# metalcycling/polynomial_reduction_with_full_domain_decomposition_preconditioner

Measured on AMD Instinct MI355X. Metric: PCG DOF-updates/sec + SpMV GB/s (%HBM peak), 3D Poisson N=7, higher is better.
Workload: dtype f64; 1 GPU; 3D Poisson, 32x32x32 elements (32^3 per GPU), N=7, flexible PCG + FDD preconditioner (single subdomain = whole domain, inner GMRES(4), polynomial reduction 6); outer=fcg, mesh=box, poly_degree=7, points_per_gpu=16777216, unique_nodes=11390625, preconditioner=fdd_gmres4, comm=single

## Files before the change

include/fdd_hip.h:

```cpp
#ifndef FDD_HIP_H
#define FDD_HIP_H

#include <stddef.h>

#ifdef __cplusplus
extern "C" {
#endif

#define FDD_ERR_INVALID_ARGUMENT (-1)
#define FDD_ERR_UNSUPPORTED (-2)
#define FDD_ERR_NOT_INITIALIZED (-3)

#define FDD_NUM_GEOM_FACTS 6
#define FDD_REDUCE_MAX_BLOCKS 2048

const char *fdd_version(void);
const char *fdd_last_error(void);
int fdd_device_count(int *count);
int fdd_set_device(int device);
int fdd_get_device(int *device);
int fdd_device_name(char *buf, size_t buf_len);
int fdd_malloc(void **ptr, size_t bytes);
int fdd_free(void *ptr);
int fdd_memcpy_h2d(void *dst, const void *src, size_t bytes, void *stream);
// ... 46 lines not shown
int fdd_dom_initialize_arrays(double *u_k, double *r_k, const double *f, int num_points, void *stream);

size_t fdd_reduce_workspace_doubles(void);
int fdd_dom_residual_norm(double *out, double *ws, const double *r_k, const double *QQt_r_k, const double *dirichlet_mask, int num_points, void *stream);
int fdd_dom_projection_inner_products(double *out2, double *ws, const double *z_k, const double *r_k, const double *p_k, const double *q_k, int num_points, void *stream);
int fdd_dom_inner_product_flexible(double *out, double *ws, const double *r_k, const double *r_kp1, const double *z_k, int num_points, void *stream);
int fdd_dom_inner_product_flexible_gamma(double *out2, double *ws, const double *r_k, const double *r_kp1, const double *z_k, int num_points, void *stream);
int fdd_dom_lincomb_flexible_gamma(double *out2, double *ws, const double *r_k, const double *r_kp1, double *z_k, int num_points, int slice_begin, int slice_size, int z_is_zero, const double *coeffs_dev, const double *const *v, const double *v_scale_dev, const double *last_dev, int m, void *stream);
int fdd_dom_inner_product(double *out, double *ws, const double *u_k, const double *v_k, const double *dirichlet_mask, int num_points, void *stream);

int fdd_dom_solution_and_residual_update(double *u_k, double *r_kp1, const double *r_k, const double *p_k, const double *q_k, double alpha_k, int num_points, void *stream);
int fdd_dom_residual_and_search_update(double *p_k, double *r_k, const double *z_k, const double *r_kp1, double beta_k, int num_points, void *stream);
int fdd_dom_solution_and_residual_update_dev(double *u_k, double *r_kp1, const double *r_k, const double *p_k, const double *q_k, const double *alpha_num, const double *alpha_den, int num_points, void *stream);
int fdd_dom_residual_and_search_update_dev(double *p_k, double *r_k, const double *z_k, const double *r_kp1, const double *beta_num, const double *beta_den, int num_points, void *stream);

int fdd_sub_stiffness_matrix_1(double *const GDu[3], const double *u, const double *const *D_hat_ptr, const int *offset, const int *vert, const int *level, const int *poly_degree, int num_levels, const double *const G[FDD_NUM_GEOM_FACTS], int num_points, int dim, void *stream);
int fdd_sub_stiffness_matrix_2(double *Au, const double *const GDu[3], const double *const *D_hat_ptr, const int *offset, const int *vert, const int *level, const int *poly_degree, int num_levels, int num_points, int dim, void *stream);
int fdd_sub_stiffness_matrix(double *Au, const double *u, const double *D_hat, const double *const G[FDD_NUM_GEOM_FACTS], const int *elem_offset, int num_elements, int poly_degree, void *stream);
int fdd_stiffness_matrix_2d(double *Au, const double *u, const double *D_hat, const double *const G[FDD_NUM_GEOM_FACTS], const int *elem_offset, int num_elements, int poly_degree, void *stream);
int fdd_sub_stiffness_matrix_gather(double *Au, const double *v, const int *point_dof, const double *D_hat, const double *const G[FDD_NUM_GEOM_FACTS], const int *elem_offset, int num_elements, int poly_degree, void *stream);

int fdd_sub_inner_product(double *out, double *ws, const double *u, const double *v, int num_values, void *stream);
int fdd_sub_weighted_inner_product(double *out, double *ws, const double *u, const double *v, const double *w, int num_values, void *stream);
int fdd_sub_projection_inner_products(double *out2, double *ws, const double *z_k, const double *r_k, const double *p_k, const double *q_k, const double *weight, int num_values, void *stream);
int fdd_sub_search_update_inner_product(double *out, double *ws, const double *r_k, const double *r_kp1, const double *z_k, const double *weight, int num_points, void *stream);
int fdd_sub_initialize_arrays(double *u_k, double *r_k, const double *f, int num_values, void *stream);
int fdd_sub_solution_and_residual_update(double *u_k, double *r_kp1, const double *r_k, const double *p_k, const double *q_k, double alpha_k, int num_values, void *stream);
int fdd_sub_residual_and_search_update(double *p_k, double *r_k, const double *z_k, const double *r_kp1, double beta_k, int num_values, void *stream);
int fdd_sub_copy_f64_f64(double *u, const double *v, int num_points, void *stream);
int fdd_sub_copy_f32_f64(float *u, const double *v, int num_points, void *stream);
int fdd_sub_copy_f64_f32(double *u, const float *v, int num_points, void *stream);
int fdd_sub_restriction_1(double *Ju, const double *J_cf, const double *u, int num_points, int n_f, int n_c, int dim, void *stream);
int fdd_sub_restriction_2(double *Ju, const double *J_cf, const double *u, int num_points, int n_f, int n_c, int dim, void *stream);
int fdd_sub_restriction_3(double *Ju, const double *J_cf, const double *u, int num_points, int n_f, int n_c, void *stream);
int fdd_sub_restriction(double *u_c, const double *J_cf, const double *u_f, int num_elements, int n_f, int n_c, void *stream);
int fdd_sub_restriction_2d(double *u_c, const double *J_cf, const double *u_f, int num_elements, int n_f, int n_c, void *stream);

int fdd_amg_vector_set_to_value(double *data, double value, int size, void *stream);
int fdd_amg_main_scaled_residual(double *Sr, double *w, const double *f_m_Au, const double *S, double alpha, int size, void *stream);
int fdd_amg_main_polynomial_evaluation(double *w, double *v, const double *r, const double *D_val, double alpha, int size, void *stream);
int fdd_amg_main_update_field(double *u, const double *w, const double *D_val, int size, void *stream);
int fdd_amg_vector_multiplication(double *uv, const double *u, const double *v, int size, void *stream);
int fdd_amg_matvec(double *y, const int *ptr, const int *col, const double *val, const double *x, double alpha, double beta, int num_rows, void *stream);
int fdd_csr_plan_matvec(const fdd_csr_plan *plan, double *y, const int *A_ptr, const int *A_col, const double *A_val, const double *x, double alpha, double beta, void *stream);
int fdd_csr_plan_matvec_to(const fdd_csr_plan *plan, double *y, const double *y_in, const int *A_ptr, const int *A_col, const double *A_val, const double *x, double alpha, double beta, void *stream);
int fdd_amg_smooth_residual_matvec(const fdd_csr_plan *plan, double *work, double *Sr, const int *A_ptr, const int *A_col, const double *A_val, const double *u, const double *f, const double *D_val, double coef, void *stream);
int fdd_amg_smooth_polynomial_matvec(const fdd_csr_plan *plan, double *work_out, const int *A_ptr, const int *A_col, const double *A_val, const double *work_in, const double *Sr, const double *D_val, double coef, void *stream);
int fdd_amg_smooth_update_matvec(const fdd_csr_plan *plan, double *u, const int *A_ptr, const int *A_col, const double *A_val, const double *work_in, const double *Sr, const double *D_val, double coef, void *stream);
int fdd_amg_smooth_start(double *work, double *Sr, const double *f, const double *D_val, double coef, int size, void *stream);

int fdd_lattice_supported(int n, int m, int *supported);
int fdd_lattice_prolong(double *u, const double *coarse, const int *owner_dof, const int *coarse_dof, int n, int m, const int *lo, const int *hi, const double *wl, long long num_elements, void *stream);
int fdd_lattice_prolong_f32(float *u, const float *coarse, const int *owner_dof, const int *coarse_dof, int n, int m, const int *lo, const int *hi, const double *wl, long long num_elements, void *stream);
int fdd_lattice_restrict(double *partial, const double *fine, const int *owner_dof, int n, int m, const int *lo, const int *hi, const double *wl, long long num_elements, void *stream);
int fdd_lattice_restrict_f32(float *partial, const float *fine, const int *owner_dof, int n, int m, const int *lo, const int *hi, const double *wl, long long num_elements, void *stream);
int fdd_csr_plan_create_f32(fdd_csr_plan **plan, const int *A_ptr_host, int num_rows, int num_cols, int num_nnz);
int fdd_csr_plan_matvec_to_f32(const fdd_csr_plan *plan, float *y, const float *y_in, const int *A_ptr, const int *A_col, const float *A_val, const float *x, float alpha, float beta, void *stream);
int fdd_amg_smooth_residual_matvec_f32(const fdd_csr_plan *plan, float *work, float *Sr, const int *A_ptr, const int *A_col, const float *A_val, const float *u, const float *f, const float *D_val, float coef, void *stream);
int fdd_amg_smooth_polynomial_matvec_f32(const fdd_csr_plan *plan, float *work_out, const int *A_ptr, const int *A_col, const float *A_val, const float *work_in, const float *Sr, const float *D_val, float coef, void *stream);
int fdd_amg_smooth_update_matvec_from_zero(const fdd_csr_plan *plan, double *u, const int *A_ptr, const int *A_col, const double *A_val, const double *work_in, const double *Sr, const double *D_val, double coef, void *stream);
int fdd_amg_smooth_update_matvec_from_zero_f32(const fdd_csr_plan *plan, float *u, const int *A_ptr, const int *A_col, const float *A_val, const float *work_in, const float *Sr, const float *D_val, float coef, void *stream);
int fdd_amg_smooth_update_matvec_f32(const fdd_csr_plan *plan, float *u, const int *A_ptr, const int *A_col, const float *A_val, const float *work_in, const float *Sr, const float *D_val, float coef, void *stream);
int fdd_amg_smooth_start_f32(float *work, float *Sr, const float *f, const float *D_val, float coef, int size, void *stream);
int fdd_amg_vector_set_to_value_f32(float *data, float value, int size, void *stream);
int fdd_amg_dot(double *out, double *ws, const double *x, const double *y, int size, void *stream);

#define FDD_MULTI_MAX 8
#define FDD_GMRES_SLOT (FDD_MULTI_MAX + 2)
int fdd_multi_weighted_inner_product(double *out, double *ws, const double *a, const double *const *b, int m, const double *w, int n, void *stream);
int fdd_multi_axpy(double *q, const double *coeffs, const double *const *v, int m, int n, void *stream);
int fdd_multi_axpy_norm2_dev(double *out, double *ws, double *y, const double *coeffs_dev, double sign, const double *const *x, int m, const double *w, int n, void *stream);
int fdd_vector_scaling_rsqrt_dev(double *au, const double *norm2_dev, const double *u, int n, void *stream);
int fdd_multi_axpy_dev(double *q, const double *coeffs_dev, const double *const *v, int m, int n, void *stream);

#define FDD_PROJECTION_MAX 16
int fdd_projection_dots(double *out, double *ws, const double *X, int ld, int K, const double *f, int n, void *stream);
int fdd_projection_apply(double *x, double *b, double *nu2_out, double *ws, const double *x_in, const double *b_in, const double *X, const double *AX, int ld, int K, const double *coeffs_dev, double sign_x, double sign_b, int n, void *stream);
int fdd_projection_store(double *Xk, double *AXk, const double *x, const double *b, const double *nu2_dev, int n, void *stream);

int fdd_cheby_step(double *x, double *d, double *r_out, const double *r_in, const double *q, const double *dinv, double c_d, double c_r, int first, int last, int n, void *stream);
int fdd_cheby_step_f32(float *x, float *d, float *r_out, const float *r_in, const float *q, const float *dinv, float c_d, float c_r, int first, int last, int n, void *stream);
int fdd_csr_plan_gather_cheby(const fdd_csr_plan *plan, double *x, double *d, double *r_out, const int *Qt_ptr, const int *Qt_col, const double *u, const double *r_in, const double *dinv, double c_d, double c_r, int last, void *stream);
int fdd_csr_plan_gather_cheby_f32(const fdd_csr_plan *plan, float *x, float *d, float *r_out, const int *Qt_ptr, const int *Qt_col, const float *u, const float *r_in, const float *dinv, float c_d, float c_r, int last, void *stream);

size_t fdd_gmres_state_bytes(void);
int fdd_gmres_begin_dev(void *state, const double *norm2_dev, int first_cycle, void *stream);
int fdd_gmres_step_dev(void *state, const double *dots_dev, int j, int iterations_before, int max_iterations, double tolerance, int use_relative, void *stream);
int fdd_gmres_finish_dev(void *state, int m, void *stream);
int fdd_gmres_fetch(void *state, double *y, double *hist, int *num_hist, int *j_last, int *steps, int *converged, void *stream);
int fdd_gmres_coefficients(void *state, const double **y_dev);
int fdd_gmres_scales(void *state, const double **inv_dev);
int fdd_gmres_last_column(void *state, const double **j_last_dev);
int fdd_sub_stiffness_matrix_gather_scaled(double *Au, const double *v, const double *v_scale_dev, const int *point_dof, const double *D_hat, const double *const G[FDD_NUM_GEOM_FACTS], const int *elem_offset, int num_elements, int poly_degree, void *stream);
int fdd_multi_weighted_inner_product_scaled(double *out, double *ws, const double *a, const double *const *b, const double *b_scale_dev, int m, const double *w, int n, void *stream);
int fdd_multi_axpy_norm2_scaled_dev(double *out, double *ws, double *dst, const double *y, const double *coeffs_dev, double sign, const double *const *x, const double *x_scale_dev, int m, const double *w, int n, void *stream);
int fdd_multi_axpy_scaled_dev(double *q, const double *coeffs_dev, const double *const *v, const double *v_scale_dev, int m, int n, void *stream);
int fdd_vector_scaling_dev(double *au, const double *scale_dev, const double *u, int n, void *stream);
int fdd_multi_lincomb_scaled_dev(double *q, int q_is_zero, const double *coeffs_dev, const double *const *v, const double *v_scale_dev, int m, int n, void *stream);
int fdd_multi_lincomb_limited_dev(double *q, int q_is_zero, const double *coeffs_dev, const double *const *v, const double *v_scale_dev, const double *last_dev, int m, int n, void *stream);
int fdd_sqrt_sum_dev(double *out, const double *parts_dev, int nparts, void *stream);
int fdd_stiffness_matrix_affine(double *Au, const double *v, const double *v_scale_dev, const int *point_dof, const double *D_hat, const double *elem_factors, const double *gll_weights, const int *elem_offset, int num_elements, int poly_degree, void *stream);
int fdd_stiffness_matrix_mfma_affine(double *Au, const double *v, const double *v_scale_dev, const int *point_dof, const double *D_hat, const double *elem_factors, const double *gll_weights, const int *elem_offset, int num_elements, int poly_degree, void *stream);
int fdd_stiffness_affine_detect(double *elem_factors, double *deviation, const double *const G[FDD_NUM_GEOM_FACTS], const int *elem_offset, const double *gll_weights, int num_elements, int poly_degree, void *stream);
int fdd_stiffness_matrix_diag(double *Au, const double *v, const double *v_scale_dev, const int *point_dof, const double *D_hat, const double *const G[FDD_NUM_GEOM_FACTS], const int *elem_offset, int num_elements, int poly_degree, void *stream);
int fdd_stiffness_matrix_diag_f32(float *Au, const float *v, const double *v_scale_dev, const int *point_dof, const float *D_hat, const float *const G[FDD_NUM_GEOM_FACTS], const int *elem_offset, int num_elements, int poly_degree, void *stream);
int fdd_stiffness_matrix_lines(double *Au, const double *v, const double *v_scale_dev, const int *point_dof, const double *D_hat, const double *const G[FDD_NUM_GEOM_FACTS], const int *elem_offset, int num_elements, int poly_degree, int diag, void *stream);
int fdd_stiffness_matrix_lines_f32(float *Au, const float *v, const double *v_scale_dev, const int *point_dof, const float *D_hat, const float *const G[FDD_NUM_GEOM_FACTS], const int *elem_offset, int num_elements, int poly_degree, int diag, void *stream);
int fdd_stiffness_offdiag_zero(int *flags_out, const double *const G[FDD_NUM_GEOM_FACTS], const int *elem_offset, int num_elements, int poly_degree, void *stream);
int fdd_stiffness_matrix_lines_shared(double *Au, const double *v, const double *v_scale_dev, const int *point_dof, const double *D_hat, const double *const G[FDD_NUM_GEOM_FACTS], const int *elem_offset, const int *factor_elem, int num_elements, int poly_degree, int diag, void *stream);
int fdd_stiffness_matrix_lines_shared_f32(float *Au, const float *v, const double *v_scale_dev, const int *point_dof, const float *D_hat, const float *const G[FDD_NUM_GEOM_FACTS], const int *elem_offset, const int *factor_elem, int num_elements, int poly_degree, int diag, void *stream);
int fdd_stiffness_matrix_lines_lean(double *Au, const double *v, const double *v_scale_dev, const int *point_dof, const double *D_hat, const double *const G[FDD_NUM_GEOM_FACTS], const int *elem_offset, const int *factor_elem, int num_elements, int poly_degree, int diag, void *stream);
int fdd_stiffness_matrix_lines_lean_f32(float *Au, const float *v, const double *v_scale_dev, const int *point_dof, const float *D_hat, const float *const G[FDD_NUM_GEOM_FACTS], const int *elem_offset, const int *factor_elem, int num_elements, int poly_degree, int diag, void *stream);
int fdd_stiffness_factor_block_hash(unsigned long long *out, const double *const G[FDD_NUM_GEOM_FACTS], const int *elem_offset, int num_elements, int poly_degree, void *stream);
int fdd_stiffness_factor_block_verify(int *mismatches, const double *const G[FDD_NUM_GEOM_FACTS], const int *elem_offset, const int *factor_elem, int num_elements, int poly_degree, void *stream);
int fdd_stiffness_matrix_affine_f32(float *Au, const float *v, const double *v_scale_dev, const int *point_dof, const float *D_hat, const float *elem_factors, const float *gll_weights, const int *elem_offset, int num_elements, int poly_degree, void *stream);
int fdd_sub_stiffness_matrix_gather_scaled_f32(float *Au, const float *v, const double *v_scale_dev, const int *point_dof, const float *D_hat, const float *const G[FDD_NUM_GEOM_FACTS], const int *elem_offset, int num_elements, int poly_degree, void *stream);
int fdd_multi_inner_product_scaled_f32(double *out, double *ws, const float *a, const float *const *b, const double *b_scale_dev, int m, int n, void *stream);
int fdd_multi_axpy_norm2_scaled_dev_f32(double *out, double *ws, float *dst, const float *y, const double *coeffs_dev, double sign, const float *const *x, const double *x_scale_dev, int m, int n, void *stream);
int fdd_vector_scaling_dev_f32(float *au, const double *scale_dev, const float *u, int n, void *stream);
int fdd_vector_diagonal_scaling_dev(double *z, const double *d, const double *scale_dev, const double *u, int n, void *stream);
int fdd_vector_diagonal_scaling_dev_f32(float *z, const float *d, const double *scale_dev, const float *u, int n, void *stream);
int fdd_vector_vector_addition_f32(float *uv, float alpha, const float *u, float beta, const float *v, int n, void *stream);
int fdd_multi_lincomb_limited_dev_f32(float *q, int q_is_zero, const double *coeffs_dev, const float *const *v, const double *v_scale_dev, const double *last_dev, int m, int n, void *stream);
int fdd_gather_rows_f32(float *t, const int *ptr, const int *col, const float *u, int row_lo, int row_hi, void *stream);
int fdd_csr_plan_gather_f32(const fdd_csr_plan *plan, float *t, const int *ptr, const int *col, const float *u, int row_lo, int row_hi, void *stream);
int fdd_gather_indexed_f32(float *out, const float *in, const int *index, int n, void *stream);
int fdd_gather_indexed_f32_f64(double *out, const float *in, const int *index, int n, void *stream);
int fdd_xmay_ratio_dev(double *out, const double *x, const double *num_dev, const double *den_dev, const double *y, int n, void *stream);
int fdd_xpby_ratio_dev(double *out, const double *x, const double *num_dev, const double *den_dev, const double *y, int n, void *stream);
int fdd_gather_weighted_norm2(double *out, double *ws, const int *Qt_ptr, const int *Qt_col, const double *u, const double *node_weight, int num_nodes, void *stream);

int fdd_dssum_fused(double *QQtu, double *t, const int *Qt_ptr, const int *Qt_col, const double *u, const double *node_weight, const double *point_mask, int node_start, int node_end, void *stream);
int fdd_dssum_gather(double *t, const int *Qt_ptr, const int *Qt_col, const double *u, const double *node_weight, int node_start, int node_end, void *stream);
int fdd_dssum_scatter(double *QQtu, const double *t, const int *Qt_ptr, const int *Qt_col, const double *point_mask, int node_start, int node_end, void *stream);
int fdd_fill_indexed(double *out, const int *idx, double value, int n, void *stream);
int fdd_gather_indexed(double *out, const double *in, const int *index, const double *scale, int n, void *stream);
int fdd_gather_indexed_split(double *out, const double *lo, const double *hi, int split, const int *index, int n, void *stream);
int fdd_scatter_add_indexed(double *y, const int *index, const double *t, int n, void *stream);
int fdd_scatter_add_indexed_f32(float *y, const int *index, const float *t, int n, void *stream);
int fdd_csr_plan_dssum(const fdd_csr_plan *plan, double *QQtu, double *t, const int *Qt_ptr, const int *Qt_col, const double *u, const double *node_weight, const double *point_mask, int row_lo, int row_hi, int mode, void *stream);
int fdd_csr_plan_gather_weighted_norm2(const fdd_csr_plan *plan, double *out, double *ws, const int *Qt_ptr, const int *Qt_col, const double *u, const double *node_weight, void *stream);

int fdd_interface_pack(double *slots, const int *slot_of, const double *prefix, int n, void *stream);
int fdd_interface_unpack(double *prefix, const double *slots, const int *slot_of, int n, void *stream);
int fdd_interface_gather(double *buf, const int *index, int n, const double *a, const double *b, void *stream);
int fdd_interface_sum(double *a, double *b, const int *ptr, const int *col, int rows, const double *buf, void *stream);

int fdd_amg_setup_row_pointers(int *ptr, int *ptr_host, const int *row_len, int rows, void *stream);
int fdd_amg_setup_spgemm_count(int *row_len, int *cursor_ws, const int *A_ptr, const int *A_col, const int *B_ptr, const int *B_col, int a_rows, int b_rows, void *stream);
int fdd_amg_setup_spgemm_fill(int *C_col, double *C_val, int *cursor_ws, const int *C_ptr, const int *A_ptr, const int *A_col, const double *A_val, const int *B_ptr, const int *B_col, const double *B_val, int a_rows, int b_rows, void *stream);
int fdd_amg_setup_transpose_count(int *row_len, const int *A_ptr, const int *A_col, const double *A_val, int a_rows, int a_cols, double drop_tol, void *stream);
int fdd_amg_setup_transpose_fill(int *T_col, double *T_val, int *cursor_ws, int *src_ws, const int *T_ptr, const int *A_ptr, const int *A_col, const double *A_val, int a_rows, int a_cols, int nnz_t, double drop_tol, void *stream);
int fdd_amg_setup_fem_stencils(double *K, unsigned int *mask, const double *x, const double *y, const double *z, const int *point_dof, int poly_degree, int num_elements, double epsilon, void *stream);
int fdd_amg_setup_fem_count(int *row_len, const int *dof_ptr, const int *dof_points, const unsigned int *mask, const int *point_dof, int poly_degree, int num_dofs, void *stream);
int fdd_amg_setup_fem_fill(int *A_col, double *A_val, const int *A_ptr, const int *dof_ptr, const int *dof_points, const unsigned int *mask, const double *K, const int *point_dof, int poly_degree, int num_dofs, void *stream);
int fdd_amg_setup_inv_sqrt_diagonal(double *D, const int *A_ptr, const int *A_col, const double *A_val, int rows, void *stream);
int fdd_amg_setup_unit_values(int *flag, const double *val, long long nnz, void *stream);
int fdd_amg_setup_lattice_dofs(int *first, int *kept, const int *point_dof, long long num_elements, int num_dofs, int n, int m, const int *keep, const int *lo, const int *hi, const double *wl, void *stream);
int fdd_amg_setup_lattice_coarse_flags(int *flag, const int *first, const int *kept, int num_dofs, void *stream);
int fdd_amg_setup_lattice_cmap(int *cmap, int *owner_dof, int *unplaced, const int *cstart, const int *first, const int *kept, long long num_points, int num_dofs, void *stream);
int fdd_amg_setup_lattice_interp_count(int *row_len, const int *cmap, const int *first, const int *point_dof, int num_dofs, int n, int m, const int *keep, const int *lo, const int *hi, const double *wl, void *stream);
int fdd_amg_setup_lattice_interp_fill(int *P_col, double *P_val, const int *P_ptr, const int *cmap, const int *first, const int *point_dof, int num_dofs, int n, int m, const int *keep, const int *lo, const int *hi, const double *wl, void *stream);
int fdd_amg_setup_lattice_coarse_points(int *coarse_point_dof, const int *point_dof, const int *cmap, long long num_elements, int n, int m, const int *keep, const int *lo, const int *hi, const double *wl, void *stream);
int fdd_amg_setup_memory_info(size_t *free_bytes, size_t *total_bytes);

#ifdef __cplusplus
}
#endif

#endif
```

include/fdd_host.h:

```cpp
#ifndef FDD_HOST_H
#define FDD_HOST_H

#include <stddef.h>

#ifdef __cplusplus
extern "C" {
#endif

const char *fddh_last_error(void);

int fddh_init(int device, void *stream, int own_stream);
int fddh_set_print(int on);
int fddh_set_timer(int on);
int fddh_timer_total(const char *key, double *seconds);
int fddh_timer_total_over_ranks(const char *key, const char *aggregation, double *seconds);

int fddh_comm_single(void);
int fddh_comm_rccl_unique_id(char *out128);
int fddh_comm_rccl_init(const char *id128, int rank, int size);
typedef int (*fddh_allreduce_fn)(void *ctx, void *buf, long long n);
typedef int (*fddh_allgather_fn)(void *ctx, const void *send, void *recv, long long bytes);
typedef int (*fddh_barrier_fn)(void *ctx);
int fddh_comm_callbacks(int rank, int size, void *ctx, fddh_allreduce_fn allreduce_sum_f64, fddh_allreduce_fn allreduce_max_f64, fddh_allgather_fn allgather_bytes, fddh_barrier_fn barrier);
typedef int (*fddh_exchange_fn)(void *ctx, int n, const int *peers, const void *const *send, const long long *send_bytes, void *const *recv, const long long *recv_bytes);
int fddh_comm_callbacks_ex(int rank, int size, void *ctx, fddh_allreduce_fn allreduce_sum_f64, fddh_allreduce_fn allreduce_max_f64, fddh_allgather_fn allgather_bytes, fddh_barrier_fn barrier, fddh_exchange_fn exchange_bytes);
int fddh_local_world_create(void **world, int size);
int fddh_local_world_destroy(void *world);
int fddh_local_world_fail(void *world);
int fddh_rank_finalize(void);
int fddh_comm_local(void *world, int rank);
int fddh_comm_info(int *rank, int *size, char *name, size_t name_len);
int fddh_comm_selftest(int n);

typedef struct fddh_problem fddh_problem;

int fddh_problem_create_box(fddh_problem **out, const int E[3], const int P[3], int poly_degree, int poly_reduction, int with_subdomain);
int fddh_problem_create_dir(fddh_problem **out, const char *directory, int poly_degree, int poly_reduction, int subdomain_overlap, int superdomain_overlap, int with_subdomain);
enum
{
    FDDH_WITH_SUBDOMAIN = 1,
    FDDH_BLOCK_LOCAL = 2,
    FDDH_FORCE_COMPOSITE = 4
};
int fddh_problem_create_box_ex(fddh_problem **out, const int E[3], const int P[3], int poly_degree, int poly_reduction, int subdomain_overlap, int superdomain_overlap, int flags);
int fddh_problem_create_dir_ex(fddh_problem **out, const char *directory, int poly_degree, int poly_reduction, int subdomain_overlap, int superdomain_overlap, int flags);
int fddh_problem_destroy(fddh_problem *p);
int fddh_write_box_mesh_files(const char *directory, const int E[3], const int P[3], int poly_degree, int rank);
int fddh_problem_create_kershaw_ex(fddh_problem **out, const int E[3], const int P[3], int poly_degree, int poly_reduction, int subdomain_overlap, int superdomain_overlap, int flags, double eps_y, double eps_z);
int fddh_write_kershaw_mesh_files(const char *directory, const int E[3], const int P[3], int poly_degree, int rank, double eps_y, double eps_z);

enum
{
    FDDH_INFO_NUM_LOCAL_POINTS = 0,
    FDDH_INFO_NUM_LOCAL_NODES,
    FDDH_INFO_NUM_BDARY_NODES,
    FDDH_INFO_NUM_INTERFACE_SLOTS,
    FDDH_INFO_NUM_TOTAL_NODES,
    FDDH_INFO_NUM_TOTAL_ELEMENTS,
    FDDH_INFO_NUM_LOCAL_ELEMENTS,
    FDDH_INFO_NUM_LEVELS,
    FDDH_INFO_SUB_NUM_VALUES,
    FDDH_INFO_SUB_NUM_DOFS,
    FDDH_INFO_NUM_ITERATIONS,
    FDDH_INFO_DIM,
    FDDH_INFO_COUNT
};
int fddh_problem_info(const fddh_problem *p, long long *info, int n);
int fddh_problem_level_degree(const fddh_problem *p, int level, int *poly_degree);

enum
{
    FDDH_SUB_IS_COMPOSITE = 0,
    FDDH_SUB_NUM_ELEMS,
    FDDH_SUB_NUM_EXT_ELEMS,
    FDDH_SUB_NUM_POINTS,
    FDDH_SUB_NUM_SUB_DOFS,
    FDDH_SUB_NUM_SUB_EXT_DOFS,
    FDDH_SUB_NUM_INTERFACE_DOFS,
    FDDH_SUB_NUM_SUP_DOFS,
    FDDH_SUB_NUM_SUP_EXT_DOFS,
    FDDH_SUB_NUM_UNIQUE_DOFS,
    FDDH_SUB_NUM_COARSE_DOFS,
    FDDH_SUB_NUM_VALUES,
    FDDH_SUB_OWN_POINTS,
    FDDH_SUB_NUM_PEERS,
    FDDH_SUB_INFO_COUNT
};
int fddh_problem_sub_info(const fddh_problem *p, long long *info, int n);
int fddh_problem_sub_region(const fddh_problem *p, int *element, int *level, int n);
int fddh_problem_sub_composite_levels(const fddh_problem *p, int *kept, int n, int *num_levels);

int fddh_problem_mesh_array(const fddh_problem *p, int level, const char *name, void *out, size_t bytes);
int fddh_problem_csr(const fddh_problem *p, int which , int *num_rows, int *num_cols, int *num_nnz, int *ptr, int *col, double *val);
int fddh_problem_assembled_weight(const fddh_problem *p, double *out, int n);

int fddh_problem_set_D_hat(fddh_problem *p, int level, const double *D_hat, int n);
int fddh_problem_get_D_hat(const fddh_problem *p, int level, double *D_hat, int n);

int fddh_problem_set_options(fddh_problem *p, int max_iterations, double tolerance, int num_vectors, int use_preconditioner, int preconditioner_type, int sub_num_vectors, int sub_max_iterations, int sub_build_tree);

int fddh_problem_affine_info(fddh_problem *p, int *fine_domain_affine, int *sub_lists_affine, int *sub_lists, double *max_deviation);
int fddh_problem_zero_factor_info(fddh_problem *p, int *enabled, int *fine_domain_diag, int *sub_lists_diag, int *sub_lists);
int fddh_problem_mfma_zero_factor_info(fddh_problem *p, int *enabled, int *fine_domain_mfma_diag, int *sub_lists_mfma_diag, int *sub_lists);
int fddh_problem_line_stiffness_info(fddh_problem *p, int *enabled, int *fine_domain_lines, int *sub_lists_lines, int *sub_lists);
int fddh_problem_shared_factor_info(fddh_problem *p, int *enabled, int *fine_domain_shared, int *fine_domain_classes, int *sub_lists_shared, int *sub_lists);
int fddh_problem_lean_line_info(fddh_problem *p, int *enabled, int *fine_domain_table_ok, int *fine_domain_lean, int *sub_lists_lean, int *sub_lists);
int fddh_problem_set_flag(fddh_problem *p, const char *name, int value);

int fddh_problem_sub_point_dofs(const fddh_problem *p, int *dof, int n);
int fddh_problem_amg_add_level(fddh_problem *p, int n, const int *A_ptr, const int *A_col, const double *A_val, const double *D_val, const double *coefs, int num_coefs, int n_coarse, const int *P_ptr, const int *P_col, const double *P_val);
int fddh_problem_amg_finalize(fddh_problem *p);
int fddh_problem_amg_apply(fddh_problem *p, const double *r, double *z);
int fddh_problem_amg_build(fddh_problem *p, int coarsest_size, double strength, int smooth_prolongator, int verbose, int *num_levels);
int fddh_problem_amg_level_info(const fddh_problem *p, int level, int *n, int *nnz_A, int *n_coarse, int *nnz_P);
int fddh_problem_amg_setup_info(const fddh_problem *p, int *levels_built_on_device, double *setup_seconds);
int fddh_problem_amg_level_transfer(const fddh_problem *p, int level, int *matrix_free);
int fddh_problem_amg_level_arrays(const fddh_problem *p, int level, int *A_ptr, int *A_col, double *A_val, double *D_val, double *coefs, int *P_ptr, int *P_col, double *P_val);

int fddh_problem_dssum(fddh_problem *p, double *out, const double *in, int apply_mask, int apply_weight);
int fddh_problem_stiffness(fddh_problem *p, double *out, const double *in, int apply_dssum);
int fddh_problem_residual_norm(fddh_problem *p, const double *r, double *norm);
int fddh_problem_make_rhs(fddh_problem *p, int function_id, unsigned long long seed, double *u_star, double *f);
int fddh_problem_make_rhs_from(fddh_problem *p, double *u_star_inout, double *f);

int fddh_problem_solve(fddh_problem *p, int solver_id, const double *f, double *u, double *history, int history_cap, int *num_history, int *num_iterations);

int fddh_problem_solve_timed(fddh_problem *p, int solver_id, const double *f, double *u, double *history, int history_cap, int *num_history, int *num_iterations, double *seconds);

int fddh_problem_projection_configure(fddh_problem *p, int capacity);
int fddh_problem_projection_clear(fddh_problem *p);
int fddh_problem_projection_info(const fddh_problem *p, int *capacity, int *size, long long *restarts);
int fddh_problem_projection_basis(const fddh_problem *p, int k, double *x, double *Ax);
int fddh_problem_solve_projected(fddh_problem *p, int solver_id, const double *f, double *u, double *history, int history_cap, int *num_history, int *num_iterations, double *projection, double *seconds);

int fddh_problem_precond_apply(fddh_problem *p, int type, const double *r, double *z, double *history, int history_cap, int *num_history);
int fddh_problem_sub_op(fddh_problem *p, int op, const double *in, double *out);
int fddh_problem_sub_residual_norm(fddh_problem *p, const double *r, double *norm);
int fddh_problem_sub_dof_op(fddh_problem *p, int op, const double *in, double *out, int n);
int fddh_problem_sub_jacobi_diagonal(fddh_problem *p, double *out, int n);
int fddh_problem_sub_dof_solve(fddh_problem *p, const double *fa, double *ua, int n);

int fddh_problem_inner_chebyshev_configure(fddh_problem *p, int order, double lower, double upper, int power_iterations);
int fddh_problem_inner_chebyshev_info(fddh_problem *p, int *order, double *lower, double *upper, double *lambda, int *power_iterations);

int fddh_problem_spmv_time(fddh_problem *p, int which, int iterations, double *avg_us, double *algorithmic_bytes);
#define FDDH_COMM_TIME_COUNT 6
int fddh_problem_comm_time(fddh_problem *p, int iterations, double *avg_us, double *bytes);
int fddh_spmv_stencil_time(int m, int iterations, double *avg_us, double *algorithmic_bytes, long long *num_nnz);

int fddh_problem_pcg_begin(fddh_problem *p, const double *f);
int fddh_problem_pcg_steps(fddh_problem *p, int steps, double *last_residual);
int fddh_problem_pcg_solution(fddh_problem *p, double *u);
int fddh_profile_enable(int on);
int fddh_profile_only(const char *kernel_key);
int fddh_profile_collect(char *json, size_t json_len);

int fddh_sync(void);
int fddh_barrier(void);

#ifdef __cplusplus
}
#endif

#endif
```

polynomial_reduction_with_full_domain_decomposition_preconditioner_amd/csrc/fdd_csr.hip:

```cpp
#include <type_traits>

#include "fdd_common.h"

#include <algorithm>
#include <cstdlib>
#include <vector>

namespace
{

constexpr int kBlock = 256;
constexpr int kBlockNnzMax = FDD_CSR_BLOCK_NNZ;
constexpr int kBlockNnzSmall = FDD_CSR_BLOCK_NNZ / 2;

template <typename F>
void with_block_nnz(int block_nnz, F &&f)
{
    if (block_nnz == kBlockNnzSmall)
        f(std::integral_constant<int, kBlockNnzSmall>{});
    else
        f(std::integral_constant<int, kBlockNnzMax>{});
}
template <bool kMayBeUnit = true, typename F>
void with_unit(bool unit, F &&f)
{
    if constexpr (kMayBeUnit)
    {
        if (unit) return f(std::true_type{});
    }
    f(std::false_type{});
}

template <typename T>
struct EpiPlainT
{
    static constexpr bool kFreeOrder = false;
    typedef T Opnd;
    __device__ T operand(int, const T *) const { return T(0); }
    __device__ T finish(T s, T, int) const { return s; }
};
typedef EpiPlainT<double> EpiPlain;
struct EpiWeight
{
    static constexpr bool kFreeOrder = false;
    typedef double Opnd;
    const double *weight;
    __device__ double operand(int row, const double *) const { return weight[row]; }
    __device__ double finish(double s, double w, int) const { return s * w; }
};
template <typename T>
struct EpiAxpbyT
{
    static constexpr bool kFreeOrder = true;
    typedef T Opnd;
    T alpha, beta;
    const T *y_in;
    __device__ T operand(int row, const T *y_old) const { return (beta == T(0)) ? T(0) : (y_in ? y_in[row] : y_old[row]); }
    __device__ T finish(T s, T y, int) const { return (beta == T(0)) ? alpha * s : alpha * s + beta * y; }
};
typedef EpiAxpbyT<double> EpiAxpby;

template <typename T>
struct Opnd2
{
    T a, b;
};
template <typename T>
struct Opnd3
{
    T a, b, c;
};
template <typename T>
struct EpiSmoothResidualT
{
    static constexpr bool kFreeOrder = true;
    typedef Opnd2<T> Opnd;
    const T *f, *D;
    T *r;
    T coef;
    __device__ Opnd operand(int row, const T *) const { return Opnd{f[row], D[row]}; }
    __device__ T finish(T s, Opnd o, int row) const
    {
        const T work = T(-1) * s + T(1) * o.a;
        const T sr = o.b * work;
        r[row] = sr;
        const T w = coef * sr;
        return w * o.b;
    }
};
template <typename T>
struct EpiSmoothPolyT
{
    static constexpr bool kFreeOrder = true;
    typedef Opnd2<T> Opnd;
    const T *r, *D;
    T coef;
    __device__ Opnd operand(int row, const T *) const { return Opnd{r[row], D[row]}; }
    __device__ T finish(T s, Opnd o, int) const
    {
        const T v = (T(1) * s) * o.b;
        const T w = coef * o.a + v;
        return w * o.b;
    }
};
template <typename T>
struct EpiSmoothUpdateT
{
    static constexpr bool kFreeOrder = true;
    typedef Opnd3<T> Opnd;
    const T *r, *D;
    T coef;
    __device__ Opnd operand(int row, const T *u_old) const { return Opnd{r[row], D[row], u_old[row]}; }
    __device__ T finish(T s, Opnd o, int) const
    {
        const T v = (T(1) * s) * o.b;
        const T w = coef * o.a + v;
        return o.c + o.b * w;
    }
};
template <typename T>
struct EpiSmoothUpdateZeroT
{
    static constexpr bool kFreeOrder = true;
    typedef Opnd2<T> Opnd;
// ... 457 lines not shown
    int b = fdd_xcd_windowed_block(blockIdx.x, G, xcd_window);
    if (b >= nblocks) return;

    auto bounds = [&](int4 m, int &r0, int &nrows, int &base, int &nnz) {
        r0 = m.x;
        int r1 = m.y;
        base = m.z;
        nnz = m.w;
        if (r0 < row_lo || r1 > row_hi)
        {
            r0 = r0 > row_lo ? r0 : row_lo;
            r1 = r1 < row_hi ? r1 : row_hi;
            if (r1 < r0) r1 = r0;
            base = A_ptr[r0];
            nnz = A_ptr[r1] - base;
        }
        nrows = r1 - r0;
    };
    auto load_streams = [&](int (&c)[kIts], T (&a)[kIts], int (&rp)[kRowIts], typename Epi::Opnd (&o)[kRowIts], int r0, int nrows, int base, int nnz) {
#pragma unroll
        for (int it = 0; it < kIts; it++)
        {
            const int k = threadIdx.x + it * kBlock;
            const int ks = (k < nnz) ? base + k : ((nnz > 0) ? base : 0);
            c[it] = __builtin_nontemporal_load(A_col + ks);
            a[it] = UNIT ? T(1) : __builtin_nontemporal_load(A_val + ks);
        }
#pragma unroll
        for (int it = 0; it < kRowIts; it++)
        {
            const int r = threadIdx.x + it * kBlock;
            const int rs = (r < nrows) ? r : 0;
            rp[it] = A_ptr[r0 + rs + 1];
            o[it] = epi.operand(r0 + rs, Au);
        }
    };

    int r0, nrows, base, nnz;
    bounds(meta[block_first + b], r0, nrows, base, nnz);
    int c[kIts], rp[kRowIts];
    T a[kIts];
    typename Epi::Opnd o[kRowIts];
    load_streams(c, a, rp, o, r0, nrows, base, nnz);
    int bn = b + G;
    int4 mn = meta[block_first + (bn < nblocks ? bn : b)];

    for (;;)
    {
        const bool more = bn < nblocks;
        T v[kIts];
#pragma unroll
        for (int it = 0; it < kIts; it++) v[it] = u[c[it]];
        int r0n, nrowsn, basen, nnzn;
        bounds(mn, r0n, nrowsn, basen, nnzn);
        int cn[kIts], rpn[kRowIts];
        T an[kIts];
        typename Epi::Opnd on[kRowIts];
        load_streams(cn, an, rpn, on, r0n, nrowsn, basen, nnzn);
        const int bnn = bn + G;
        const int4 mnn = meta[block_first + (bnn < nblocks ? bnn : (more ? bn : b))];

#pragma unroll
        for (int it = 0; it < kIts; it++)
        {
            const int k = threadIdx.x + it * kBlock;
            if (k < nnz) x[k] = a[it] * v[it];
        }
        if (threadIdx.x == 0) sp[0] = 0;
#pragma unroll
        for (int it = 0; it < kRowIts; it++)
        {
            const int r = threadIdx.x + it * kBlock;
            if (r < nrows) sp[r + 1] = rp[it] - base;
        }
        __syncthreads();
#pragma unroll
        for (int it = 0; it < kRowIts; it++)
        {
            const int r = threadIdx.x + it * kBlock;
            if (r < nrows)
            {
                T s = T(0);
                for (int j = sp[r]; j < sp[r + 1]; j++) s += x[j];
                Au[r0 + r] = epi.finish(s, o[it], r0 + r);
            }
        }
        if (!more) break;
        __syncthreads();
        b = bn;
        bn = bnn;
        mn = mnn;
        r0 = r0n;
        nrows = nrowsn;
        base = basen;
        nnz = nnzn;
#pragma unroll
        for (int it = 0; it < kIts; it++)
        {
            c[it] = cn[it];
            a[it] = an[it];
        }
#pragma unroll
        for (int it = 0; it < kRowIts; it++)
        {
            rp[it] = rpn[it];
            o[it] = on[it];
        }
    }
}

inline int gather_pipelined_per_cu()
{
    static const int v = fdd_env_int("FDD_TUNE_GATHER_PIPELINED", 4);
    return v;
}

template <int kBlockNnz>
__global__ __launch_bounds__(kBlock) void gather_norm2_block_kernel(double *__restrict__ ws, const int *__restrict__ Qt_ptr, const int *__restrict__ Qt_col, const double *__restrict__ u, const double *__restrict__ w, const int *__restrict__ row_blocks, int num_blocks)
{
    __shared__ double x[kBlockNnz];
    __shared__ double wsum[kBlock / FDD_WAVE];
    constexpr int kIts = kBlockNnz / kBlock;
    double acc = 0.0;

    for (int b = blockIdx.x; b < num_blocks; b += gridDim.x)
    {
        const int r0 = row_blocks[b];
        const int r1 = row_blocks[b + 1];
        const int base = Qt_ptr[r0];
        const int nnz = Qt_ptr[r1] - base;
        int c[kIts];
#pragma unroll
        for (int it = 0; it < kIts; it++)
        {
            const int k = threadIdx.x + it * kBlock;
            c[it] = Qt_col[(k < nnz) ? base + k : ((nnz > 0) ? base : 0)];
        }
        __syncthreads();
#pragma unroll
        for (int it = 0; it < kIts; it++)
        {
            const int k = threadIdx.x + it * kBlock;
            const double v = u[c[it]];
            if (k < nnz) x[k] = 1.0 * v;
        }
        __syncthreads();
        for (int row = r0 + threadIdx.x; row < r1; row += kBlock)
        {
            const int j0 = Qt_ptr[row] - base;
            const int j1 = Qt_ptr[row + 1] - base;
            double s = 0.0;
            for (int j = j0; j < j1; j++) s += x[j];
            const double wn = w[row];
            s = s * wn;
            acc += s * s * wn;
        }
    }

    acc = wave_sum(acc);
    if ((threadIdx.x & (FDD_WAVE - 1)) == 0) wsum[threadIdx.x / FDD_WAVE] = acc;
    __syncthreads();
    if (threadIdx.x == 0)
    {
        double tsum = wsum[0];
#pragma unroll
        for (int k = 1; k < kBlock / FDD_WAVE; k++) tsum += wsum[k];
        ws[blockIdx.x] = tsum;
// ... 572 lines not shown
static int plan_gather_cheby(const fdd_csr_plan *plan, T *x, T *d, T *r_out, const int *Qt_ptr, const int *Qt_col, const T *u, const T *r_in, const T *dinv, T c_d, T c_r, int last, void *stream)
{
    FDD_REQUIRE(plan != nullptr);
    if (plan->num_rows == 0) return 0;
    FDD_REQUIRE(x != nullptr && d != nullptr && Qt_ptr != nullptr && Qt_col != nullptr && u != nullptr && r_in != nullptr && dinv != nullptr && (last || r_out != nullptr));
    FDD_REQUIRE((const void *)u != (const void *)x && (const void *)u != (const void *)d && (const void *)u != (const void *)r_out);
    constexpr bool kDouble = std::is_same<T, double>::value;
    if (plan->value_bytes != (int)sizeof(T))
    {
        fdd_set_error("%s", kDouble ? "fdd_csr_plan_gather_cheby: a plan of fdd_csr_plan_create_f32" : "fdd_csr_plan_gather_cheby_f32: not a plan of fdd_csr_plan_create_f32");
        return FDD_ERR_INVALID_ARGUMENT;
    }
    if (!(plan->unit_values && plan->sell_slices == 0 && launch_short_pipelined<T>(plan, x, Qt_ptr, Qt_col, (const T *)nullptr, u, EpiChebyStepT<T>{r_in, dinv, r_out, d, c_d, c_r, last ? 1 : 0}, BlockRange{0, plan->num_blocks}, 0, plan->num_rows, fdd_stream(stream), true)))
    {
        fdd_set_error("fdd_csr_plan_gather_cheby%s: not a unit-value plan of the pipelined short-row kernel", kDouble ? "" : "_f32");
        return FDD_ERR_INVALID_ARGUMENT;
    }
    FDD_LAUNCH_CHECK();
    return 0;
}
extern "C" {

int fdd_csr_plan_gather_cheby(const fdd_csr_plan *plan, double *x, double *d, double *r_out, const int *Qt_ptr, const int *Qt_col, const double *u, const double *r_in, const double *dinv, double c_d, double c_r, int last, void *stream)
{
    return plan_gather_cheby<double>(plan, x, d, r_out, Qt_ptr, Qt_col, u, r_in, dinv, c_d, c_r, last, stream);
}

int fdd_csr_plan_gather_cheby_f32(const fdd_csr_plan *plan, float *x, float *d, float *r_out, const int *Qt_ptr, const int *Qt_col, const float *u, const float *r_in, const float *dinv, float c_d, float c_r, int last, void *stream)
{
    return plan_gather_cheby<float>(plan, x, d, r_out, Qt_ptr, Qt_col, u, r_in, dinv, c_d, c_r, last, stream);
}

int fdd_csr_plan_dssum(const fdd_csr_plan *plan, double *QQtu, double *t, const int *Qt_ptr, const int *Qt_col, const double *u, const double *node_weight, const double *point_mask, int row_lo, int row_hi, int mode, void *stream)
{
    FDD_REQUIRE(plan != nullptr && mode >= 0 && mode <= 2);
    FDD_REQUIRE(row_lo >= 0 && row_hi >= row_lo && row_hi <= plan->num_rows);
    if (row_hi == row_lo) return 0;
    FDD_REQUIRE(plan->unit_values != 0);
    FDD_REQUIRE(Qt_ptr != nullptr && Qt_col != nullptr);
    FDD_REQUIRE(mode == 1 || QQtu != nullptr);
    FDD_REQUIRE(mode == 2 || u != nullptr);
    FDD_REQUIRE(mode == 0 || t != nullptr);

    if (plan->kind == 0 || plan->has_long_rows)
    {
        if (mode == 0) return fdd_dssum_fused(QQtu, t, Qt_ptr, Qt_col, u, node_weight, point_mask, row_lo, row_hi, stream);
        if (mode == 1) return fdd_dssum_gather(t, Qt_ptr, Qt_col, u, node_weight, row_lo, row_hi, stream);
        return fdd_dssum_scatter(QQtu, t, Qt_ptr, Qt_col, point_mask, row_lo, row_hi, stream);
    }

    const BlockRange blocks = blocks_overlapping(plan, row_lo, row_hi);
    if (blocks.empty()) return 0;
    hipStream_t s = fdd_stream(stream);
    const bool W = node_weight != nullptr && mode != 2, M = point_mask != nullptr && mode != 1;
    const auto run = [&](auto kMode, auto kWeight, auto kMask) {
        launch_dssum_blocks<double, decltype(kMode)::value, decltype(kWeight)::value, decltype(kMask)::value>(plan, blocks, QQtu, t, Qt_ptr, Qt_col, u, node_weight, point_mask, row_lo, row_hi, s);
    };
    constexpr std::integral_constant<int, 0> fused{};
    constexpr std::integral_constant<int, 1> gather{};
    constexpr std::integral_constant<int, 2> scatter{};
    constexpr std::true_type yes{};
    constexpr std::false_type no{};
    if (mode == 0)
    {
        if (W && M) run(fused, yes, yes);
        else if (W) run(fused, yes, no);
        else if (M) run(fused, no, yes);
        else run(fused, no, no);
    }
    else if (mode == 1)
    {
        if (W) run(gather, yes, no);
        else if (!launch_short_pipelined<double>(plan, t, Qt_ptr, Qt_col, (const double *)nullptr, u, EpiPlain{}, blocks, row_lo, row_hi, s, true)) run(gather, no, no);
    }
    else
    {
        if (M) run(scatter, no, yes);
        else run(scatter, no, no);
    }
    FDD_LAUNCH_CHECK();
    return 0;
}

int fdd_csr_plan_gather_weighted_norm2(const fdd_csr_plan *plan, double *out, double *ws, const int *Qt_ptr, const int *Qt_col, const double *u, const double *node_weight, void *stream)
{
    FDD_REQUIRE(plan != nullptr && out != nullptr && ws != nullptr);
    hipStream_t s = fdd_stream(stream);
    if (plan->num_rows == 0) return (int)hipMemsetAsync(out, 0, sizeof(double), s);
    FDD_REQUIRE(plan->unit_values != 0 && Qt_ptr != nullptr && Qt_col != nullptr && u != nullptr && node_weight != nullptr);
    if (plan->kind == 0 || plan->has_long_rows) return fdd_gather_weighted_norm2(out, ws, Qt_ptr, Qt_col, u, node_weight, plan->num_rows, stream);
    const int grid = plan->num_blocks < FDD_REDUCE_MAX_BLOCKS ? plan->num_blocks : FDD_REDUCE_MAX_BLOCKS;
    with_block_nnz(plan->block_nnz, [&](auto nnz) {
        hipLaunchKernelGGL(gather_norm2_block_kernel<decltype(nnz)::value>, dim3(grid), dim3(kBlock), 0, s, ws, Qt_ptr, Qt_col, u, node_weight, plan->row_blocks_dev, plan->num_blocks);
    });
    FDD_LAUNCH_CHECK();
    hipLaunchKernelGGL(fold_partials_kernel, dim3(1), dim3(kBlock), 0, s, out, ws, grid);
    FDD_LAUNCH_CHECK();
    return 0;
}

int fdd_csr_plan_set_unit_values(fdd_csr_plan *plan, int unit_values)
{
    FDD_REQUIRE(plan != nullptr);
    plan->unit_values = unit_values != 0;
    return 0;
}

int fdd_csr_plan_kind(const fdd_csr_plan *plan, int *kind)
{
    FDD_REQUIRE(plan != nullptr && kind != nullptr);
    *kind = plan->kind;
    return 0;
}

int fdd_csr_plan_pipelined(const fdd_csr_plan *plan, int *pipelined)
{
    FDD_REQUIRE(plan != nullptr && pipelined != nullptr);
    *pipelined = (plan->sell_slices == 0 && short_pipelined_applies(plan)) ? 1 : 0;
    return 0;
}

int fdd_csr_plan_multiply(const fdd_csr_plan *plan, double *Au, const int *A_ptr, const int *A_col, const double *A_val, const double *u, const double *weight, void *stream)
{
    FDD_REQUIRE(plan != nullptr);
    FDD_REQUIRE(plan->value_bytes == 8);
    if (plan->num_rows == 0 || plan->num_cols == 0) return 0;
    FDD_REQUIRE(Au != nullptr && A_ptr != nullptr && u != nullptr);

    if (weight) return plan_launch<double, false>(plan, Au, A_ptr, A_col, A_val, u, EpiWeight{weight}, stream);
    return plan_launch<double, false>(plan, Au, A_ptr, A_col, A_val, u, EpiPlain{}, stream);
}

int fdd_csr_plan_matvec(const fdd_csr_plan *plan, double *y, const int *A_ptr, const int *A_col, const double *A_val, const double *x, double alpha, double beta, void *stream)
{
    return fdd_csr_plan_matvec_to(plan, y, nullptr, A_ptr, A_col, A_val, x, alpha, beta, stream);
}

int fdd_csr_plan_matvec_to(const fdd_csr_plan *plan, double *y, const double *y_in, const int *A_ptr, const int *A_col, const double *A_val, const double *x, double alpha, double beta, void *stream)
{
    return plan_spmv_entry(plan, y, A_ptr, A_col, A_val, x, EpiAxpby{alpha, beta, y_in}, stream, FDD_PRECONDITION(y != nullptr && A_ptr != nullptr && x != nullptr && y != x));
}

int fdd_amg_smooth_residual_matvec(const fdd_csr_plan *plan, double *work, double *Sr, const int *A_ptr, const int *A_col, const double *A_val, const double *u, const double *f, const double *D_val, double coef, void *stream)
{
    return plan_spmv_entry(plan, work, A_ptr, A_col, A_val, u, EpiSmoothResidual{f, D_val, Sr, coef}, stream, FDD_PRECONDITION(work != nullptr && Sr != nullptr && A_ptr != nullptr && u != nullptr && f != nullptr && D_val != nullptr && work != u && Sr != u));
}

int fdd_amg_smooth_polynomial_matvec(const fdd_csr_plan *plan, double *work_out, const int *A_ptr, const int *A_col, const double *A_val, const double *work_in, const double *Sr, const double *D_val, double coef, void *stream)
{
    return plan_spmv_entry(plan, work_out, A_ptr, A_col, A_val, work_in, EpiSmoothPoly{Sr, D_val, coef}, stream, FDD_PRECONDITION(work_out != nullptr && A_ptr != nullptr && work_in != nullptr && Sr != nullptr && D_val != nullptr && work_out != work_in));
}

int fdd_amg_smooth_update_matvec(const fdd_csr_plan *plan, double *u, const int *A_ptr, const int *A_col, const double *A_val, const double *work_in, const double *Sr, const double *D_val, double coef, void *stream)
{
    return plan_spmv_entry(plan, u, A_ptr, A_col, A_val, work_in, EpiSmoothUpdate{Sr, D_val, coef}, stream, FDD_PRECONDITION(u != nullptr && A_ptr != nullptr && work_in != nullptr && Sr != nullptr && D_val != nullptr && u != work_in));
}

int fdd_amg_smooth_update_matvec_from_zero(const fdd_csr_plan *plan, double *u, const int *A_ptr, const int *A_col, const double *A_val, const double *work_in, const double *Sr, const double *D_val, double coef, void *stream)
{
    return plan_spmv_entry(plan, u, A_ptr, A_col, A_val, work_in, EpiSmoothUpdateZeroT<double>{Sr, D_val, coef}, stream, FDD_PRECONDITION(u != nullptr && A_ptr != nullptr && work_in != nullptr && Sr != nullptr && D_val != nullptr && u != work_in));
}

int fdd_csr_plan_matvec_to_f32(const fdd_csr_plan *plan, float *y, const float *y_in, const int *A_ptr, const int *A_col, const float *A_val, const float *x, float alpha, float beta, void *stream)
{
    return plan_spmv_entry(plan, y, A_ptr, A_col, A_val, x, EpiAxpbyT<float>{alpha, beta, y_in}, stream, FDD_PRECONDITION(y != nullptr && A_ptr != nullptr && A_val != nullptr && x != nullptr && y != x));
}
// ... 23 lines not shown
```

polynomial_reduction_with_full_domain_decomposition_preconditioner_amd/csrc/fdd_stiffness.hip:

```cpp
#include "fdd_common.h"

namespace
{

constexpr int kBlock = 256;

template <typename T>
struct GPtrsT
{
    const T *g[FDD_NUM_GEOM_FACTS];
};

struct GPtrs
{
    const double *g[FDD_NUM_GEOM_FACTS];
};
struct GDuPtrs
{
    double *g[3];
};
struct LevelTable
{
    const double *D_hat[16];
    int poly_degree[16];
// ... 483 lines not shown
#pragma unroll
    for (int p = 0; p < 8; p++)
    {
        const T *Dp = line_row(D_hat, p);
#pragma unroll
        for (int i = 0; i < 8; i++) au[i] += Dp[i] * gdu[p];
    }
}

enum : int
{
    kLeanTerms = 1,
    kLeanResident = 2
};

template <typename T, bool kResident>
struct LeanTable
{
    static constexpr int slot(int m) { return m - (m > 9) - (m > 18) - (m > 27); }
    const T *D_hat;
    T d[kResident ? 29 : 1];
    __device__ __forceinline__ explicit LeanTable(const T *__restrict__ D) : D_hat(D)
    {
        if constexpr (kResident)
        {
            T top[32];
#pragma unroll
            for (int m = 0; m < 32; m++) top[m] = D[m];
#pragma unroll
            for (int m = 0; m < 32; m++)
                if (m != 9 and m != 18 and m != 27)
                {
                    T v = top[m];
                    asm volatile("" : "+s"(v));
                    d[slot(m)] = v;
                }
        }
    }
    __device__ __forceinline__ const T *row(int r) const { return kResident ? nullptr : line_row(D_hat, r); }
    __device__ __forceinline__ T at(const T *row_r, int r, int c) const
    {
        if constexpr (kResident)
        {
            const int m = c + 8 * r;
            return m < 32 ? d[slot(m)] : -d[slot(63 - m)];
        }
        else
            return row_r[c];
    }
};
__device__ __forceinline__ constexpr bool lean_zero_entry(int r, int c) { return r == c and r >= 1 and r <= 6; }

template <typename T, bool kResident>
__device__ __forceinline__ void lean_du(T (&du)[8], const T (&ul)[8], const LeanTable<T, kResident> &D)
{
#pragma unroll
    for (int i = 0; i < 8; i++)
    {
        const T *Di = D.row(i);
        du[i] = D.at(Di, i, 0) * ul[0];
#pragma unroll
        for (int p = 1; p < 8; p++)
            if (not lean_zero_entry(i, p)) du[i] += D.at(Di, i, p) * ul[p];
    }
}
template <typename T, bool kResident>
__device__ __forceinline__ void lean_au(T (&au)[8], const T (&gdu)[8], const LeanTable<T, kResident> &D)
{
#pragma unroll
    for (int p = 0; p < 8; p++)
    {
        const T *Dp = D.row(p);
#pragma unroll
        for (int i = 0; i < 8; i++)
        {
            if (p == 0)
                au[i] = D.at(Dp, 0, i) * gdu[0];
            else if (not lean_zero_entry(p, i))
                au[i] += D.at(Dp, p, i) * gdu[p];
        }
    }
}

template <typename T, bool kGather, bool kNTStore, bool kShared = false, int kLean = 0>
__global__ __launch_bounds__(kBlock, 4) void line_stiffness_kernel_t(T *__restrict__ Au, const T *__restrict__ u, const int *__restrict__ point_dof, const double *__restrict__ u_scale, const T *__restrict__ D_hat, GPtrsT<T> G, const int *__restrict__ elem_offset, int num_elements, const int *__restrict__ factor_elem)
{
    using C = LineCfg;
    constexpr int n = C::n, nn = C::nn;
    __shared__ T s_a[C::epb][C::tile];
    __shared__ T s_b[C::epb][C::tile];

    const int tid = threadIdx.x;
    const int e_loc = __builtin_amdgcn_readfirstlane(tid >> 6);
    const int l = tid & 63;
    const int a = l & 7, b = l >> 3;
    const int elem = blockIdx.x * C::epb + e_loc;
    if (elem >= num_elements) return;
    const size_t base = elem_offset ? (size_t)elem_offset[elem] : (size_t)elem * C::n3;
    size_t fbase = base;
    if (kShared)
    {
        const int rep = factor_elem[elem];
        fbase = elem_offset ? (size_t)elem_offset[rep] : (size_t)rep * C::n3;
    }
    T *ta = s_a[e_loc], *tb = s_b[e_loc];
    constexpr bool kTerms = (kLean & kLeanTerms) != 0, kResident = (kLean & kLeanResident) != 0;
    static_assert(kTerms or not kResident, "the resident table does not hold the diagonal entries");
    const LeanTable<T, kResident> Dl(D_hat);

    T r_u[n];
    if (kGather)
    {
        const int *pd = point_dof + base;
        int d[n];
#pragma unroll
        for (int k = 0; k < n; k++) d[k] = __builtin_nontemporal_load(pd + (l + k * nn));
#pragma unroll
        for (int k = 0; k < n; k++) r_u[k] = u[d[k] < 0 ? 0 : d[k]];
#pragma unroll
        for (int k = 0; k < n; k++) r_u[k] = (d[k] < 0) ? T(0) : r_u[k];
        if (u_scale)
        {
            const T sc = (T)(*u_scale);
#pragma unroll
            for (int k = 0; k < n; k++) r_u[k] = sc * r_u[k];
        }
    }
    else
    {
        const T *up = u + base;
#pragma unroll
        for (int k = 0; k < n; k++) r_u[k] = __builtin_nontemporal_load(up + (l + k * nn));
    }

    T r_3[n];
    if constexpr (not kTerms)
    {
#pragma unroll
        for (int m = 0; m < n; m++) r_3[m] = T(0);
    }

    {
        T g0[n], g1[n], g2[n];
#pragma unroll
        for (int k = 0; k < n; k++) g2[k] = kShared ? G.g[2][fbase + (l + k * nn)] : __builtin_nontemporal_load(G.g[2] + fbase + (l + k * nn));
        {
            const T *g0p = G.g[0] + fbase + 8 * l;
#pragma unroll
            for (int p = 0; p < n; p++) g0[p] = g0p[p];
        }
        {
            const T *g1p = G.g[1] + fbase + (a + nn * b);
#pragma unroll
            for (int p = 0; p < n; p++) g1[p] = kShared ? g1p[8 * p] : __builtin_nontemporal_load(g1p + 8 * p);
        }

#pragma unroll
        for (int k = 0; k < n; k++) ta[C::at(a, b, k)] = r_u[k];
        element_sync<true>();

#pragma unroll
        for (int k = 0; k < n; k++)
        {
            if constexpr (kTerms)
            {
                const T *Dk = Dl.row(k);
                T Du_3 = Dl.at(Dk, k, 0) * r_u[0];
#pragma unroll
                for (int p = 1; p < n; p++)
                    if (not lean_zero_entry(k, p)) Du_3 += Dl.at(Dk, k, p) * r_u[p];
                const T GDu_3 = g2[k] * Du_3;
#pragma unroll
                for (int m = 0; m < n; m++)
                {
                    if (k == 0)
                        r_3[m] = Dl.at(Dk, 0, m) * GDu_3;
                    else if (not lean_zero_entry(k, m))
                        r_3[m] += Dl.at(Dk, k, m) * GDu_3;
                }
            }
            else
            {
                const T *Dk = line_row(D_hat, k);
                T Du_3 = T(0);
#pragma unroll
                for (int p = 0; p < n; p++) Du_3 += Dk[p] * r_u[p];
                const T GDu_3 = g2[k] * Du_3;
#pragma unroll
                for (int m = 0; m < n; m++) r_3[m] += Dk[m] * GDu_3;
            }
        }

        T ul[n], w[n], au[n];
#pragma unroll
        for (int p = 0; p < n; p++) ul[p] = ta[C::at(p, a, b)];
        if constexpr (kTerms) lean_du(w, ul, Dl); else line_du(w, ul, D_hat);
#pragma unroll
        for (int p = 0; p < n; p++) w[p] = g0[p] * w[p];
        if constexpr (kTerms) lean_au(au, w, Dl); else line_au(au, w, D_hat);
#pragma unroll
        for (int p = 0; p < n; p++) tb[C::at(p, a, b)] = au[p];
#pragma unroll
        for (int p = 0; p < n; p++) ul[p] = ta[C::at(a, p, b)];
        element_sync<true>();
        if constexpr (kTerms) lean_du(w, ul, Dl); else line_du(w, ul, D_hat);
#pragma unroll
        for (int p = 0; p < n; p++) w[p] = g1[p] * w[p];
        if constexpr (kTerms) lean_au(au, w, Dl); else line_au(au, w, D_hat);
#pragma unroll
        for (int p = 0; p < n; p++) ta[C::at(a, p, b)] = au[p];
        element_sync<true>();
    }

    T *Aup = Au + base;
#pragma unroll
    for (int k = 0; k < n; k++)
    {
        const T v = (tb[C::at(a, b, k)] + ta[C::at(a, b, k)]) + r_3[k];
        if (kNTStore)
            __builtin_nontemporal_store(v, Aup + (l + k * nn));
        else
            Aup[l + k * nn] = v;
    }
}

template <typename T, int kLean>
int launch_lines_t(T *Au, const T *u, const int *point_dof, const double *u_scale, const T *D_hat, const GPtrsT<T> &G, const int *elem_offset, const int *factor_elem, int num_elements, void *stream)
{
    const int grid = (num_elements + LineCfg::epb - 1) / LineCfg::epb;
    fdd_for_bool(factor_elem != nullptr, [&](auto shared) {
        for_gather_nt_store(point_dof, [&](auto gather, auto nt) {
            hipLaunchKernelGGL((line_stiffness_kernel_t<T, decltype(gather)::value, decltype(nt)::value, decltype(shared)::value, kLean>), dim3(grid), dim3(kBlock), 0, fdd_stream(stream), Au, u, point_dof, u_scale, D_hat, G, elem_offset, num_elements, factor_elem);
        });
    });
    FDD_LAUNCH_CHECK();
    return 0;
}

#ifdef FDD_LEAN_LINE_DEV
static int g_lean_line_parts = 0;
extern "C" int fdd_dev_lean_line_parts(int parts)
{
    if (parts != 0 && parts != kLeanTerms && parts != (kLeanTerms | kLeanResident)) return FDD_ERR_UNSUPPORTED;
    g_lean_line_parts = parts;
    return 0;
}
#endif

enum class LineEntry
{
    streamed,
    shared,
    lean
};
template <typename T>
int lines_dispatch(LineEntry entry, T *Au, const T *u, const int *point_dof, const double *u_scale, const T *D_hat, const T *const G[FDD_NUM_GEOM_FACTS], const int *elem_offset, const int *factor_elem, int num_elements, int poly_degree, int diag, void *stream)
{
    if (entry == LineEntry::shared && diag != 1)
    {
        fdd_set_error("the shared-block line form of the stiffness kernel exists on three factor arrays only (diag = 1), got diag = %d", diag);
        return FDD_ERR_UNSUPPORTED;
    }
    FDD_REQUIRE(num_elements >= 0 && (entry == LineEntry::lean || diag == 0 || diag == 1));
    if (entry == LineEntry::lean && (poly_degree != 7 || diag != 1))
    {
        fdd_set_error("the lean line form of the stiffness kernel supports poly_degree 7 on three factor arrays (diag = 1) only, got poly_degree %d, diag = %d", poly_degree, diag);
        return FDD_ERR_UNSUPPORTED;
    }
    if (poly_degree != 7)
    {
        fdd_set_error("the line form of the stiffness kernel supports poly_degree 7 only, got %d", poly_degree);
        return FDD_ERR_UNSUPPORTED;
    }
    if (diag == 0)
    {
        fdd_set_error("the line form of the stiffness kernel on six factor arrays measured no faster than the slab form and is not compiled in (diag = 0)");
        return FDD_ERR_UNSUPPORTED;
    }
    if (num_elements == 0) return 0;
    FDD_REQUIRE(Au != nullptr && u != nullptr && D_hat != nullptr && G != nullptr);
    FDD_REQUIRE(entry != LineEntry::shared || factor_elem != nullptr);
    GPtrsT<T> g;
    if (int rc = fdd_three_factors(g, G)) return rc;
    if (entry != LineEntry::lean) return launch_lines_t<T, 0>(Au, u, point_dof, u_scale, D_hat, g, elem_offset, entry == LineEntry::shared ? factor_elem : nullptr, num_elements, stream);
    constexpr int kParts = sizeof(T) == 8 ? (kLeanTerms | kLeanResident) : kLeanTerms;
#ifdef FDD_LEAN_LINE_DEV
    constexpr int kOther = kParts ^ kLeanResident;
    if (g_lean_line_parts == kOther) return launch_lines_t<T, kOther>(Au, u, point_dof, u_scale, D_hat, g, elem_offset, factor_elem, num_elements, stream);
#endif
    return launch_lines_t<T, kParts>(Au, u, point_dof, u_scale, D_hat, g, elem_offset, factor_elem, num_elements, stream);
}

__device__ __forceinline__ unsigned long long factor_word_mix(unsigned long long bits, unsigned long long position)
{
    unsigned long long z = bits + (position + 1ull) * 0x9e3779b97f4a7c15ull;
    z = (z ^ (z >> 30)) * 0xbf58476d1ce4e5b9ull;
    z = (z ^ (z >> 27)) * 0x94d049bb133111ebull;
    return z ^ (z >> 31);
}

__global__ __launch_bounds__(kBlock) void factor_block_hash_kernel(unsigned long long *__restrict__ out, GPtrs G, const int *__restrict__ elem_offset, int n3, int num_elements)
{
    __shared__ unsigned long long s_h[kBlock];
    for (int e = blockIdx.x; e < num_elements; e += gridDim.x)
    {
        const size_t base = elem_offset ? (size_t)elem_offset[e] : (size_t)e * n3;
        unsigned long long h = 0;
        for (int idx = threadIdx.x; idx < 3 * n3; idx += kBlock)
        {
            const int f = idx / n3;
            h += factor_word_mix((unsigned long long)__double_as_longlong(G.g[f][base + (idx - f * n3)]), (unsigned long long)idx);
        }
        s_h[threadIdx.x] = h;
        __syncthreads();
        for (int w = kBlock / 2; w > 0; w >>= 1)
        {
            if ((int)threadIdx.x < w) s_h[threadIdx.x] += s_h[threadIdx.x + w];
            __syncthreads();
        }
        if (threadIdx.x == 0) out[e] = s_h[0];
        __syncthreads();
    }
}

__global__ __launch_bounds__(kBlock) void factor_block_verify_kernel(int *__restrict__ mismatches, GPtrs G, const int *__restrict__ elem_offset, const int *__restrict__ factor_elem, int n3, int num_elements)
{
    for (int e = blockIdx.x; e < num_elements; e += gridDim.x)
    {
        const int rep = factor_elem[e];
        int differs = 0;
        if (rep < 0 or rep >= num_elements)
            differs = 1;
        else if (rep != e)
        {
            const size_t base = elem_offset ? (size_t)elem_offset[e] : (size_t)e * n3;
            const size_t rbase = elem_offset ? (size_t)elem_offset[rep] : (size_t)rep * n3;
            for (int idx = threadIdx.x; idx < 3 * n3; idx += kBlock)
            {
                const int f = idx / n3;
                const int at = idx - f * n3;
                differs |= __double_as_longlong(G.g[f][base + at]) != __double_as_longlong(G.g[f][rbase + at]);
            }
        }
        if (__syncthreads_or(differs) and threadIdx.x == 0) atomicAdd(mismatches, 1);
    }
}

__global__ __launch_bounds__(kBlock) void offdiag_zero_kernel(int *__restrict__ flags, GPtrs G, const int *__restrict__ elem_offset, int n3, size_t num_points)
{
    bool nz[3] = {false, false, false};
    for (size_t idx = (size_t)blockIdx.x * kBlock + threadIdx.x; idx < num_points; idx += (size_t)gridDim.x * kBlock)
    {
        const size_t e = idx / n3;
        const size_t at = elem_offset ? (size_t)elem_offset[e] + (idx - e * n3) : idx;
#pragma unroll
        for (int f = 0; f < 3; f++) nz[f] = nz[f] or (__double_as_longlong(G.g[3 + f][at]) & 0x7fffffffffffffffLL) != 0;
    }
#pragma unroll
    for (int f = 0; f < 3; f++)
        if (nz[f]) flags[f] = 1;
}

__global__ __launch_bounds__(kBlock) void affine_detect_kernel(double *__restrict__ c_out, double *__restrict__ deviation, GPtrs G, const int *__restrict__ elem_offset, const double *__restrict__ w, int n, int num_elements)
{
    __shared__ double s_c[FDD_NUM_GEOM_FACTS];
    __shared__ double s_max[kBlock / FDD_WAVE];
// ... 223 lines not shown
    if (num_points == 0) return 0;
    FDD_REQUIRE(GDu != nullptr && u != nullptr && D_hat != nullptr && G != nullptr);
    GDuPtrs gd;
    GPtrs g;
    for (int k = 0; k < 3; k++) gd.g[k] = GDu[k];
    for (int k = 0; k < FDD_NUM_GEOM_FACTS; k++) g.g[k] = G[k];
    const int grid = (num_points + kBlock - 1) / kBlock;
    if (dim == 2)
        hipLaunchKernelGGL(dom_stiffness_1_kernel<2>, dim3(grid), dim3(kBlock), 0, fdd_stream(stream), gd, u, D_hat, g, num_points, poly_degree + 1);
    else
        hipLaunchKernelGGL(dom_stiffness_1_kernel<3>, dim3(grid), dim3(kBlock), 0, fdd_stream(stream), gd, u, D_hat, g, num_points, poly_degree + 1);
    FDD_LAUNCH_CHECK();
    return 0;
}

int fdd_dom_stiffness_matrix_2(double *Au, const double *const GDu[3], const double *D_hat, int num_points, int poly_degree, int dim, void *stream)
{
    FDD_REQUIRE(num_points >= 0 && poly_degree >= 1 && (dim == 2 || dim == 3));
    if (num_points == 0) return 0;
    FDD_REQUIRE(Au != nullptr && GDu != nullptr && D_hat != nullptr);
    GDuPtrs gd;
    for (int k = 0; k < 3; k++) gd.g[k] = const_cast<double *>(GDu[k]);
    const int grid = (num_points + kBlock - 1) / kBlock;
    if (dim == 2)
        hipLaunchKernelGGL(dom_stiffness_2_kernel<2>, dim3(grid), dim3(kBlock), 0, fdd_stream(stream), Au, gd, D_hat, num_points, poly_degree + 1);
    else
        hipLaunchKernelGGL(dom_stiffness_2_kernel<3>, dim3(grid), dim3(kBlock), 0, fdd_stream(stream), Au, gd, D_hat, num_points, poly_degree + 1);
    FDD_LAUNCH_CHECK();
    return 0;
}

int fdd_dom_stiffness_matrix(double *Au, const double *u, const double *D_hat, const double *const G[FDD_NUM_GEOM_FACTS], int num_elements, int poly_degree, void *stream)
{
    return fused_dispatch<double>(Au, u, nullptr, nullptr, D_hat, G, nullptr, num_elements, poly_degree, stream);
}

int fdd_sub_stiffness_matrix(double *Au, const double *u, const double *D_hat, const double *const G[FDD_NUM_GEOM_FACTS], const int *elem_offset, int num_elements, int poly_degree, void *stream)
{
    return fused_dispatch<double>(Au, u, nullptr, nullptr, D_hat, G, elem_offset, num_elements, poly_degree, stream);
}

int fdd_stiffness_matrix_2d(double *Au, const double *u, const double *D_hat, const double *const G[FDD_NUM_GEOM_FACTS], const int *elem_offset, int num_elements, int poly_degree, void *stream)
{
    return fused_dispatch_2d(Au, u, D_hat, G, elem_offset, num_elements, poly_degree, stream);
}

int fdd_sub_stiffness_matrix_gather(double *Au, const double *v, const int *point_dof, const double *D_hat, const double *const G[FDD_NUM_GEOM_FACTS], const int *elem_offset, int num_elements, int poly_degree, void *stream)
{
    FDD_REQUIRE(point_dof != nullptr);
    return fused_dispatch<double>(Au, v, point_dof, nullptr, D_hat, G, elem_offset, num_elements, poly_degree, stream);
}

int fdd_sub_stiffness_matrix_gather_scaled(double *Au, const double *v, const double *v_scale_dev, const int *point_dof, const double *D_hat, const double *const G[FDD_NUM_GEOM_FACTS], const int *elem_offset, int num_elements, int poly_degree, void *stream)
{
    FDD_REQUIRE(point_dof != nullptr);
    return fused_dispatch<double>(Au, v, point_dof, v_scale_dev, D_hat, G, elem_offset, num_elements, poly_degree, stream);
}

int fdd_stiffness_matrix_affine(double *Au, const double *v, const double *v_scale_dev, const int *point_dof, const double *D_hat, const double *elem_factors, const double *gll_weights, const int *elem_offset, int num_elements, int poly_degree, void *stream)
{
    return fused_dispatch_affine<double>(Au, v, point_dof, v_scale_dev, D_hat, elem_factors, gll_weights, elem_offset, num_elements, poly_degree, stream);
}

int fdd_stiffness_matrix_diag(double *Au, const double *v, const double *v_scale_dev, const int *point_dof, const double *D_hat, const double *const G[FDD_NUM_GEOM_FACTS], const int *elem_offset, int num_elements, int poly_degree, void *stream)
{
    return fused_dispatch<double, true>(Au, v, point_dof, v_scale_dev, D_hat, G, elem_offset, num_elements, poly_degree, stream);
}

int fdd_stiffness_matrix_diag_f32(float *Au, const float *v, const double *v_scale_dev, const int *point_dof, const float *D_hat, const float *const G[FDD_NUM_GEOM_FACTS], const int *elem_offset, int num_elements, int poly_degree, void *stream)
{
    return fused_dispatch<float, true>(Au, v, point_dof, v_scale_dev, D_hat, G, elem_offset, num_elements, poly_degree, stream);
}

int fdd_stiffness_matrix_lines(double *Au, const double *v, const double *v_scale_dev, const int *point_dof, const double *D_hat, const double *const G[FDD_NUM_GEOM_FACTS], const int *elem_offset, int num_elements, int poly_degree, int diag, void *stream)
{
    return lines_dispatch<double>(LineEntry::streamed, Au, v, point_dof, v_scale_dev, D_hat, G, elem_offset, nullptr, num_elements, poly_degree, diag, stream);
}

int fdd_stiffness_matrix_lines_f32(float *Au, const float *v, const double *v_scale_dev, const int *point_dof, const float *D_hat, const float *const G[FDD_NUM_GEOM_FACTS], const int *elem_offset, int num_elements, int poly_degree, int diag, void *stream)
{
    return lines_dispatch<float>(LineEntry::streamed, Au, v, point_dof, v_scale_dev, D_hat, G, elem_offset, nullptr, num_elements, poly_degree, diag, stream);
}

int fdd_stiffness_matrix_lines_shared(double *Au, const double *v, const double *v_scale_dev, const int *point_dof, const double *D_hat, const double *const G[FDD_NUM_GEOM_FACTS], const int *elem_offset, const int *factor_elem, int num_elements, int poly_degree, int diag, void *stream)
{
    return lines_dispatch<double>(LineEntry::shared, Au, v, point_dof, v_scale_dev, D_hat, G, elem_offset, factor_elem, num_elements, poly_degree, diag, stream);
}

int fdd_stiffness_matrix_lines_shared_f32(float *Au, const float *v, const double *v_scale_dev, const int *point_dof, const float *D_hat, const float *const G[FDD_NUM_GEOM_FACTS], const int *elem_offset, const int *factor_elem, int num_elements, int poly_degree, int diag, void *stream)
{
    return lines_dispatch<float>(LineEntry::shared, Au, v, point_dof, v_scale_dev, D_hat, G, elem_offset, factor_elem, num_elements, poly_degree, diag, stream);
}

int fdd_stiffness_matrix_lines_lean(double *Au, const double *v, const double *v_scale_dev, const int *point_dof, const double *D_hat, const double *const G[FDD_NUM_GEOM_FACTS], const int *elem_offset, const int *factor_elem, int num_elements, int poly_degree, int diag, void *stream)
{
    return lines_dispatch<double>(LineEntry::lean, Au, v, point_dof, v_scale_dev, D_hat, G, elem_offset, factor_elem, num_elements, poly_degree, diag, stream);
}

int fdd_stiffness_matrix_lines_lean_f32(float *Au, const float *v, const double *v_scale_dev, const int *point_dof, const float *D_hat, const float *const G[FDD_NUM_GEOM_FACTS], const int *elem_offset, const int *factor_elem, int num_elements, int poly_degree, int diag, void *stream)
{
    return lines_dispatch<float>(LineEntry::lean, Au, v, point_dof, v_scale_dev, D_hat, G, elem_offset, factor_elem, num_elements, poly_degree, diag, stream);
}

constexpr int kFactorBlockGrid = 1 << 20;
static int factor_block_args(GPtrs &g, const double *const G[FDD_NUM_GEOM_FACTS], int num_elements, int poly_degree)
{
    FDD_REQUIRE(num_elements >= 0 && poly_degree >= 1 && G != nullptr);
    if (poly_degree > 15)
    {
        fdd_set_error("the factor-block entries support poly_degree 1..15, got %d", poly_degree);
        return FDD_ERR_UNSUPPORTED;
    }
    return fdd_three_factors(g, G);
}

int fdd_stiffness_factor_block_hash(unsigned long long *out, const double *const G[FDD_NUM_GEOM_FACTS], const int *elem_offset, int num_elements, int poly_degree, void *stream)
{
    GPtrs g;
    if (int rc = factor_block_args(g, G, num_elements, poly_degree)) return rc;
    if (num_elements == 0) return 0;
    FDD_REQUIRE(out != nullptr);
    const int n = poly_degree + 1;
    hipLaunchKernelGGL(factor_block_hash_kernel, dim3(num_elements < kFactorBlockGrid ? num_elements : kFactorBlockGrid), dim3(kBlock), 0, fdd_stream(stream), out, g, elem_offset, n * n * n, num_elements);
    FDD_LAUNCH_CHECK();
    return 0;
}

int fdd_stiffness_factor_block_verify(int *mismatches, const double *const G[FDD_NUM_GEOM_FACTS], const int *elem_offset, const int *factor_elem, int num_elements, int poly_degree, void *stream)
{
    GPtrs g;
    if (int rc = factor_block_args(g, G, num_elements, poly_degree)) return rc;
    FDD_REQUIRE(mismatches != nullptr);
    FDD_HIP_CHECK(hipMemsetAsync(mismatches, 0, sizeof(int), fdd_stream(stream)));
    if (num_elements == 0) return 0;
    FDD_REQUIRE(factor_elem != nullptr);
    const int n = poly_degree + 1;
    hipLaunchKernelGGL(factor_block_verify_kernel, dim3(num_elements < kFactorBlockGrid ? num_elements : kFactorBlockGrid), dim3(kBlock), 0, fdd_stream(stream), mismatches, g, elem_offset, factor_elem, n * n * n, num_elements);
    FDD_LAUNCH_CHECK();
    return 0;
}

int fdd_stiffness_offdiag_zero(int *flags_out, const double *const G[FDD_NUM_GEOM_FACTS], const int *elem_offset, int num_elements, int poly_degree, void *stream)
{
    FDD_REQUIRE(num_elements >= 0 && poly_degree >= 1 && flags_out != nullptr);
    FDD_HIP_CHECK(hipMemsetAsync(flags_out, 0, 3 * sizeof(int), fdd_stream(stream)));
    if (num_elements == 0) return 0;
    FDD_REQUIRE(G != nullptr && G[3] != nullptr && G[4] != nullptr && G[5] != nullptr);
    GPtrs g;
    for (int k = 0; k < FDD_NUM_GEOM_FACTS; k++) g.g[k] = G[k];
    const int n = poly_degree + 1, n3 = n * n * n;
    const size_t num_points = (size_t)num_elements * n3;
    hipLaunchKernelGGL(offdiag_zero_kernel, dim3(fdd_stream_grid((long long)num_points, kBlock)), dim3(kBlock), 0, fdd_stream(stream), flags_out, g, elem_offset, n3, num_points);
    FDD_LAUNCH_CHECK();
    return 0;
}

int fdd_stiffness_affine_detect(double *elem_factors, double *deviation, const double *const G[FDD_NUM_GEOM_FACTS], const int *elem_offset, const double *gll_weights, int num_elements, int poly_degree, void *stream)
{
    FDD_REQUIRE(num_elements >= 0 && poly_degree >= 1);
    if (num_elements == 0) return 0;
    FDD_REQUIRE(elem_factors != nullptr && deviation != nullptr && G != nullptr && gll_weights != nullptr);
    GPtrs g;
    for (int k = 0; k < FDD_NUM_GEOM_FACTS; k++)
    {
        FDD_REQUIRE(G[k] != nullptr);
        g.g[k] = G[k];
// ... 59 lines not shown
```

polynomial_reduction_with_full_domain_decomposition_preconditioner_amd/host/element_operator.hpp:

```cpp
#ifndef FDD_ELEMENT_OPERATOR_HPP
#define FDD_ELEMENT_OPERATOR_HPP

#include <algorithm>
#include <array>
#include <cstring>
#include <stdexcept>
#include <string>
#include <type_traits>
#include <unordered_map>
#include <vector>

#include "config.hpp"
#include "gll.hpp"

namespace fdd
{

template <typename Vec>
inline memory to_float(const Vec &v)
{
    std::vector<float> t(v.begin(), v.end());
    memory m = dev().malloc<float>(std::max<size_t>(t.size(), 1));
    if (not t.empty()) m.copyFrom(t.data(), t.size() * sizeof(float));
    return m;
}

struct LevelList
{
    int level = 0;
    int poly_degree = 1;
    int dim = 3;
    int num_elements = 0;
    int first_offset = 0;
    const double *G[NUM_GEOM_FACTS] = {nullptr, nullptr, nullptr, nullptr, nullptr, nullptr};
    const double *D_hat = nullptr;
    memory G32[NUM_GEOM_FACTS], D_hat32;
    bool affine = false;
    double affine_deviation = -1.0;
    memory affine_c, affine_w, affine_c32, affine_w32;
    bool offdiag_zero = false;
    bool shared_blocks = false;
    int factor_classes = 0;
    memory factor_elem;
    bool lean_D_hat = false, lean_D_hat32 = false;

    size_t num_points() const { return (size_t)num_elements * (poly_degree + 1) * (poly_degree + 1) * (dim == 3 ? poly_degree + 1 : 1); }
};

struct StiffnessFlags
{
    bool mfma_stiffness;
    bool skip_zero_factors;
    bool mfma_skip_zero_factors;
    bool line_stiffness;
    bool shared_factor_blocks;
    bool lean_line_stiffness;

    StiffnessFlags();
};

struct StiffnessFlagRow
{
    const char *name;
    bool StiffnessFlags::*member;
    struct
    {
        const void *fn;
        const char *name;
    } entries[5];
};

inline const std::array<StiffnessFlagRow, 6> &stiffness_flag_table()
{
#define FDD_ENTRY(name) {(const void *)&name, #name}
    static const std::array<StiffnessFlagRow, 6> table = {{
        {"mfma_stiffness", &StiffnessFlags::mfma_stiffness, {}},
        {"skip_zero_factors", &StiffnessFlags::skip_zero_factors, {FDD_ENTRY(fdd_stiffness_offdiag_zero), FDD_ENTRY(fdd_stiffness_matrix_diag), FDD_ENTRY(fdd_stiffness_matrix_diag_f32)}},
        {"mfma_skip_zero_factors", &StiffnessFlags::mfma_skip_zero_factors, {FDD_ENTRY(fdd_stiffness_matrix_mfma_diag), FDD_ENTRY(fdd_stiffness_offdiag_zero), FDD_ENTRY(fdd_stiffness_matrix_diag), FDD_ENTRY(fdd_stiffness_matrix_diag_f32)}},
        {"line_stiffness", &StiffnessFlags::line_stiffness, {FDD_ENTRY(fdd_stiffness_matrix_lines), FDD_ENTRY(fdd_stiffness_matrix_lines_f32)}},
        {"shared_factor_blocks", &StiffnessFlags::shared_factor_blocks, {FDD_ENTRY(fdd_stiffness_matrix_lines_shared), FDD_ENTRY(fdd_stiffness_matrix_lines_shared_f32), FDD_ENTRY(fdd_stiffness_factor_block_hash), FDD_ENTRY(fdd_stiffness_factor_block_verify)}},
        {"lean_line_stiffness", &StiffnessFlags::lean_line_stiffness, {FDD_ENTRY(fdd_stiffness_matrix_lines_lean), FDD_ENTRY(fdd_stiffness_matrix_lines_lean_f32)}},
    }};
#undef FDD_ENTRY
    return table;
}

inline const StiffnessFlagRow *stiffness_flag_row(const std::string &flag)
{
    for (const StiffnessFlagRow &row : stiffness_flag_table())
        if (flag == row.name) return &row;
    return nullptr;
}

inline const char *missing_stiffness_entry(const StiffnessFlagRow &row)
{
    for (const auto &e : row.entries)
        if (e.name and e.fn == nullptr) return e.name;
    return nullptr;
}
inline const char *missing_stiffness_entry(const char *flag) { return missing_stiffness_entry(*stiffness_flag_row(flag)); }

inline StiffnessFlags::StiffnessFlags()
{
    for (const StiffnessFlagRow &row : stiffness_flag_table()) this->*row.member = missing_stiffness_entry(row) == nullptr;
}

inline bool set_stiffness_flag(StiffnessFlags &flags, const std::string &flag, bool on)
{
    const StiffnessFlagRow *row = stiffness_flag_row(flag);
    if (not row) return false;
    if (on)
        if (const char *missing = missing_stiffness_entry(*row)) throw std::runtime_error(flag + " needs " + missing + ", which the loaded kernel library does not export");
    flags.*row->member = on;
    return true;
}
inline bool stiffness_flag(const StiffnessFlags &flags, const char *flag) { return flags.*stiffness_flag_row(flag)->member; }

inline void detect_zero_factors(LevelList &ll)
{
    ll.offdiag_zero = false;
    if (ll.dim != 3 or ll.poly_degree > 15 or ll.num_elements == 0 or missing_stiffness_entry("skip_zero_factors")) return;
    int flags[3] = {1, 1, 1};
    memory flags_dev = dev().malloc<int>(3);
    FDD_CALL(fdd_stiffness_offdiag_zero(flags_dev.as<int>(), ll.G, nullptr, ll.num_elements, ll.poly_degree, dev().stream));
    flags_dev.copyTo(flags, sizeof(flags));
    flags_dev.free();
    ll.offdiag_zero = flags[0] == 0 and flags[1] == 0 and flags[2] == 0;
}

constexpr size_t shared_factor_bytes_limit = (size_t)1 << 20;

inline void detect_shared_blocks(LevelList &ll)
{
    ll.shared_blocks = false;
    ll.factor_classes = 0;
    ll.factor_elem.free();
    if (not ll.offdiag_zero or ll.dim != 3 or ll.poly_degree > 15 or ll.num_elements == 0 or missing_stiffness_entry("shared_factor_blocks")) return;
    const size_t ne = (size_t)ll.num_elements;
    std::vector<unsigned long long> hash(ne);
    memory hash_dev = dev().malloc<unsigned long long>(ne);
    FDD_CALL(fdd_stiffness_factor_block_hash(hash_dev.as<unsigned long long>(), ll.G, nullptr, ll.num_elements, ll.poly_degree, dev().stream));
    hash_dev.copyTo(hash.data(), ne * sizeof(unsigned long long));
    hash_dev.free();
    std::vector<int> rep(ne);
    std::unordered_map<unsigned long long, int> first;
    for (size_t e = 0; e < ne; e++) rep[e] = first.emplace(hash[e], (int)e).first->second;
    ll.factor_classes = (int)first.size();
    const size_t block_bytes = 3 * (ll.num_points() / ne) * sizeof(double);
    if (first.size() * block_bytes > shared_factor_bytes_limit or 2 * first.size() > ne) return;
    int mismatches = 1;
    memory rep_dev = dev().malloc<int>(ne), mismatches_dev = dev().malloc<int>(1);
    rep_dev.copyFrom(rep.data(), ne * sizeof(int));
    FDD_CALL(fdd_stiffness_factor_block_verify(mismatches_dev.as<int>(), ll.G, nullptr, rep_dev.as<int>(), ll.num_elements, ll.poly_degree, dev().stream));
    mismatches_dev.copyTo(&mismatches, sizeof(int));
    mismatches_dev.free();
    if (mismatches != 0)
    {
        rep_dev.free();
        return;
    }
    ll.factor_elem = rep_dev;
    ll.shared_blocks = true;
}

// ... 131 lines not shown
    }
};

template <typename Real, typename Entry64, typename Entry32>
inline auto entry_of(Entry64 *entry, Entry32 *entry_f32)
{
    if constexpr (std::is_same<Real, float>::value)
        return entry_f32;
    else
        return entry;
}

template <typename Real>
inline bool launch_three_arrays(const StiffnessChoice &c, const LevelList &ll, Real *q, const Real *v, const double *scale_dev, const int *point_index)
{
    const ListArrays<Real> a(ll);
    void *s = dev().stream;
    const int *factor_elem = c.shared ? ll.factor_elem.as<int>() : nullptr;
    if (c.family == StiffnessFamily::diag)
        FDD_CALL(entry_of<Real>(fdd_stiffness_matrix_diag, fdd_stiffness_matrix_diag_f32)(q, v, scale_dev, point_index, a.D_hat, a.G, nullptr, ll.num_elements, ll.poly_degree, s));
    else if (c.family == StiffnessFamily::mfma_diag)
    {
        if constexpr (std::is_same<Real, double>::value) FDD_CALL(fdd_stiffness_matrix_mfma_diag(q, v, scale_dev, point_index, a.D_hat, a.G, nullptr, ll.num_elements, ll.poly_degree, s));
    }
    else if (c.family != StiffnessFamily::lines)
        return false;
    else if (c.lean)
        FDD_CALL(entry_of<Real>(fdd_stiffness_matrix_lines_lean, fdd_stiffness_matrix_lines_lean_f32)(q, v, scale_dev, point_index, a.D_hat, a.G, nullptr, factor_elem, ll.num_elements, ll.poly_degree, 1, s));
    else if (c.shared)
        FDD_CALL(entry_of<Real>(fdd_stiffness_matrix_lines_shared, fdd_stiffness_matrix_lines_shared_f32)(q, v, scale_dev, point_index, a.D_hat, a.G, nullptr, factor_elem, ll.num_elements, ll.poly_degree, 1, s));
    else
        FDD_CALL(entry_of<Real>(fdd_stiffness_matrix_lines, fdd_stiffness_matrix_lines_f32)(q, v, scale_dev, point_index, a.D_hat, a.G, nullptr, ll.num_elements, ll.poly_degree, 1, s));
    return true;
}

inline void apply_local(const LevelList &ll, double *Au, const double *u, const std::vector<memory> &workspace, const StiffnessFlags &flags)
{
    void *stream = dev().stream;
    Au += ll.first_offset, u += ll.first_offset;
    const StiffnessChoice c = choose_stiffness(ll, flags, false, StiffnessForm::local, Au == u);
    if (c.family == StiffnessFamily::two_launch)
    {
        double *GDu[3] = {workspace[0].as<double>(), workspace[1].as<double>(), workspace[2].as<double>()};
        FDD_CALL(fdd_dom_stiffness_matrix_1(GDu, u, ll.D_hat, ll.G, (int)ll.num_points(), ll.poly_degree, ll.dim, stream));
        FDD_CALL(fdd_dom_stiffness_matrix_2(Au, GDu, ll.D_hat, (int)ll.num_points(), ll.poly_degree, ll.dim, stream));
        return;
    }
    const StiffnessProfile p = stiffness_profile(StiffnessForm::local, c, false);
    ProfileScope prof(p.label, p.bytes_per_point * (double)ll.num_points());
    if (launch_three_arrays<double>(c, ll, Au, u, nullptr, nullptr)) return;
    if (c.family == StiffnessFamily::mfma)
        FDD_CALL(fdd_stiffness_matrix_mfma(Au, u, ll.D_hat, ll.G, nullptr, ll.num_elements, ll.poly_degree, stream));
    else if (c.family == StiffnessFamily::fused)
        FDD_CALL(fdd_sub_stiffness_matrix(Au, u, ll.D_hat, ll.G, nullptr, ll.num_elements, ll.poly_degree, stream));
    else
        FDD_CALL(fdd_stiffness_matrix_2d(Au, u, ll.D_hat, ll.G, nullptr, ll.num_elements, ll.poly_degree, stream));
}

template <typename Real>
inline void apply_gather(const LevelList &ll, Real *q, const Real *v, const int *point_index, const double *scale_dev, int gathered_values, const StiffnessFlags &flags)
{
    constexpr bool f32 = std::is_same<Real, float>::value;
    void *stream = dev().stream;
    q += ll.first_offset, point_index += ll.first_offset;
    const StiffnessChoice c = choose_stiffness(ll, flags, f32, StiffnessForm::gather);
    const StiffnessProfile p = stiffness_profile(StiffnessForm::gather, c, f32);
    ProfileScope prof(p.label, p.bytes_per_point * (double)ll.num_points() + (double)sizeof(Real) * gathered_values);
    if (launch_three_arrays<Real>(c, ll, q, v, scale_dev, point_index)) return;
    const ListArrays<Real> a(ll);
    const bool matrix_cores = c.family == StiffnessFamily::mfma or c.family == StiffnessFamily::mfma_affine;
    if (c.family == StiffnessFamily::affine or c.family == StiffnessFamily::mfma_affine)
    {
        if constexpr (f32)
            FDD_CALL(fdd_stiffness_matrix_affine_f32(q, v, scale_dev, point_index, a.D_hat, a.affine_c, a.affine_w, nullptr, ll.num_elements, ll.poly_degree, stream));
        else
            FDD_CALL((matrix_cores ? fdd_stiffness_matrix_mfma_affine : fdd_stiffness_matrix_affine)(q, v, scale_dev, point_index, a.D_hat, a.affine_c, a.affine_w, nullptr, ll.num_elements, ll.poly_degree, stream));
    }
    else if constexpr (f32)
        FDD_CALL(fdd_sub_stiffness_matrix_gather_scaled_f32(q, v, scale_dev, point_index, a.D_hat, a.G, nullptr, ll.num_elements, ll.poly_degree, stream));
    else
        FDD_CALL((matrix_cores ? fdd_stiffness_matrix_mfma_gather : fdd_sub_stiffness_matrix_gather_scaled)(q, v, scale_dev, point_index, a.D_hat, a.G, nullptr, ll.num_elements, ll.poly_degree, stream));
}

constexpr double affine_tolerance = 64.0 * 2.220446049250313e-16;
inline bool detect_affine(LevelList &ll)
{
    if (ll.dim != 3 or ll.poly_degree > 15 or ll.num_elements == 0) return false;
    if (ll.affine_deviation < 0.0)
    {
        const int n = ll.poly_degree + 1;
        std::vector<double> z(n), w(n), dev_hst(ll.num_elements);
        gll::zwgll(z.data(), w.data(), n);
        ll.affine_w = dev().malloc<double>(n);
        ll.affine_w.copyFrom(w.data(), (size_t)n * sizeof(double));
        ll.affine_c = dev().malloc<double>((size_t)ll.num_elements * NUM_GEOM_FACTS);
        memory dev_dev = dev().malloc<double>(ll.num_elements);
        FDD_CALL(fdd_stiffness_affine_detect(ll.affine_c.as<double>(), dev_dev.as<double>(), ll.G, nullptr, ll.affine_w.as<double>(), ll.num_elements, ll.poly_degree, dev().stream));
        dev_dev.copyTo(dev_hst.data(), dev_hst.size() * sizeof(double));
        dev_dev.free();
        ll.affine_deviation = 0.0;
        for (double x : dev_hst) ll.affine_deviation = (x == x) ? std::max(ll.affine_deviation, x) : 1.0;
    }
    return ll.affine_deviation <= affine_tolerance;
}

inline void affine_float_copies(LevelList &ll)
{
    if (ll.affine_deviation < 0.0 or ll.affine_c32.ptr()) return;
    const int n = ll.poly_degree + 1;
    std::vector<double> z(n), w(n), c_hst((size_t)ll.num_elements * NUM_GEOM_FACTS);
    gll::zwgll(z.data(), w.data(), n);
    ll.affine_c.copyTo(c_hst.data(), c_hst.size() * sizeof(double));
    ll.affine_c32 = to_float(c_hst);
    ll.affine_w32 = to_float(w);
}

}

#endif
```

polynomial_reduction_with_full_domain_decomposition_preconditioner_amd/host/fdd_device.hpp:

```cpp
#ifndef FDD_DEVICE_HPP
#define FDD_DEVICE_HPP

#include <cstddef>
#include <cstdio>
#include <cstdlib>
#include <string>
#include <utility>
#include <vector>

#include "fdd_hip.h"

#pragma weak fdd_amg_setup_row_pointers
#pragma weak fdd_amg_setup_spgemm_count
#pragma weak fdd_amg_setup_spgemm_fill
#pragma weak fdd_amg_setup_transpose_count
#pragma weak fdd_amg_setup_transpose_fill
#pragma weak fdd_amg_setup_fem_stencils
#pragma weak fdd_amg_setup_fem_count
#pragma weak fdd_amg_setup_fem_fill
#pragma weak fdd_amg_setup_inv_sqrt_diagonal
#pragma weak fdd_amg_setup_unit_values
#pragma weak fdd_amg_setup_lattice_dofs
#pragma weak fdd_amg_setup_lattice_coarse_flags
#pragma weak fdd_amg_setup_lattice_cmap
#pragma weak fdd_amg_setup_lattice_interp_count
#pragma weak fdd_amg_setup_lattice_interp_fill
#pragma weak fdd_amg_setup_lattice_coarse_points
#pragma weak fdd_amg_setup_memory_info
#pragma weak fdd_dom_lincomb_flexible_gamma
#pragma weak fdd_projection_dots
#pragma weak fdd_projection_apply
#pragma weak fdd_projection_store
#pragma weak fdd_cheby_step
#pragma weak fdd_cheby_step_f32
#pragma weak fdd_csr_plan_gather_cheby
#pragma weak fdd_csr_plan_gather_cheby_f32
#pragma weak fdd_stiffness_matrix_diag
#pragma weak fdd_stiffness_matrix_diag_f32
#pragma weak fdd_stiffness_offdiag_zero
#pragma weak fdd_stiffness_matrix_mfma_diag
#pragma weak fdd_stiffness_matrix_lines
#pragma weak fdd_stiffness_matrix_lines_f32
#pragma weak fdd_stiffness_matrix_lines_shared
#pragma weak fdd_stiffness_matrix_lines_shared_f32
#pragma weak fdd_stiffness_factor_block_hash
#pragma weak fdd_stiffness_factor_block_verify
#pragma weak fdd_stiffness_matrix_lines_lean
#pragma weak fdd_stiffness_matrix_lines_lean_f32

namespace fdd
{

inline const char *missing_amg_setup_entry()
{
#define FDD_SETUP_ENTRY(name) {(const void *)&name, #name}
    const struct
    {
        const void *fn;
        const char *name;
    } entries[] = {FDD_SETUP_ENTRY(fdd_amg_setup_row_pointers), FDD_SETUP_ENTRY(fdd_amg_setup_spgemm_count),    FDD_SETUP_ENTRY(fdd_amg_setup_spgemm_fill),
                   FDD_SETUP_ENTRY(fdd_amg_setup_transpose_count), FDD_SETUP_ENTRY(fdd_amg_setup_transpose_fill), FDD_SETUP_ENTRY(fdd_amg_setup_fem_stencils),
                   FDD_SETUP_ENTRY(fdd_amg_setup_fem_count),    FDD_SETUP_ENTRY(fdd_amg_setup_fem_fill),        FDD_SETUP_ENTRY(fdd_amg_setup_inv_sqrt_diagonal),
                   FDD_SETUP_ENTRY(fdd_amg_setup_unit_values), FDD_SETUP_ENTRY(fdd_amg_setup_lattice_dofs), FDD_SETUP_ENTRY(fdd_amg_setup_lattice_coarse_flags), FDD_SETUP_ENTRY(fdd_amg_setup_lattice_cmap), FDD_SETUP_ENTRY(fdd_amg_setup_lattice_interp_count), FDD_SETUP_ENTRY(fdd_amg_setup_lattice_interp_fill), FDD_SETUP_ENTRY(fdd_amg_setup_lattice_coarse_points), FDD_SETUP_ENTRY(fdd_amg_setup_memory_info)};
#undef FDD_SETUP_ENTRY
    for (const auto &e : entries)
        if (e.fn == nullptr) return e.name;
    return nullptr;
}

inline const char *missing_chebyshev_entry(bool fused)
{
    if (&fdd_cheby_step == nullptr) return "fdd_cheby_step";
    if (&fdd_cheby_step_f32 == nullptr) return "fdd_cheby_step_f32";
    if (fused and &fdd_csr_plan_gather_cheby == nullptr) return "fdd_csr_plan_gather_cheby";
    if (fused and &fdd_csr_plan_gather_cheby_f32 == nullptr) return "fdd_csr_plan_gather_cheby_f32";
    return nullptr;
}

inline void check(int rc, const char *what)
{
    if (rc != 0)
    {
        fprintf(stderr, "ERROR: %s failed (code %d): %s\n", what, rc, fdd_last_error());
        exit(EXIT_FAILURE);
    }
}

#define FDD_CALL(expr) ::fdd::check((expr), #expr)

struct device_t
{
    void *stream = nullptr;
    bool owns_stream = false;
    bool initialised = false;
    unsigned long long rank_instance = 0;

    template <typename T>
    class memory malloc(size_t n);

    void finish() { FDD_CALL(fdd_stream_sync(stream)); }
};

inline device_t &dev()
{
    static thread_local device_t d;
    return d;
}

class memory
{
  private:
    char *base_ = nullptr;
    size_t count_ = 0;
    size_t elem_ = 1;
    bool owner_ = false;

  public:
    memory() {}
    memory(void *p, size_t count, size_t elem, bool owner) : base_((char *)p), count_(count), elem_(elem), owner_(owner) {}

    void *ptr() const { return base_; }
    template <typename T>
    T *as() const
    {
        return reinterpret_cast<T *>(base_);
    }
    size_t size() const { return count_; }
    bool isInitialized() const { return base_ != nullptr; }

    void copyFrom(const void *src, size_t bytes) { FDD_CALL(fdd_memcpy_h2d(base_, src, bytes, dev().stream)); }
    void copyFrom(const memory &src, size_t bytes) { FDD_CALL(fdd_memcpy_d2d(base_, src.base_, bytes, dev().stream)); }
// ... 138 lines not shown
```

polynomial_reduction_with_full_domain_decomposition_preconditioner_amd/host/fdd_host_capi.cpp:

```cpp
#include "fdd_host.h"

#include <atomic>
#include <chrono>
#include <cmath>
#include <cstdarg>
#include <cstring>
#include <limits>
#include <exception>
#include <memory>
#include <string>
#include <sys/stat.h>
#include <unordered_map>
#include <functional>
#include <vector>

#include "box_mesh.hpp"
#include "domain.hpp"
#include "subdomain.hpp"

typedef double SType;
typedef double PType;

static thread_local char g_err[512] = "";

// ... 867 lines not shown
    catch (const std::exception &e)
    {
        return fail("%s", e.what());
    }
}

int fddh_problem_affine_info(fddh_problem *p, int *fine_domain_affine, int *sub_lists_affine, int *sub_lists, double *max_deviation)
{
    try
    {
        if (int rc = rank_check(p)) return rc;
        if (!p) return fail("null argument");
        Domain<SType> &dom = p->fine();
        double worst = dom.operator_list().affine_deviation;
        int lists = 0, affine = 0;
        if (p->subdomain)
            for (auto &ll : p->subdomain->operator_lists())
            {
                lists++;
                if (ll.affine) affine++;
                worst = std::max(worst, ll.affine_deviation);
            }
        if (fine_domain_affine) *fine_domain_affine = dom.operator_list().affine ? 1 : 0;
        if (sub_lists_affine) *sub_lists_affine = affine;
        if (sub_lists) *sub_lists = lists;
        if (max_deviation) *max_deviation = worst;
        return 0;
    }
    catch (const std::exception &e)
    {
        return fail("%s", e.what());
    }
}

static int stiffness_info(fddh_problem *p, const char *flag, bool (fdd::StiffnessChoice::*is)() const, int *enabled, int *fine_domain, int *sub_lists_on, int *sub_lists, const std::function<void(const fdd::LevelList &)> &more = nullptr)
{
    try
    {
        if (int rc = rank_check(p)) return rc;
        if (!p) return fail("null argument");
        Domain<SType> &dom = p->fine();
        if (enabled) *enabled = fdd::stiffness_flag(dom.stiffness, flag) ? 1 : 0;
        if (fine_domain) *fine_domain = (dom.operator_choice().*is)() ? 1 : 0;
        if (more) more(dom.operator_list());
        if (sub_lists_on) *sub_lists_on = p->subdomain ? p->subdomain->count_lists(is) : 0;
        if (sub_lists) *sub_lists = p->subdomain ? (int)p->subdomain->operator_lists().size() : 0;
        return 0;
    }
    catch (const std::exception &e)
    {
        return fail("%s", e.what());
    }
}

int fddh_problem_zero_factor_info(fddh_problem *p, int *enabled, int *fine_domain_diag, int *sub_lists_diag, int *sub_lists)
{
    return stiffness_info(p, "skip_zero_factors", &fdd::StiffnessChoice::three_arrays, enabled, fine_domain_diag, sub_lists_diag, sub_lists);
}

int fddh_problem_mfma_zero_factor_info(fddh_problem *p, int *enabled, int *fine_domain_mfma_diag, int *sub_lists_mfma_diag, int *sub_lists)
{
    return stiffness_info(p, "mfma_skip_zero_factors", &fdd::StiffnessChoice::mfma_three_arrays, enabled, fine_domain_mfma_diag, sub_lists_mfma_diag, sub_lists);
}

int fddh_problem_line_stiffness_info(fddh_problem *p, int *enabled, int *fine_domain_lines, int *sub_lists_lines, int *sub_lists)
{
    return stiffness_info(p, "line_stiffness", &fdd::StiffnessChoice::lines, enabled, fine_domain_lines, sub_lists_lines, sub_lists);
}

int fddh_problem_shared_factor_info(fddh_problem *p, int *enabled, int *fine_domain_shared, int *fine_domain_classes, int *sub_lists_shared, int *sub_lists)
{
    return stiffness_info(p, "shared_factor_blocks", &fdd::StiffnessChoice::shared_lines, enabled, fine_domain_shared, sub_lists_shared, sub_lists, [&](const fdd::LevelList &list) {
        if (fine_domain_classes) *fine_domain_classes = list.factor_classes;
    });
}

int fddh_problem_lean_line_info(fddh_problem *p, int *enabled, int *fine_domain_table_ok, int *fine_domain_lean, int *sub_lists_lean, int *sub_lists)
{
    return stiffness_info(p, "lean_line_stiffness", &fdd::StiffnessChoice::lean_lines, enabled, fine_domain_lean, sub_lists_lean, sub_lists, [&](const fdd::LevelList &list) {
        if (fine_domain_table_ok) *fine_domain_table_ok = list.lean_D_hat ? 1 : 0;
    });
}

int fddh_problem_set_flag(fddh_problem *p, const char *name, int value)
{
    try
    {
        if (int rc = rank_check(p)) return rc;
        if (!p || !name) return fail("null argument");
        const std::string s(name);
        if (s == "fused_dssum")
        {
            for (auto &kv : p->domains) kv.second.fused_dssum = value != 0;
            if (p->subdomain) p->subdomain->fused_dssum = value != 0;
        }
        else if (s == "restructured_inner_solve")
        {
            if (p->subdomain) p->subdomain->restructured = value != 0;
            for (auto &kv : p->domains) kv.second.restructured_outer = value != 0;
        }
        else if (s == "neighbour_interface_exchange")
        {
            for (auto &kv : p->domains) kv.second.neighbour_interface_exchange = value != 0;
        }
        else if (s == "fold_coarse_exchange")
        {
            if (p->subdomain) p->subdomain->fold_coarse_exchange = value != 0;
        }
        else if (s == "assembled_outer_solve")
        {
            for (auto &kv : p->domains) kv.second.assembled_outer = value != 0;
        }
        else if (s == "shared_residual_norm")
        {
            for (auto &kv : p->domains) kv.second.shared_residual_norm = value != 0;
        }
        else if (s == "skip_last_basis_store")
        {
            if (p->subdomain) p->subdomain->skip_last_basis_store = value != 0;
        }
        else if (s == "early_gamma")
        {
            for (auto &kv : p->domains) kv.second.early_gamma = value != 0;
        }
        else if (s == "unit_stitch_in_place")
        {
            for (auto &kv : p->domains) kv.second.unit_stitch_in_place = value != 0;
        }
        else if (s == "fused_update_flexible_dot")
        {
            for (auto &kv : p->domains) kv.second.fused_update_flexible_dot = value != 0;
        }
        else if (s == "lazy_steps")
        {
            for (auto &kv : p->domains) kv.second.lazy_steps = value != 0;
        }
        else if (s == "device_bookkeeping")
        {
            if (p->subdomain) p->subdomain->device_bookkeeping = value != 0;
            for (auto &kv : p->domains) kv.second.device_scalars = value != 0;
        }
        else if (s == "assembled_inner_solve")
        {
            if (p->subdomain) p->subdomain->assembled_inner = value != 0;
        }
        else if (s == "amg_device_setup")
        {
            if (!p->subdomain) return fail("problem was created without a Subdomain");
            if (value != 0)
                if (const char *missing = fdd::missing_amg_setup_entry()) return fail("amg_device_setup needs %s, which the loaded kernel library does not export", missing);
            p->subdomain->amg_device_setup = value != 0;
        }
        else if (s == "sub_use_preconditioner")
        {
            if (!p->subdomain) return fail("problem was created without a Subdomain");
            p->subdomain->use_preconditioner = value == 1;
            p->subdomain->use_jacobi = value == 2;
        }
        else if (s == "affine_geometry")
        {
            for (auto &kv : p->domains) kv.second.set_affine_geometry(value != 0);
            if (p->subdomain) p->subdomain->set_affine_geometry(value != 0);
            p->fine().projection.clear();
            if (p->subdomain) p->subdomain->operator_changed();
        }
        else if (fdd::stiffness_flag_row(s))
// ... 1081 lines not shown
```

polynomial_reduction_with_full_domain_decomposition_preconditioner_amd/host/subdomain.hpp:

```cpp
#ifndef FDD_SUBDOMAIN_HPP
#define FDD_SUBDOMAIN_HPP

#include <algorithm>
#include <cmath>
#include <map>
#include <stdexcept>
#include <unordered_map>
#include <chrono>
#include <vector>

#include "amg.hpp"
#include "amg_device_setup.hpp"
#include "composite.hpp"
#include "config.hpp"
#include "csr_matrix.hpp"
#include "domain.hpp"
#include "element_operator.hpp"
#include "gll.hpp"
#include "gmres.hpp"
#include "low_order.hpp"
#include "math.hpp"
#include "timer.hpp"

template <typename DType>
struct Stiffness_Operator
{
    int num_dofs = 0;
    int num_points = 0;
    int num_extended_dofs = 0;

    CSR_Matrix<DType> Q;
    CSR_Matrix<DType> Qt;

    CSR_Matrix<DType> A;
    CSR_Matrix<DType> P;
    CSR_Matrix<DType> Pt;

    fdd::memory geom_fact[NUM_GEOM_FACTS];

    std::vector<fdd::LevelList> level_lists;
};

template <typename DType>
class Subdomain
{
  private:
    std::vector<fdd::memory> work_dev;

    int poly_reduction = 1;
    int subdomain_overlap = 1;
    int superdomain_overlap = 1;

    std::vector<int> poly_degree;
    int num_levels = 0;

    struct Level
    {
        int num_points;
        int num_elements;
        int poly_degree;
        int offset;
    };
    std::vector<Level> levels;

    std::map<std::pair<int, int>, std::pair<std::vector<DType>, fdd::memory>> J_cf;

    std::vector<std::pair<std::vector<DType>, fdd::memory>> D_hat;

    Stiffness_Operator<DType> subdomain_operator;
    Stiffness_Operator<DType> superdomain_operator;
    CSR_Matrix<DType> Qt_coarse;

    int num_interface_dofs = 0;
    CSR_Matrix<DType> Q_int, Qt_int, QQt_int;

    int num_dofs = 0;
    int num_blocks = 0;
    fdd::memory norm_weight;
    fdd::memory inner_weight;

    fdd::memory f, u_k, r_k, r_kp1, q_k, z_k, p_k;
    std::vector<fdd::memory> V, Z;
    fdd::GmresScalars<DType> gmres_scalars;

    fdd::memory reduce_ws;
    fdd::memory scalars;

    template <typename Real>
    struct DofKrylov
    {
        std::vector<fdd::memory> VA;
        fdd::memory qa;
        std::vector<fdd::memory> ZA;
        fdd::memory ua, fa;
        void ensure(int m, int na, bool keep_Z)
// ... 613 lines not shown
                FDD_CALL(fdd_scatter_add_indexed(fa_out.as<double>(), ring_rows.template as<int>(), ring_tmp.as<double>(), G_ring.num_rows, fdd::dev().stream));
            }
        }
        else
            G_unit.gather_scatter(nullptr, fa_out.as<double>(), Tr.as<double>(), nullptr, nullptr, 0, nse, 1);
        if (n_slaves > 0)
        {
            G_unit.gather_scatter(nullptr, slave_vals.as<double>() - nse, Tr.as<double>(), nullptr, nullptr, nse, nse + n_slaves, 1);
            St_slave.multiply(st_tmp, slave_vals);
            FDD_CALL(fdd_scatter_add_indexed(fa_out.as<double>(), st_rows.template as<int>(), st_tmp.as<double>(), St_slave.num_rows, fdd::dev().stream));
        }
        if (n_reg > 0)
        {
            fdd::memory dst = fa_out.slice(ns, n_reg);
            dst.copyFrom(Tr.slice(subdomain_operator.num_points + nI, n_reg), (size_t)n_reg * sizeof(DType));
        }
    }

    void composite_solution_points(fdd::memory &u_l, fdd::memory &ua_in)
    {
        if (n_slaves > 0)
        {
            fdd::memory slaves = ua_in.slice(slave_base, n_slaves);
            S_slave.multiply(slaves, ua_in);
        }
        FDD_CALL(fdd_gather_indexed(u_l.as<double>(), ua_in.as<double>(), point_dof_dev.template as<int>(), nullptr, own_points, fdd::dev().stream));
    }


    struct SinglePrecision
    {
        bool ready = false;
        amg::Csr32 S, St, Asup;
        fdd::memory q_pts, slaves, st_tmp;
    } sp;

    void prepare_single_precision()
    {
        if (sp.ready) return;
        void *stream = fdd::dev().stream;
        for (auto &ll : subdomain_operator.level_lists)
        {
            const size_t np = ll.num_points();
            for (int g = 0; g < NUM_GEOM_FACTS; g++)
            {
                ll.G32[g] = fdd::dev().malloc<float>(std::max<size_t>(np, 1));
                FDD_CALL(fdd_sub_copy_f32_f64(ll.G32[g].template as<float>(), ll.G[g], (int)np, stream));
            }
        }
        for (auto &ll : subdomain_operator.level_lists)
        {
            ll.D_hat32 = fdd::to_float(D_hat[ll.level].first);
            fdd::check_lean_table32(ll, D_hat[ll.level].first);
        }
        auto plan32 = [](amg::Csr32 &M32, CSR_Matrix<DType> &M) {
            if (M.num_rows == 0 or M.num_nnz == 0) return;
            M32.val = fdd::to_float(M.val_hst);
            FDD_CALL(fdd_csr_plan_create_f32(&M32.plan, M.ptr_hst.data(), M.num_rows, M.num_cols, M.num_nnz));
        };
        if (is_composite)
        {
            plan32(sp.S, S_slave);
            plan32(sp.St, St_slave);
            plan32(sp.Asup, A_sup_reg);
        }
        sp.q_pts = fdd::dev().malloc<float>(std::max(subdomain_operator.num_points, 1));
        sp.slaves = fdd::dev().malloc<float>(std::max(n_slaves, 1));
        sp.st_tmp = fdd::dev().malloc<float>(std::max(St_slave.num_rows, 1));
        sp.ready = true;
    }

    static void multiply(CSR_Matrix<DType> &M, amg::Csr32 &, double *y, const double *x) { M.multiply(y, x); }
    static void multiply(CSR_Matrix<DType> &M, amg::Csr32 &M32, float *y, const float *x)
    {
        if (M32.plan) FDD_CALL(fdd_csr_plan_matvec_to_f32(M32.plan, y, nullptr, M.ptr.template as<int>(), M.col.template as<int>(), M32.val.template as<float>(), x, 1.0f, 0.0f, fdd::dev().stream));
    }

    template <typename Real>
    void stiffness_from_dofs(Real *q, const Real *za, const double *scale_dev = nullptr)
    {
        for (auto &ll : subdomain_operator.level_lists) fdd::apply_gather(ll, q, za, point_dof_dev.template as<int>(), scale_dev, subdomain_operator.num_extended_dofs, stiffness);
    }

    template <typename Real>
    void operator_dofs(Real *y, Real *x, const double *scale_dev = nullptr)
    {
        constexpr bool f32 = std::is_same<Real, float>::value;
        void *stream = fdd::dev().stream;
        Real *q = (f32 ? sp.q_pts : q_k).template as<Real>();
        const int nse = subdomain_operator.num_extended_dofs;
        if (not is_composite)
        {
            stiffness_from_dofs(q, x, scale_dev);
            if constexpr (f32)
                subdomain_operator.Qt.gather(y, q, 0, nse);
            else
                subdomain_operator.Qt.gather(y, q, 0, nse, norm_weight_is_one ? nullptr : norm_weight.as<double>());
            return;
        }
        const int ns = subdomain_operator.num_dofs, nI = num_interface_dofs, n_reg = superdomain_operator.num_dofs - nI;
        if (n_sup_copies > 0) fdd::ops::gather_indexed(x + num_dofs, x, copy_src.template as<int>(), n_sup_copies, stream);
        if (n_slaves > 0) multiply(S_slave, sp.S, x + slave_base, x);
        stiffness_from_dofs(q, x, scale_dev);
        G_unit.gather(y, q, 0, nse);
        if (n_slaves > 0)
        {
            Real *sl = (f32 ? sp.slaves : slave_vals).template as<Real>(), *st = (f32 ? sp.st_tmp : st_tmp).template as<Real>();
            G_unit.gather(sl - nse, q, nse, nse + n_slaves);
            multiply(St_slave, sp.St, st, sl);
            fdd::ops::scatter_add_indexed(y, st_rows.template as<int>(), st, St_slave.num_rows, stream);
        }
        if (n_reg > 0)
        {
            multiply(A_sup_reg, sp.Asup, y + ns, x + (ns - nI));
            if (scale_dev) fdd::ops::scaling_dev(y + ns, scale_dev, y + ns, n_reg, stream);
        }
    }

  public:
    int precision = 64;

    bool set_precision(int bits)
    {
        if (bits != 64 and bits != 32) return false;
        if (bits == 32 and not(dim == 3 and device_bookkeeping and ((assembled_inner and can_assemble()) or composite_dof_space()))) return false;
        precision = bits;
        if (amg_hierarchy.ready())
        {
            amg_hierarchy.set_f32_io(false);
            if (not amg_hierarchy.set_precision(bits)) return false;
        }
        return true;
    }

  private:

  public:
    bool composite_dof_space() const { return is_composite and comp_dofs_ready and assembled_inner and device_bookkeeping and num_vectors <= FDD_MULTI_MAX; }
    int own_dofs() const { return is_composite ? comp.num_own_dofs : subdomain_operator.num_extended_dofs; }

    void gmres_composite_dofs(fdd::memory &ua_out, fdd::memory &r_pts, bool print_history = true, bool use_relative = false, const double *own_assembled = nullptr)
    {
        fdd::memory &fa = krylov64.fa;
        if (not fa.ptr()) fa = fdd::dev().malloc<DType>(std::max(dof_alloc_size(), 1));
        tree_operator(f, r_pts);
        composite_rhs_dofs(fa, f, own_assembled);
        gmres_dofs_device(ua_out, fa, print_history, use_relative);
    }
    fdd::memory new_dof_vector() { return fdd::dev().malloc<DType>(std::max(dof_alloc_size(), 1)); }
    void comm_probe_coarse()
    {
        if (not is_composite or (fdd::comm().size == 1 and superdomain_operator.num_extended_dofs == 0)) return;
        fdd::memory coarse = work_dev[0].slice(levels[num_levels - 1].offset, coarse_pad);
        fdd::comm().allgather(coarse.ptr(), coarse_all.ptr(), (size_t)coarse_pad * sizeof(DType));
    }
    void comm_probe_ring()
    {
        if (not is_composite) return;
        fdd::comm().exchange(exchange_ops.data(), (int)exchange_ops.size());
    }
    void comm_probe_ring_and_coarse()
    {
        if (not is_composite) return;
        fdd::comm().exchange(exchange_ops_folded.data(), (int)exchange_ops_folded.size());
    }
    double comm_ring_and_coarse_bytes() const
    {
        double b = 0.0;
        for (const fdd::ExchangeOp &op : exchange_ops_folded) b += (double)op.send_bytes;
        return b;
    }
    double comm_coarse_bytes() const { return is_composite ? (double)coarse_pad * sizeof(DType) * fdd::comm().size : 0.0; }
    double comm_ring_bytes() const
    {
        double b = 0.0;
// ... 409 lines not shown
            D_hat[l].second = dl.D_hat;
        }

        is_composite = (fdd::comm().size > 1 and not block_local) or force_composite;
        if (is_composite)
            initialize_composite(domains, domain);
        else
            initialize_conforming(domains, domain);

        num_values = subdomain_operator.num_points + superdomain_operator.num_extended_dofs;
        num_blocks = (num_values + BLOCK_SIZE - 1) / BLOCK_SIZE;

        {
            inner_weight = fdd::dev().malloc<DType>(num_values);
            subdomain_operator.Q.multiply(inner_weight, norm_weight);
            std::vector<DType> w(num_values);
            inner_weight.copyTo(w.data(), (size_t)num_values * sizeof(DType));
            for (int i = 0; i < superdomain_operator.num_extended_dofs; i++) w[(size_t)subdomain_operator.num_points + i] = norm_weight_hst[(size_t)subdomain_operator.num_extended_dofs + i];
            for (int i = 0; i < num_values; i++)
                if (w[i] > 0.0) w[i] = 1.0;
            inner_weight.copyFrom(w.data(), (size_t)num_values * sizeof(DType));
        }

        f = fdd::dev().malloc<DType>(num_values);
        u_k = fdd::dev().malloc<DType>(num_values);
        r_k = fdd::dev().malloc<DType>(num_values);
        r_kp1 = fdd::dev().malloc<DType>(num_values);
        q_k = fdd::dev().malloc<DType>(num_values);
        z_k = fdd::dev().malloc<DType>(num_values);
        p_k = fdd::dev().malloc<DType>(num_values);

        reduce_ws = fdd::dev().malloc<double>(fdd_reduce_workspace_doubles());
        scalars = fdd::dev().malloc<double>(2 * FDD_GMRES_SLOT);

        subdomain_operator.Q.release_host();
        subdomain_operator.Qt.release_host();
    }

    template <typename PType>
    void initialize_conforming(std::unordered_map<int, PType> &domains, PType &domain)
    {
        const int P = domain.num_local_points;
        const int total_level_points = levels[num_levels - 1].offset + levels[num_levels - 1].num_points;

        work_dev.resize(3);
        for (int w = 0; w < 3; w++) work_dev[w] = fdd::dev().malloc<DType>((size_t)total_level_points + (size_t)P + 16);

        for (int g = 0; g < NUM_GEOM_FACTS; g++) subdomain_operator.geom_fact[g] = domain.geom_fact[g];

        std::vector<double> tmp(P);
        {
            const auto &node = domain.scatter_matrix().col_hst;
            std::vector<int> dof_of_node(domain.num_local_nodes, 0);
            for (int p = 0; p < P; p++)
                if (domain.mesh.p_mask[p] > 0.0) dof_of_node[node[p]] = 1;
            int count = 0;
            for (int n = 0; n < domain.num_local_nodes; n++)
                if (dof_of_node[n]) dof_of_node[n] = ++count;
            for (int p = 0; p < P; p++) tmp[p] = (domain.mesh.p_mask[p] > 0.0) ? (double)dof_of_node[node[p]] : 0.0;
        }

        int max_dof = 0;
        for (int p = 0; p < P; p++) max_dof = std::max(max_dof, (int)tmp[p]);

        {
            std::vector<int> q_ptr((size_t)P + 1, 0);
            for (int p = 0; p < P; p++) q_ptr[p + 1] = q_ptr[p] + (tmp[p] > 0.0 ? 1 : 0);
            fdd::low_order::pod_vector<int> q_col((size_t)q_ptr[P]);
            fdd::low_order::pod_vector<DType> q_val((size_t)q_ptr[P]);
            fdd::low_order::parallel_ranges(P, fdd::low_order::range_parts(P), [&](long long p0, long long p1, int) {
                for (long long p = p0; p < p1; p++)
                    if (tmp[p] > 0.0)
                    {
                        q_col[q_ptr[p]] = (int)tmp[p] - 1;
                        q_val[q_ptr[p]] = (DType)1.0;
                    }
            });
            if (q_ptr[P] > 0)
                subdomain_operator.Q.adopt_csr(P, max_dof, std::move(q_ptr), std::move(q_col), std::move(q_val));
            else
                subdomain_operator.Q.initialize(P, max_dof);
        }
        subdomain_operator.Q.transpose(subdomain_operator.Qt);
        point_dof.assign(P, -1);
        for (int p = 0; p < P; p++)
            if (tmp[p] > 0.0) point_dof[p] = (int)tmp[p] - 1;
        point_dof_dev = fdd::dev().malloc<int>(std::max(P, 1));
        point_dof_dev.copyFrom(point_dof.data(), (size_t)P * sizeof(int));
        {
            std::vector<int> no_dof;
            for (int p = 0; p < P; p++)
                if (!(tmp[p] > 0.0)) no_dof.push_back(p);
            num_points_without_dof = (int)no_dof.size();
            points_without_dof = fdd::dev().malloc<int>(std::max(num_points_without_dof, 1));
            points_without_dof.copyFrom(no_dof.data(), no_dof.size() * sizeof(int));
        }
        std::vector<double>().swap(tmp);

        subdomain_operator.num_dofs = max_dof;
        subdomain_operator.num_points = subdomain_operator.Q.num_rows;
        subdomain_operator.num_extended_dofs = subdomain_operator.Q.num_cols;

        {
            fdd::LevelList ll;
            ll.level = 0;
            ll.poly_degree = poly_degree[0];
            ll.dim = dim;
            ll.D_hat = D_hat[0].second.template as<double>();
            ll.num_elements = domain.num_local_elements;
            ll.first_offset = 0;
            for (int g = 0; g < NUM_GEOM_FACTS; g++) ll.G[g] = subdomain_operator.geom_fact[g].template as<double>();
            fdd::detect_zero_factors(ll);
            fdd::detect_shared_blocks(ll);
            fdd::check_lean_table(ll, D_hat[ll.level].first);
            subdomain_operator.level_lists.push_back(ll);
        }

        superdomain_operator.num_dofs = 0;
        superdomain_operator.num_points = 0;
        superdomain_operator.num_extended_dofs = 0;

        {
            PType &coarse = domains[poly_degree[num_levels - 1]];
            const int size = coarse.num_local_points;
            std::vector<double> dof(size);
            for (int i = 0; i < size; i++) dof[i] = (coarse.mesh.p_mask[i] > 0.0) ? (double)coarse.mesh.glo_num[i] : 0.0;
            ranking(dof);
            int num_coarse_dofs = 0;
            for (int i = 0; i < size; i++) num_coarse_dofs = std::max(num_coarse_dofs, (int)dof[i]);
            Qt_coarse.initialize(num_coarse_dofs, size);
            Qt_coarse.reserve(size);
            for (int i = 0; i < size; i++)
                if (dof[i] > 0.0) Qt_coarse.add_entry((int)dof[i] - 1, i, 1.0);
            Qt_coarse.assemble();
        }

        num_interface_dofs = 0;
        num_dofs = subdomain_operator.num_dofs + superdomain_operator.num_dofs - num_interface_dofs;
        identity_matrix(Q_int, num_dofs);
        identity_matrix(Qt_int, num_dofs);
        identity_matrix(QQt_int, num_dofs);

        {
            const int nw = subdomain_operator.num_extended_dofs + superdomain_operator.num_extended_dofs;
            std::vector<DType> w(std::max(nw, 1), 1.0);
            norm_weight = fdd::dev().malloc<DType>(std::max(nw, 1));
            norm_weight.copyFrom(w.data(), w.size() * sizeof(DType));
            norm_weight_hst = w;
            norm_weight_is_one = true;
        }

    }

    static void unit_matrix(CSR_Matrix<DType> &A, int rows, int cols, const int *col)
    {
        std::vector<int> ptr(rows + 1, 0), cc;
        std::vector<DType> vv;
        for (int i = 0; i < rows; i++)
        {
            if (col[i] >= 0)
            {
                cc.push_back(col[i]);
                vv.push_back(1.0);
            }
            ptr[i + 1] = (int)cc.size();
        }
        A.assemble_from_csr(rows, cols, ptr.data(), cc.data(), vv.data());
    }

    static void host_csr_matrix(CSR_Matrix<DType> &A, const fdd::low_order::HostCSR &H)
    {
        A.assemble_from_csr(H.rows, H.cols, H.ptr.data(), H.col.data(), H.val.data());
    }

    template <typename PType>
    void initialize_composite(std::unordered_map<int, PType> &domains, PType &domain)
    {
        fdd::SetupTimer setup_timing("Subdomain::initialize_composite", fdd::comm().rank == 0);
        std::map<std::pair<int, int>, std::vector<double>> J;
        for (auto &kv : J_cf) J[kv.first] = kv.second.first;
        comp = fdd::composite::build(domains, poly_degree, subdomain_overlap, superdomain_overlap, (double)epsilon, J, D_hat[num_levels - 1].first, std::vector<int>(domain.scatter_matrix().col_hst.begin(), domain.scatter_matrix().col_hst.end()), domain.num_local_nodes, grading);
        setup_timing.lap("composite::build");
        const fdd::composite::Composite &c = comp;

        own_points = levels[0].num_points;
        const int NP = c.num_sub_ext_points;
        const int nse = c.sub_num_ext_dofs, nue = c.sup_num_ext_dofs;
        num_ring_points = NP - own_points;

        rstdout("Composite region: %d own + %d ring + %d extended elements (%d points), %d + %d subdomain dofs, %d interface, superdomain %d of %d coarse dofs (+%d extended), %d unique dofs\n", levels[0].num_elements,
                c.num_sub_elems - levels[0].num_elements, c.num_sub_ext_elems - c.num_sub_elems, NP, c.sub_num_dofs, nse - c.sub_num_dofs, c.num_interface_dofs, c.sup_num_dofs, c.num_coarse_dofs, nue - c.sup_num_dofs, c.num_dofs);

        const bool own_copy = num_ring_points > 0;
        for (int g = 0; g < NUM_GEOM_FACTS; g++)
        {
            if (own_copy)
            {
                ring_geom[g] = fdd::dev().malloc<DType>(std::max(NP, 1));
                ring_geom[g].copyFrom(c.G[g].data(), (size_t)NP * sizeof(DType));
                subdomain_operator.geom_fact[g] = ring_geom[g];
            }
            else
                subdomain_operator.geom_fact[g] = domain.geom_fact[g];
        }

        setup_timing.lap("region geometry to the device");
        for (auto &ll : subdomain_operator.level_lists) ll.factor_elem.free();
        subdomain_operator.level_lists.clear();
        for (int l = 0; l < num_levels; l++)
        {
            const int first = c.level_first_elem[l], count = c.level_num_elems[l];
            if (count == 0) continue;
            fdd::LevelList ll;
            ll.level = l;
            ll.poly_degree = poly_degree[l];
            ll.dim = dim;
            ll.D_hat = D_hat[l].second.template as<double>();
            ll.num_elements = count;
            ll.first_offset = c.sub[first].offset;
            for (int g = 0; g < NUM_GEOM_FACTS; g++) ll.G[g] = subdomain_operator.geom_fact[g].template as<double>() + ll.first_offset;
            fdd::detect_zero_factors(ll);
            fdd::detect_shared_blocks(ll);
            fdd::check_lean_table(ll, D_hat[ll.level].first);
            subdomain_operator.level_lists.push_back(ll);
        }

        subdomain_operator.Q.initialize(NP, nse);
        subdomain_operator.Q.reserve(c.Q_row.size());
        for (size_t t = 0; t < c.Q_row.size(); t++) subdomain_operator.Q.add_entry(c.Q_row[t], c.Q_col[t], c.Q_val[t]);
        subdomain_operator.Q.assemble();
        subdomain_operator.Q.transpose(subdomain_operator.Qt);
        subdomain_operator.num_dofs = c.sub_num_dofs;
        subdomain_operator.num_points = NP;
        subdomain_operator.num_extended_dofs = nse;

        setup_timing.lap("Q and Qt");
        point_dof = c.point_dof;
        point_dof_dev = fdd::dev().malloc<int>(std::max(NP, 1));
        point_dof_dev.copyFrom(point_dof.data(), (size_t)NP * sizeof(int));

        superdomain_operator.num_dofs = c.sup_num_dofs;
        superdomain_operator.num_extended_dofs = nue;
        superdomain_operator.num_points = 0;
        host_csr_matrix(superdomain_operator.A, c.A_sup);
        host_csr_matrix(superdomain_operator.Pt, c.Pt_sup);
        {
            const int nv = c.num_vertices, R = fdd::comm().size;
            int max_count = 0;
            for (int p = 0; p < R; p++) max_count = std::max(max_count, c.proc_count[p]);
            coarse_pad = max_count * nv;
            std::vector<int> owner_of(c.num_total_elements);
            for (int p = 0; p < R; p++)
                for (int e = 0; e < c.proc_count[p]; e++) owner_of[c.proc_offset[p] + e] = p;
            fdd::low_order::HostCSR Q = c.Qt_coarse;
            for (int &col : Q.col)
            {
                const int e = col / nv, v = col % nv, p = owner_of[e];
                col = p * coarse_pad + (e - c.proc_offset[p]) * nv + v;
            }
            Q.cols = R * coarse_pad;
            host_csr_matrix(Qt_coarse, Q);
            coarse_all = fdd::dev().malloc<DType>(std::max((size_t)R * coarse_pad, (size_t)1));
        }

        setup_timing.lap("superdomain operators");
        num_interface_dofs = c.num_interface_dofs;
        num_dofs = c.num_dofs;
        unit_matrix(Q_int, nse + nue, num_dofs, c.Q_int_col.data());
        unit_matrix(Qt_int, num_dofs, nse + nue, c.Qt_int_col.data());
        unit_matrix(QQt_int, nse + nue, nse + nue, c.QQt_int_col.data());
        norm_weight_hst.assign(c.norm_weight.begin(), c.norm_weight.end());
        norm_weight = fdd::dev().malloc<DType>(std::max(nse + nue, 1));
        norm_weight.copyFrom(norm_weight_hst.data(), norm_weight_hst.size() * sizeof(DType));
        norm_weight_is_one = false;

        setup_timing.lap("interface maps and weights");
        {
            std::vector<int> sidx, uidx((size_t)std::max(num_ring_points, 1), 0);
            size_t recv_total = 0;
            for (const fdd::composite::PeerPlan &pl : c.peers) recv_total += (size_t)pl.recv_points;
            exchange_ops.clear();
            std::vector<size_t> send_at, recv_at;
            size_t rat = 0;
            for (const fdd::composite::PeerPlan &pl : c.peers)
            {
                send_at.push_back(sidx.size());
                recv_at.push_back(rat);
                for (size_t k = 0; k < pl.send_level.size(); k++)
                {
                    const int l = pl.send_level[k], e = pl.send_elem[k];
                    const int np = levels[l].num_points / std::max(levels[l].num_elements, 1);
                    for (int v = 0; v < np; v++) sidx.push_back(levels[l].offset + e * np + v);
                }
                for (int r : pl.recv_elem)
                    for (int v = 0; v < c.sub[r].num_points; v++) uidx[(size_t)c.sub[r].offset - own_points + v] = (int)rat++;
            }
            num_send_points = (int)sidx.size();
            send_index = fdd::dev().malloc<int>(std::max(num_send_points, 1));
            send_index.copyFrom(sidx.data(), sidx.size() * sizeof(int));
            send_all = fdd::dev().malloc<DType>(std::max(num_send_points, 1));
            recv_all = fdd::dev().malloc<DType>(std::max(recv_total, (size_t)1));
            unpack_index = fdd::dev().malloc<int>(std::max(num_ring_points, 1));
            unpack_index.copyFrom(uidx.data(), (size_t)num_ring_points * sizeof(int));
            for (size_t k = 0; k < c.peers.size(); k++)
            {
                fdd::ExchangeOp op;
                op.peer = c.peers[k].rank;
                op.send = send_all.template as<DType>() + send_at[k];
                op.send_bytes = (size_t)c.peers[k].send_points * sizeof(DType);
                op.recv = recv_all.template as<DType>() + recv_at[k];
                op.recv_bytes = (size_t)c.peers[k].recv_points * sizeof(DType);
                exchange_ops.push_back(op);
            }
        }
// ... 854 lines not shown
```

polynomial_reduction_with_full_domain_decomposition_preconditioner_amd/host_api.py:

```python
from __future__ import annotations

import ctypes
import os
from typing import Optional, Sequence

import numpy as np

from . import lib

vp = ctypes.c_void_p

INFO_NAMES = [
    "num_local_points",
    "num_local_nodes",
    "num_bdary_nodes",
    "num_interface_slots",
    "num_total_nodes",
    "num_total_elements",
    "num_local_elements",
    "num_levels",
    "sub_num_values",
    "sub_num_dofs",
    "num_iterations",
    "dim",
# ... 300 lines not shown
        _H().call("fddh_problem_info", self.h, buf, len(INFO_NAMES))
        return {k: int(buf[i]) for i, k in enumerate(INFO_NAMES)}

    def refresh(self):
        self.info = self._info()
        return self.info

    def level_degree(self, level):
        d = ctypes.c_int()
        _H().call("fddh_problem_level_degree", self.h, level, ctypes.byref(d))
        return d.value

    def mesh_array(self, name, level=0):
        deg = self.level_degree(level)
        npts = self.info["num_local_elements"] * (deg + 1) ** self.info["dim"]
        if name == "z" and self.info["dim"] == 2:
            return np.zeros(npts)
        dtype = {"glo_num": np.int64, "node_degree": np.int32}.get(name, np.float64)
        out = np.zeros(npts, dtype)
        _H().call("fddh_problem_mesh_array", self.h, level, name.encode(), _dp(out), out.nbytes)
        return out

    def csr(self, which):
        nr, nc, nz = ctypes.c_int(), ctypes.c_int(), ctypes.c_int()
        _H().call("fddh_problem_csr", self.h, which, ctypes.byref(nr), ctypes.byref(nc), ctypes.byref(nz), None, None, None)
        ptr = np.zeros(nr.value + 1, np.int32)
        col = np.zeros(nz.value, np.int32)
        val = np.zeros(nz.value)
        _H().call("fddh_problem_csr", self.h, which, None, None, None, _dp(ptr), _dp(col), _dp(val))
        return (nr.value, nc.value), ptr, col, val

    def assembled_weight(self):
        out = np.zeros(self.info["num_local_nodes"])
        _H().call("fddh_problem_assembled_weight", self.h, _dp(out), len(out))
        return out

    def set_D_hat(self, level, D):
        D = np.ascontiguousarray(D, dtype=np.float64)
        n = self.level_degree(level) + 1
        _H().call("fddh_problem_set_D_hat", self.h, level, _dp(D), n)

    def get_D_hat(self, level):
        n = self.level_degree(level) + 1
        D = np.zeros(n * n)
        _H().call("fddh_problem_get_D_hat", self.h, level, _dp(D), n)
        return D

    def set_options(self, max_iterations=-1, tolerance=float("nan"), num_vectors=-1, use_preconditioner=-1, preconditioner_type=-1, sub_num_vectors=-1, sub_max_iterations=-1, sub_build_tree=-1):
        _H().call("fddh_problem_set_options", self.h, max_iterations, tolerance, num_vectors, int(use_preconditioner), preconditioner_type, sub_num_vectors, sub_max_iterations, int(sub_build_tree))

    def set_flag(self, name, value):
        _H().call("fddh_problem_set_flag", self.h, name.encode(), int(value))

    def affine_info(self):
        dom, aff, lists, dev = ctypes.c_int(0), ctypes.c_int(0), ctypes.c_int(0), ctypes.c_double(-1.0)
        _H().call("fddh_problem_affine_info", self.h, ctypes.byref(dom), ctypes.byref(aff), ctypes.byref(lists), ctypes.byref(dev))
        return {"fine_domain": bool(dom.value), "sub_lists_affine": aff.value, "sub_lists": lists.value, "max_deviation": dev.value}

    def zero_factor_info(self):
        on, dom, diag, lists = ctypes.c_int(0), ctypes.c_int(0), ctypes.c_int(0), ctypes.c_int(0)
        _H().call("fddh_problem_zero_factor_info", self.h, ctypes.byref(on), ctypes.byref(dom), ctypes.byref(diag), ctypes.byref(lists))
        return {"enabled": bool(on.value), "fine_domain": bool(dom.value), "sub_lists_diag": diag.value, "sub_lists": lists.value}

    def mfma_zero_factor_info(self):
        on, dom, diag, lists = ctypes.c_int(0), ctypes.c_int(0), ctypes.c_int(0), ctypes.c_int(0)
        _H().call("fddh_problem_mfma_zero_factor_info", self.h, ctypes.byref(on), ctypes.byref(dom), ctypes.byref(diag), ctypes.byref(lists))
        return {"enabled": bool(on.value), "fine_domain": bool(dom.value), "sub_lists_mfma_diag": diag.value, "sub_lists": lists.value}

    def line_stiffness_info(self):
        on, dom, lines, lists = ctypes.c_int(0), ctypes.c_int(0), ctypes.c_int(0), ctypes.c_int(0)
        _H().call("fddh_problem_line_stiffness_info", self.h, ctypes.byref(on), ctypes.byref(dom), ctypes.byref(lines), ctypes.byref(lists))
        return {"enabled": bool(on.value), "fine_domain": bool(dom.value), "sub_lists_lines": lines.value, "sub_lists": lists.value}

    def shared_factor_info(self):
        on, dom, classes, shared, lists = ctypes.c_int(0), ctypes.c_int(0), ctypes.c_int(0), ctypes.c_int(0), ctypes.c_int(0)
        _H().call("fddh_problem_shared_factor_info", self.h, ctypes.byref(on), ctypes.byref(dom), ctypes.byref(classes), ctypes.byref(shared), ctypes.byref(lists))
        return {"enabled": bool(on.value), "fine_domain": bool(dom.value), "fine_domain_classes": classes.value, "sub_lists_shared": shared.value, "sub_lists": lists.value}

    def lean_line_info(self):
        on, ok, dom, lean, lists = ctypes.c_int(0), ctypes.c_int(0), ctypes.c_int(0), ctypes.c_int(0), ctypes.c_int(0)
        _H().call("fddh_problem_lean_line_info", self.h, ctypes.byref(on), ctypes.byref(ok), ctypes.byref(dom), ctypes.byref(lean), ctypes.byref(lists))
        return {"enabled": bool(on.value), "fine_domain_table_ok": bool(ok.value), "fine_domain": bool(dom.value), "sub_lists_lean": lean.value, "sub_lists": lists.value}

    def dssum(self, u, mask=True, weight=False):
        out = np.zeros(self.n)
        _H().call("fddh_problem_dssum", self.h, _dp(out), _dp(np.ascontiguousarray(u)), int(mask), int(weight))
        return out

    def stiffness(self, u, dssum=False):
        out = np.zeros(self.n)
        _H().call("fddh_problem_stiffness", self.h, _dp(out), _dp(np.ascontiguousarray(u)), int(dssum))
        return out

    def residual_norm(self, r):
        v = ctypes.c_double()
        _H().call("fddh_problem_residual_norm", self.h, _dp(np.ascontiguousarray(r)), ctypes.byref(v))
        return v.value

    def make_rhs(self, function_id=0, seed=0):
        u_star, f = np.zeros(self.n), np.zeros(self.n)
        _H().call("fddh_problem_make_rhs", self.h, function_id, seed, _dp(u_star), _dp(f))
        return u_star, f

    def make_rhs_from(self, u_star):
        u_star = np.ascontiguousarray(u_star, dtype=np.float64).copy()
        f = np.zeros(self.n)
        _H().call("fddh_problem_make_rhs_from", self.h, _dp(u_star), _dp(f))
        return u_star, f

    def solve(self, f, method="fcg"):
        u = np.zeros(self.n)
        cap = 4096
        hist = np.zeros(cap)
        nh, its = ctypes.c_int(), ctypes.c_int()
        _H().call("fddh_problem_solve", self.h, 0 if method == "fcg" else 1, _dp(np.ascontiguousarray(f)), _dp(u), _dp(hist), cap, ctypes.byref(nh), ctypes.byref(its))
        return u, its.value, hist[: min(nh.value, cap)].copy()

    def solve_timed(self, f, method="fcg", want_solution=False):
        u = np.zeros(self.n) if want_solution else None
        cap = 4096
        hist = np.zeros(cap)
        nh, its, sec = ctypes.c_int(), ctypes.c_int(), ctypes.c_double()
        _H().call("fddh_problem_solve_timed", self.h, 0 if method == "fcg" else 1, _dp(np.ascontiguousarray(f)), _dp(u), _dp(hist), cap, ctypes.byref(nh), ctypes.byref(its), ctypes.byref(sec))
        return its.value, hist[: min(nh.value, cap)].copy(), sec.value

    def projection(self, capacity):
        _H().call("fddh_problem_projection_configure", self.h, int(capacity))

    def projection_clear(self):
        _H().call("fddh_problem_projection_clear", self.h)

    def projection_info(self):
        cap, size, restarts = ctypes.c_int(), ctypes.c_int(), ctypes.c_longlong()
        _H().call("fddh_problem_projection_info", self.h, ctypes.byref(cap), ctypes.byref(size), ctypes.byref(restarts))
        return {"capacity": cap.value, "size": size.value, "restarts": restarts.value}

    def projection_basis(self, k):
        x, ax = np.zeros(self.n), np.zeros(self.n)
        _H().call("fddh_problem_projection_basis", self.h, int(k), _dp(x), _dp(ax))
        return x, ax

    def solve_projected(self, f, method="fcg", timed=False):
        u = np.zeros(self.n)
        cap = 4096
        hist = np.zeros(cap)
        nh, its, sec = ctypes.c_int(), ctypes.c_int(), ctypes.c_double()
        proj = np.zeros(4)
        _H().call("fddh_problem_solve_projected", self.h, 0 if method == "fcg" else 1, _dp(np.ascontiguousarray(f, dtype=np.float64)), _dp(u), _dp(hist), cap, ctypes.byref(nh), ctypes.byref(its), _dp(proj),
                  ctypes.byref(sec) if timed else None)
        if timed:
            proj = np.append(proj, sec.value)
        return u, its.value, hist[: min(nh.value, cap)].copy(), proj

    def precond_apply(self, r, method="gmres"):
        z = np.zeros(self.n)
        hist = np.zeros(64)
        nh = ctypes.c_int()
        _H().call("fddh_problem_precond_apply", self.h, 0 if method == "fcg" else 1, _dp(np.ascontiguousarray(r)), _dp(z), _dp(hist), 64, ctypes.byref(nh))
        return z, hist[: nh.value].copy()

    def comm_time(self, iterations=20):
        us = (ctypes.c_double * 6)()
        nbytes = (ctypes.c_double * 6)()
        _H().call("fddh_problem_comm_time", self.h, int(iterations), us, nbytes)
        names = ["allreduce_3_scalars", "interface_pair_allreduce", "coarse_allgather", "ring_exchange", "interface_pair_neighbour_exchange", "ring_and_coarse_exchange"]
        return {n: {"avg_us": us[k], "bytes": nbytes[k]} for k, n in enumerate(names)}
# ... 145 lines not shown
```

Measured before the change: 8.517 billion DOF-updates/s.

## Assemble stiffness output directly into dofs, gathering only shared rows

Points are classified by how many element-local copies map to each dof: single-owner points, pairs, and general. The line stiffness kernel then writes single and pair contributions straight into the dof vector, encoding the class in the high bits of point_dof. A mapped CSR gather sums only the remaining general rows. The goal is to drop the full extended-point intermediate and the Qt gather pass over every point, saving HBM traffic per operator apply. In exchange it adds host-side class construction, a new kernel variant and a runtime eligibility check, gated by a flag whose default is not visible here.

Measured after the change: 8.776 billion DOF-updates/s (median of 6 runs). 3.0% higher.

```diff
diff --git a/include/fdd_hip.h b/include/fdd_hip.h
--- a/include/fdd_hip.h
+++ b/include/fdd_hip.h
@@ -152,6 +152,7 @@
 int fdd_cheby_step_f32(float *x, float *d, float *r_out, const float *r_in, const float *q, const float *dinv, float c_d, float c_r, int first, int last, int n, void *stream);
 int fdd_csr_plan_gather_cheby(const fdd_csr_plan *plan, double *x, double *d, double *r_out, const int *Qt_ptr, const int *Qt_col, const double *u, const double *r_in, const double *dinv, double c_d, double c_r, int last, void *stream);
 int fdd_csr_plan_gather_cheby_f32(const fdd_csr_plan *plan, float *x, float *d, float *r_out, const int *Qt_ptr, const int *Qt_col, const float *u, const float *r_in, const float *dinv, float c_d, float c_r, int last, void *stream);
+int fdd_csr_plan_gather_mapped(const fdd_csr_plan *plan, double *y, const int *row_map, const int *ptr, const int *col, const double *u, void *stream);
 
 size_t fdd_gmres_state_bytes(void);
 int fdd_gmres_begin_dev(void *state, const double *norm2_dev, int first_cycle, void *stream);
@@ -181,6 +182,7 @@
 int fdd_stiffness_matrix_lines_shared_f32(float *Au, const float *v, const double *v_scale_dev, const int *point_dof, const float *D_hat, const float *const G[FDD_NUM_GEOM_FACTS], const int *elem_offset, const int *factor_elem, int num_elements, int poly_degree, int diag, void *stream);
 int fdd_stiffness_matrix_lines_lean(double *Au, const double *v, const double *v_scale_dev, const int *point_dof, const double *D_hat, const double *const G[FDD_NUM_GEOM_FACTS], const int *elem_offset, const int *factor_elem, int num_elements, int poly_degree, int diag, void *stream);
 int fdd_stiffness_matrix_lines_lean_f32(float *Au, const float *v, const double *v_scale_dev, const int *point_dof, const float *D_hat, const float *const G[FDD_NUM_GEOM_FACTS], const int *elem_offset, const int *factor_elem, int num_elements, int poly_degree, int diag, void *stream);
+int fdd_stiffness_matrix_lines_direct(double *Au, double *y, const double *v, const double *v_scale_dev, const int *point_class_dof, const double *D_hat, const double *const G[FDD_NUM_GEOM_FACTS], const int *elem_offset, const int *factor_elem, int lean, int num_elements, int poly_degree, int diag, void *stream);
 int fdd_stiffness_factor_block_hash(unsigned long long *out, const double *const G[FDD_NUM_GEOM_FACTS], const int *elem_offset, int num_elements, int poly_degree, void *stream);
 int fdd_stiffness_factor_block_verify(int *mismatches, const double *const G[FDD_NUM_GEOM_FACTS], const int *elem_offset, const int *factor_elem, int num_elements, int poly_degree, void *stream);
 int fdd_stiffness_matrix_affine_f32(float *Au, const float *v, const double *v_scale_dev, const int *point_dof, const float *D_hat, const float *elem_factors, const float *gll_weights, const int *elem_offset, int num_elements, int poly_degree, void *stream);
diff --git a/include/fdd_host.h b/include/fdd_host.h
--- a/include/fdd_host.h
+++ b/include/fdd_host.h
@@ -105,6 +105,8 @@
 int fddh_problem_line_stiffness_info(fddh_problem *p, int *enabled, int *fine_domain_lines, int *sub_lists_lines, int *sub_lists);
 int fddh_problem_shared_factor_info(fddh_problem *p, int *enabled, int *fine_domain_shared, int *fine_domain_classes, int *sub_lists_shared, int *sub_lists);
 int fddh_problem_lean_line_info(fddh_problem *p, int *enabled, int *fine_domain_table_ok, int *fine_domain_lean, int *sub_lists_lean, int *sub_lists);
+int fddh_problem_assembly_info(fddh_problem *p, int *enabled, int *in_effect, long long *rows, long long *points, int *reduced_row_blocks, char *why_not, size_t why_not_len);
+int fddh_problem_assembly_arrays(fddh_problem *p, int *num_points, int *num_rows, int *num_nnz, int *point_class_dof, int *ptr, int *col, int *row_map);
 int fddh_problem_set_flag(fddh_problem *p, const char *name, int value);
 
 int fddh_problem_sub_point_dofs(const fddh_problem *p, int *dof, int n);
diff --git a/polynomial_reduction_with_full_domain_decomposition_preconditioner_amd/csrc/fdd_csr.hip b/polynomial_reduction_with_full_domain_decomposition_preconditioner_amd/csrc/fdd_csr.hip
--- a/polynomial_reduction_with_full_domain_decomposition_preconditioner_amd/csrc/fdd_csr.hip
+++ b/polynomial_reduction_with_full_domain_decomposition_preconditioner_amd/csrc/fdd_csr.hip
@@ -40,6 +40,24 @@
     __device__ T finish(T s, T, int) const { return s; }
 };
 typedef EpiPlainT<double> EpiPlain;
+template <typename T>
+struct EpiMappedT
+{
+    static constexpr bool kFreeOrder = false;
+    static constexpr bool kRowMap = true;
+    typedef int Opnd;
+    const int *row_map;
+    __device__ int operand(int row, const T *) const { return row_map[row]; }
+    __device__ T finish(T s, int, int) const { return s; }
+};
+template <typename Epi, typename = void>
+struct EpiRowMap : std::false_type
+{
+};
+template <typename Epi>
+struct EpiRowMap<Epi, std::enable_if_t<Epi::kRowMap>> : std::true_type
+{
+};
 struct EpiWeight
 {
     static constexpr bool kFreeOrder = false;
@@ -663,7 +681,10 @@
             {
                 T s = T(0);
                 for (int j = sp[r]; j < sp[r + 1]; j++) s += x[j];
-                Au[r0 + r] = epi.finish(s, o[it], r0 + r);
+                if constexpr (EpiRowMap<Epi>::value)
+                    Au[o[it]] = epi.finish(s, o[it], r0 + r);
+                else
+                    Au[r0 + r] = epi.finish(s, o[it], r0 + r);
             }
         }
         if (!more) break;
@@ -1402,6 +1423,21 @@
     return 0;
 }
 
+int fdd_csr_plan_gather_mapped(const fdd_csr_plan *plan, double *y, const int *row_map, const int *ptr, const int *col, const double *u, void *stream)
+{
+    FDD_REQUIRE(plan != nullptr);
+    if (plan->num_rows == 0) return 0;
+    FDD_REQUIRE(y != nullptr && row_map != nullptr && ptr != nullptr && col != nullptr && u != nullptr && (const void *)u != (const void *)y);
+    if (!(plan->value_bytes == 8 && plan->unit_values && plan->kind == 1 && plan->sell_slices == 0 &&
+          launch_short_pipelined<double>(plan, y, ptr, col, (const double *)nullptr, u, EpiMappedT<double>{row_map}, BlockRange{0, plan->num_blocks}, 0, plan->num_rows, fdd_stream(stream), true)))
+    {
+        fdd_set_error("fdd_csr_plan_gather_mapped: not a unit-value fp64 plan of the pipelined short-row kernel");
+        return FDD_ERR_INVALID_ARGUMENT;
+    }
+    FDD_LAUNCH_CHECK();
+    return 0;
+}
+
 int fdd_csr_plan_gather_weighted_norm2(const fdd_csr_plan *plan, double *out, double *ws, const int *Qt_ptr, const int *Qt_col, const double *u, const double *node_weight, void *stream)
 {
     FDD_REQUIRE(plan != nullptr && out != nullptr && ws != nullptr);
diff --git a/polynomial_reduction_with_full_domain_decomposition_preconditioner_amd/csrc/fdd_stiffness.hip b/polynomial_reduction_with_full_domain_decomposition_preconditioner_amd/csrc/fdd_stiffness.hip
--- a/polynomial_reduction_with_full_domain_decomposition_preconditioner_amd/csrc/fdd_stiffness.hip
+++ b/polynomial_reduction_with_full_domain_decomposition_preconditioner_amd/csrc/fdd_stiffness.hip
@@ -589,11 +589,37 @@
     }
 }
 
-template <typename T, bool kGather, bool kNTStore, bool kShared = false, int kLean = 0>
-__global__ __launch_bounds__(kBlock, 4) void line_stiffness_kernel_t(T *__restrict__ Au, const T *__restrict__ u, const int *__restrict__ point_dof, const double *__restrict__ u_scale, const T *__restrict__ D_hat, GPtrsT<T> G, const int *__restrict__ elem_offset, int num_elements, const int *__restrict__ factor_elem)
+constexpr int kDirectDofBits = 29;
+constexpr int kDirectDofMask = (1 << kDirectDofBits) - 1;
+enum : int
+{
+    kClassGeneral = 0,
+    kClassSingle = 1,
+    kClassPairLow = 2,
+    kClassPairHigh = 3
+};
+template <typename T, int kDirect>
+struct LineDirect
+{
+    T *__restrict__ y;
+};
+template <typename T>
+struct LineDirect<T, 0>
+{
+};
+template <typename T>
+__device__ __forceinline__ T *line_hand_over(int e_loc)
+{
+    __shared__ T s_h[LineCfg::epb][LineCfg::nn];
+    return s_h[e_loc];
+}
+
+template <typename T, bool kGather, bool kNTStore, bool kShared = false, int kLean = 0, int kDirect = 0>
+__global__ __launch_bounds__(kBlock, 4) void line_stiffness_kernel_t(T *__restrict__ Au, const T *__restrict__ u, const int *__restrict__ point_dof, const double *__restrict__ u_scale, const T *__restrict__ D_hat, GPtrsT<T> G, const int *__restrict__ elem_offset, int num_elements, const int *__restrict__ factor_elem, LineDirect<T, kDirect> direct)
 {
     using C = LineCfg;
     constexpr int n = C::n, nn = C::nn;
+    static_assert(kDirect == 0 or kGather, "the classes of the points come with point_dof");
     __shared__ T s_a[C::epb][C::tile];
     __shared__ T s_b[C::epb][C::tile];
 
@@ -602,132 +628,187 @@
     const int l = tid & 63;
     const int a = l & 7, b = l >> 3;
     const int elem = blockIdx.x * C::epb + e_loc;
-    if (elem >= num_elements) return;
-    const size_t base = elem_offset ? (size_t)elem_offset[elem] : (size_t)elem * C::n3;
-    size_t fbase = base;
-    if (kShared)
-    {
-        const int rep = factor_elem[elem];
-        fbase = elem_offset ? (size_t)elem_offset[rep] : (size_t)rep * C::n3;
-    }
-    T *ta = s_a[e_loc], *tb = s_b[e_loc];
-    constexpr bool kTerms = (kLean & kLeanTerms) != 0, kResident = (kLean & kLeanResident) != 0;
-    static_assert(kTerms or not kResident, "the resident table does not hold the diagonal entries");
-    const LeanTable<T, kResident> Dl(D_hat);
-
-    T r_u[n];
-    if (kGather)
-    {
-        const int *pd = point_dof + base;
-        int d[n];
-#pragma unroll
-        for (int k = 0; k < n; k++) d[k] = __builtin_nontemporal_load(pd + (l + k * nn));
-#pragma unroll
-        for (int k = 0; k < n; k++) r_u[k] = u[d[k] < 0 ? 0 : d[k]];
-#pragma unroll
-        for (int k = 0; k < n; k++) r_u[k] = (d[k] < 0) ? T(0) : r_u[k];
-        if (u_scale)
-        {
-            const T sc = (T)(*u_scale);
-#pragma unroll
-            for (int k = 0; k < n; k++) r_u[k] = sc * r_u[k];
-        }
-    }
-    else
-    {
-        const T *up = u + base;
-#pragma unroll
-        for (int k = 0; k < n; k++) r_u[k] = __builtin_nontemporal_load(up + (l + k * nn));
-    }
-
-    T r_3[n];
-    if constexpr (not kTerms)
-    {
-#pragma unroll
-        for (int m = 0; m < n; m++) r_3[m] = T(0);
-    }
-
-    {
-        T g0[n], g1[n], g2[n];
-#pragma unroll
-        for (int k = 0; k < n; k++) g2[k] = kShared ? G.g[2][fbase + (l + k * nn)] : __builtin_nontemporal_load(G.g[2] + fbase + (l + k * nn));
-        {
-            const T *g0p = G.g[0] + fbase + 8 * l;
-#pragma unroll
-            for (int p = 0; p < n; p++) g0[p] = g0p[p];
-        }
-        {
-            const T *g1p = G.g[1] + fbase + (a + nn * b);
-#pragma unroll
-            for (int p = 0; p < n; p++) g1[p] = kShared ? g1p[8 * p] : __builtin_nontemporal_load(g1p + 8 * p);
-        }
-
-#pragma unroll
-        for (int k = 0; k < n; k++) ta[C::at(a, b, k)] = r_u[k];
-        element_sync<true>();
-
-#pragma unroll
-        for (int k = 0; k < n; k++)
-        {
-            if constexpr (kTerms)
-            {
-                const T *Dk = Dl.row(k);
-                T Du_3 = Dl.at(Dk, k, 0) * r_u[0];
-#pragma unroll
-                for (int p = 1; p < n; p++)
-                    if (not lean_zero_entry(k, p)) Du_3 += Dl.at(Dk, k, p) * r_u[p];
-                const T GDu_3 = g2[k] * Du_3;
-#pragma unroll
-                for (int m = 0; m < n; m++)
+    if constexpr (kDirect == 0)
+    {
+        if (elem >= num_elements) return;
+    }
+    const bool active = kDirect == 0 or elem < num_elements;
+    int d[n];
+    T v[n];
+    if (active)
+    {
+        const size_t base = elem_offset ? (size_t)elem_offset[elem] : (size_t)elem * C::n3;
+        size_t fbase = base;
+        if (kShared)
+        {
+            const int rep = factor_elem[elem];
+            fbase = elem_offset ? (size_t)elem_offset[rep] : (size_t)rep * C::n3;
+        }
+        T *ta = s_a[e_loc], *tb = s_b[e_loc];
+        constexpr bool kTerms = (kLean & kLeanTerms) != 0, kResident = (kLean & kLeanResident) != 0;
+        static_assert(kTerms or not kResident, "the resident table does not hold the diagonal entries");
+        const LeanTable<T, kResident> Dl(D_hat);
+
+        T r_u[n];
+        if (kGather)
+        {
+            const int *pd = point_dof + base;
+#pragma unroll
+            for (int k = 0; k < n; k++) d[k] = __builtin_nontemporal_load(pd + (l + k * nn));
+#pragma unroll
+            for (int k = 0; k < n; k++) r_u[k] = u[d[k] < 0 ? 0 : (kDirect != 0 ? (d[k] & kDirectDofMask) : d[k])];
+#pragma unroll
+            for (int k = 0; k < n; k++) r_u[k] = (d[k] < 0) ? T(0) : r_u[k];
+            if (u_scale)
+            {
+                const T sc = (T)(*u_scale);
+#pragma unroll
+                for (int k = 0; k < n; k++) r_u[k] = sc * r_u[k];
+            }
+        }
+        else
+        {
+            const T *up = u + base;
+#pragma unroll
+            for (int k = 0; k < n; k++) r_u[k] = __builtin_nontemporal_load(up + (l + k * nn));
+        }
+
+        T r_3[n];
+        if constexpr (not kTerms)
+        {
+#pragma unroll
+            for (int m = 0; m < n; m++) r_3[m] = T(0);
+        }
+
+        {
+            T g0[n], g1[n], g2[n];
+#pragma unroll
+            for (int k = 0; k < n; k++) g2[k] = kShared ? G.g[2][fbase + (l + k * nn)] : __builtin_nontemporal_load(G.g[2] + fbase + (l + k * nn));
+            {
+                const T *g0p = G.g[0] + fbase + 8 * l;
+#pragma unroll
+                for (int p = 0; p < n; p++) g0[p] = g0p[p];
+            }
+            {
+                const T *g1p = G.g[1] + fbase + (a + nn * b);
+#pragma unroll
+                for (int p = 0; p < n; p++) g1[p] = kShared ? g1p[8 * p] : __builtin_nontemporal_load(g1p + 8 * p);
+            }
+
+#pragma unroll
+            for (int k = 0; k < n; k++) ta[C::at(a, b, k)] = r_u[k];
+            element_sync<true>();
+
+#pragma unroll
+            for (int k = 0; k < n; k++)
+            {
+                if constexpr (kTerms)
                 {
-                    if (k == 0)
-                        r_3[m] = Dl.at(Dk, 0, m) * GDu_3;
-                    else if (not lean_zero_entry(k, m))
-                        r_3[m] += Dl.at(Dk, k, m) * GDu_3;
+                    const T *Dk = Dl.row(k);
+                    T Du_3 = Dl.at(Dk, k, 0) * r_u[0];
+#pragma unroll
+                    for (int p = 1; p < n; p++)
+                        if (not lean_zero_entry(k, p)) Du_3 += Dl.at(Dk, k, p) * r_u[p];
+                    const T GDu_3 = g2[k] * Du_3;
+#pragma unroll
+                    for (int m = 0; m < n; m++)
+                    {
+                        if (k == 0)
+                            r_3[m] = Dl.at(Dk, 0, m) * GDu_3;
+                        else if (not lean_zero_entry(k, m))
+                            r_3[m] += Dl.at(Dk, k, m) * GDu_3;
+                    }
                 }
-            }
-            else
-            {
-                const T *Dk = line_row(D_hat, k);
-                T Du_3 = T(0);
-#pragma unroll
-                for (int p = 0; p < n; p++) Du_3 += Dk[p] * r_u[p];
-                const T GDu_3 = g2[k] * Du_3;
-#pragma unroll
-                for (int m = 0; m < n; m++) r_3[m] += Dk[m] * GDu_3;
-            }
-        }
-
-        T ul[n], w[n], au[n];
-#pragma unroll
-        for (int p = 0; p < n; p++) ul[p] = ta[C::at(p, a, b)];
-        if constexpr (kTerms) lean_du(w, ul, Dl); else line_du(w, ul, D_hat);
-#pragma unroll
-        for (int p = 0; p < n; p++) w[p] = g0[p] * w[p];
-        if constexpr (kTerms) lean_au(au, w, Dl); else line_au(au, w, D_hat);
-#pragma unroll
-        for (int p = 0; p < n; p++) tb[C::at(p, a, b)] = au[p];
-#pragma unroll
-        for (int p = 0; p < n; p++) ul[p] = ta[C::at(a, p, b)];
-        element_sync<true>();
-        if constexpr (kTerms) lean_du(w, ul, Dl); else line_du(w, ul, D_hat);
-#pragma unroll
-        for (int p = 0; p < n; p++) w[p] = g1[p] * w[p];
-        if constexpr (kTerms) lean_au(au, w, Dl); else line_au(au, w, D_hat);
-#pragma unroll
-        for (int p = 0; p < n; p++) ta[C::at(a, p, b)] = au[p];
-        element_sync<true>();
-    }
-
-    T *Aup = Au + base;
-#pragma unroll
-    for (int k = 0; k < n; k++)
-    {
-        const T v = (tb[C::at(a, b, k)] + ta[C::at(a, b, k)]) + r_3[k];
-        if (kNTStore)
-            __builtin_nontemporal_store(v, Aup + (l + k * nn));
+                else
+                {
+                    const T *Dk = line_row(D_hat, k);
+                    T Du_3 = T(0);
+#pragma unroll
+                    for (int p = 0; p < n; p++) Du_3 += Dk[p] * r_u[p];
+                    const T GDu_3 = g2[k] * Du_3;
+#pragma unroll
+                    for (int m = 0; m < n; m++) r_3[m] += Dk[m] * GDu_3;
+                }
+            }
+
+            T ul[n], w[n], au[n];
+#pragma unroll
+            for (int p = 0; p < n; p++) ul[p] = ta[C::at(p, a, b)];
+            if constexpr (kTerms) lean_du(w, ul, Dl); else line_du(w, ul, D_hat);
+#pragma unroll
+            for (int p = 0; p < n; p++) w[p] = g0[p] * w[p];
+            if constexpr (kTerms) lean_au(au, w, Dl); else line_au(au, w, D_hat);
+#pragma unroll
+            for (int p = 0; p < n; p++) tb[C::at(p, a, b)] = au[p];
+#pragma unroll
+            for (int p = 0; p < n; p++) ul[p] = ta[C::at(a, p, b)];
+            element_sync<true>();
+            if constexpr (kTerms) lean_du(w, ul, Dl); else line_du(w, ul, D_hat);
+#pragma unroll
+            for (int p = 0; p < n; p++) w[p] = g1[p] * w[p];
+            if constexpr (kTerms) lean_au(au, w, Dl); else line_au(au, w, D_hat);
+#pragma unroll
+            for (int p = 0; p < n; p++) ta[C::at(a, p, b)] = au[p];
+            element_sync<true>();
+        }
+
+        T *Aup = Au + base;
+        if constexpr (kDirect == 0)
+        {
+#pragma unroll
+            for (int k = 0; k < n; k++)
+            {
+                v[k] = (tb[C::at(a, b, k)] + ta[C::at(a, b, k)]) + r_3[k];
+                if (kNTStore)
+                    __builtin_nontemporal_store(v[k], Aup + (l + k * nn));
+                else
+                    Aup[l + k * nn] = v[k];
+            }
+        }
         else
-            Aup[l + k * nn] = v;
+        {
+#pragma unroll
+            for (int k = 0; k < n; k++)
+            {
+                v[k] = (tb[C::at(a, b, k)] + ta[C::at(a, b, k)]) + r_3[k];
+                const int cls = d[k] >> kDirectDofBits, dof = d[k] & kDirectDofMask;
+                if (cls == kClassGeneral)
+                {
+                    if (kNTStore)
+                        __builtin_nontemporal_store(v[k], Aup + (l + k * nn));
+                    else
+                        Aup[l + k * nn] = v[k];
+                }
+                else if (cls == kClassSingle)
+                {
+                    const T s = T(0) + v[k];
+                    if (kDirect == 2)
+                        __builtin_nontemporal_store(s, direct.y + dof);
+                    else
+                        direct.y[dof] = s;
+                }
+                else if (cls == kClassPairLow)
+                    line_hand_over<T>(e_loc)[b + 8 * k] = v[k];
+            }
+        }
+    }
+    if constexpr (kDirect != 0)
+    {
+        element_sync<false>();
+        if (active)
+        {
+            const T *left = line_hand_over<T>(e_loc > 0 ? e_loc - 1 : 0);
+#pragma unroll
+            for (int k = 0; k < n; k++)
+                if ((d[k] >> kDirectDofBits) == kClassPairHigh)
+                {
+                    const T s = (T(0) + left[b + 8 * k]) + v[k];
+                    if (kDirect == 2)
+                        __builtin_nontemporal_store(s, direct.y + (d[k] & kDirectDofMask));
+                    else
+                        direct.y[d[k] & kDirectDofMask] = s;
+                }
+        }
     }
 }
 
@@ -737,7 +818,29 @@
     const int grid = (num_elements + LineCfg::epb - 1) / LineCfg::epb;
     fdd_for_bool(factor_elem != nullptr, [&](auto shared) {
         for_gather_nt_store(point_dof, [&](auto gather, auto nt) {
-            hipLaunchKernelGGL((line_stiffness_kernel_t<T, decltype(gather)::value, decltype(nt)::value, decltype(shared)::value, kLean>), dim3(grid), dim3(kBlock), 0, fdd_stream(stream), Au, u, point_dof, u_scale, D_hat, G, elem_offset, num_elements, factor_elem);
+            hipLaunchKernelGGL((line_stiffness_kernel_t<T, decltype(gather)::value, decltype(nt)::value, decltype(shared)::value, kLean>), dim3(grid), dim3(kBlock), 0, fdd_stream(stream), Au, u, point_dof, u_scale, D_hat, G, elem_offset, num_elements, factor_elem, LineDirect<T, 0>{});
+        });
+    });
+    FDD_LAUNCH_CHECK();
+    return 0;
+}
+
+inline bool assemble_nt_store()
+{
+    static const bool nt_store = fdd_env_int("FDD_TUNE_ASSEMBLE_NT_STORE", 0) != 0;
+    return nt_store;
+}
+
+template <int kLean>
+int launch_lines_direct(double *Au, double *y, const double *u, const int *point_class_dof, const double *u_scale, const double *D_hat, const GPtrsT<double> &G, const int *elem_offset, const int *factor_elem, int num_elements, void *stream)
+{
+    const int grid = (num_elements + LineCfg::epb - 1) / LineCfg::epb;
+    fdd_for_bool(factor_elem != nullptr, [&](auto shared) {
+        fdd_for_bool(stiffness_nt_store(), [&](auto nt) {
+            fdd_for_bool(assemble_nt_store(), [&](auto nt_y) {
+                constexpr int kDirect = decltype(nt_y)::value ? 2 : 1;
+                hipLaunchKernelGGL((line_stiffness_kernel_t<double, true, decltype(nt)::value, decltype(shared)::value, kLean, kDirect>), dim3(grid), dim3(kBlock), 0, fdd_stream(stream), Au, u, point_class_dof, u_scale, D_hat, G, elem_offset, num_elements, factor_elem, LineDirect<double, kDirect>{y});
+            });
         });
     });
     FDD_LAUNCH_CHECK();
@@ -761,7 +864,7 @@
     lean
 };
 template <typename T>
-int lines_dispatch(LineEntry entry, T *Au, const T *u, const int *point_dof, const double *u_scale, const T *D_hat, const T *const G[FDD_NUM_GEOM_FACTS], const int *elem_offset, const int *factor_elem, int num_elements, int poly_degree, int diag, void *stream)
+int lines_dispatch(LineEntry entry, T *Au, const T *u, const int *point_dof, const double *u_scale, const T *D_hat, const T *const G[FDD_NUM_GEOM_FACTS], const int *elem_offset, const int *factor_elem, int num_elements, int poly_degree, int diag, void *stream, bool direct = false, T *direct_y = nullptr)
 {
     if (entry == LineEntry::shared && diag != 1)
     {
@@ -787,8 +890,15 @@
     if (num_elements == 0) return 0;
     FDD_REQUIRE(Au != nullptr && u != nullptr && D_hat != nullptr && G != nullptr);
     FDD_REQUIRE(entry != LineEntry::shared || factor_elem != nullptr);
+    FDD_REQUIRE(not direct || (point_dof != nullptr && direct_y != nullptr && (const void *)direct_y != (const void *)u && (const void *)direct_y != (const void *)Au));
     GPtrsT<T> g;
     if (int rc = fdd_three_factors(g, G)) return rc;
+    if constexpr (sizeof(T) == 8)
+        if (direct)
+        {
+            if (entry != LineEntry::lean) return launch_lines_direct<0>(Au, direct_y, u, point_dof, u_scale, D_hat, g, elem_offset, entry == LineEntry::shared ? factor_elem : nullptr, num_elements, stream);
+            return launch_lines_direct<(kLeanTerms | kLeanResident)>(Au, direct_y, u, point_dof, u_scale, D_hat, g, elem_offset, factor_elem, num_elements, stream);
+        }
     if (entry != LineEntry::lean) return launch_lines_t<T, 0>(Au, u, point_dof, u_scale, D_hat, g, elem_offset, entry == LineEntry::shared ? factor_elem : nullptr, num_elements, stream);
     constexpr int kParts = sizeof(T) == 8 ? (kLeanTerms | kLeanResident) : kLeanTerms;
 #ifdef FDD_LEAN_LINE_DEV
@@ -1178,6 +1288,12 @@
     return lines_dispatch<float>(LineEntry::streamed, Au, v, point_dof, v_scale_dev, D_hat, G, elem_offset, nullptr, num_elements, poly_degree, diag, stream);
 }
 
+int fdd_stiffness_matrix_lines_direct(double *Au, double *y, const double *v, const double *v_scale_dev, const int *point_class_dof, const double *D_hat, const double *const G[FDD_NUM_GEOM_FACTS], const int *elem_offset, const int *factor_elem, int lean, int num_elements, int poly_degree, int diag, void *stream)
+{
+    const LineEntry entry = lean != 0 ? LineEntry::lean : (factor_elem != nullptr ? LineEntry::shared : LineEntry::streamed);
+    return lines_dispatch<double>(entry, Au, v, point_class_dof, v_scale_dev, D_hat, G, elem_offset, factor_elem, num_elements, poly_degree, diag, stream, true, y);
+}
+
 int fdd_stiffness_matrix_lines_shared(double *Au, const double *v, const double *v_scale_dev, const int *point_dof, const double *D_hat, const double *const G[FDD_NUM_GEOM_FACTS], const int *elem_offset, const int *factor_elem, int num_elements, int poly_degree, int diag, void *stream)
 {
     return lines_dispatch<double>(LineEntry::shared, Au, v, point_dof, v_scale_dev, D_hat, G, elem_offset, factor_elem, num_elements, poly_degree, diag, stream);
diff --git a/polynomial_reduction_with_full_domain_decomposition_preconditioner_amd/host/assembly_classes.hpp b/polynomial_reduction_with_full_domain_decomposition_preconditioner_amd/host/assembly_classes.hpp
--- /dev/null
+++ b/polynomial_reduction_with_full_domain_decomposition_preconditioner_amd/host/assembly_classes.hpp
@@ -0,0 +1,156 @@
+#ifndef FDD_ASSEMBLY_CLASSES_HPP
+#define FDD_ASSEMBLY_CLASSES_HPP
+
+#include <string>
+#include <vector>
+
+#include "element_operator.hpp"
+
+namespace fdd
+{
+
+struct AssemblyClasses
+{
+    static constexpr int kDofBits = 29;
+    enum : int
+    {
+        general = 0,
+        single = 1,
+        pair_low = 2,
+        pair_high = 3,
+        none = 4
+    };
+
+    bool built = false;
+    std::string unusable;
+    long long rows[3] = {0, 0, 0};
+    long long points[5] = {0, 0, 0, 0, 0};
+    int reduced_blocks = 0;
+    std::vector<int> point_class_dof, ptr, col, row_map;
+
+    bool on_device = false;
+    memory point_class_dof_dev, ptr_dev, col_dev, row_map_dev;
+    fdd_csr_plan *plan = nullptr;
+
+    void clear()
+    {
+        for (memory *m : {&point_class_dof_dev, &ptr_dev, &col_dev, &row_map_dev}) m->free();
+        if (plan) FDD_CALL(fdd_csr_plan_destroy(plan));
+        *this = AssemblyClasses();
+    }
+
+    void build(const int *qt_ptr, const int *qt_col, int num_rows, int num_points, const std::vector<int> &point_dof, const std::vector<LevelList> &lists)
+    {
+        clear();
+        built = true;
+        point_class_dof.assign(point_dof.begin(), point_dof.end());
+        std::vector<char> cls((size_t)num_rows, (char)general);
+        const auto locate = [&](int p, int &list, int &e, int &i, int &jk) {
+            for (size_t t = 0; t < lists.size(); t++)
+            {
+                const LevelList &ll = lists[t];
+                if (ll.dim != 3 or ll.poly_degree != 7 or p < ll.first_offset or (long long)p >= (long long)ll.first_offset + (long long)ll.num_points()) continue;
+                const int at = p - ll.first_offset;
+                list = (int)t, e = at / 512, i = at & 7, jk = (at >> 3) & 63;
+                return true;
+            }
+            return false;
+        };
+        bool consistent = (int)point_dof.size() == num_points;
+        std::vector<char> seen((size_t)num_points, 0);
+        for (int r = 0; r < num_rows; r++)
+        {
+            const int len = qt_ptr[r + 1] - qt_ptr[r];
+            const int *c = qt_col + qt_ptr[r];
+            for (int t = 0; t < len; t++)
+            {
+                if (c[t] < 0 or c[t] >= num_points or (consistent and (point_dof[c[t]] != r or seen[c[t]])))
+                    consistent = false;
+                else
+                    seen[c[t]] = 1;
+            }
+            if (len == 1)
+                cls[r] = (char)single;
+            else if (len == 2 and consistent)
+            {
+                int l0, e0, i0, jk0, l1, e1, i1, jk1;
+                if (locate(c[0], l0, e0, i0, jk0) and locate(c[1], l1, e1, i1, jk1) and l0 == l1 and e1 == e0 + 1 and i0 == 7 and i1 == 0 and jk0 == jk1 and e0 / 4 == e1 / 4) cls[r] = (char)pair_low;
+            }
+        }
+        if (consistent)
+            for (int p = 0; p < num_points; p++)
+                if ((point_dof[p] >= 0) != (seen[p] != 0)) consistent = false;
+        if (not consistent)
+            unusable = "point_dof is not the transpose of Qt's columns";
+        else if (num_rows > (1 << kDofBits))
+            unusable = "the dof count leaves no spare bits in point_dof";
+        if (not unusable.empty())
+        {
+            point_class_dof.clear();
+            return;
+        }
+        ptr.assign(1, 0);
+        for (int r = 0; r < num_rows; r++)
+        {
+            const int len = qt_ptr[r + 1] - qt_ptr[r];
+            const int *c = qt_col + qt_ptr[r];
+            const int k = cls[r] == (char)pair_low ? 2 : (int)cls[r];
+            rows[k]++;
+            for (int t = 0; t < len; t++)
+            {
+                const int pc = cls[r] == (char)pair_low ? (t == 0 ? pair_low : pair_high) : (int)cls[r];
+                point_class_dof[c[t]] = r | (pc << kDofBits);
+                points[pc]++;
+            }
+        }
+        for (int r = 0; r < num_rows; r++)
+            if (cls[r] == (char)general)
+            {
+                col.insert(col.end(), qt_col + qt_ptr[r], qt_col + qt_ptr[r + 1]);
+                ptr.push_back((int)col.size());
+                row_map.push_back(r);
+            }
+        points[none] = (long long)num_points - points[general] - points[single] - points[pair_low] - points[pair_high];
+    }
+
+    bool ensure_device()
+    {
+        if (on_device) return true;
+        if (not built or not unusable.empty()) return false;
+        const size_t nr = row_map.size();
+        if (nr > 0)
+        {
+            FDD_CALL(fdd_csr_plan_create(&plan, ptr.data(), (int)nr, (int)point_class_dof.size(), (int)col.size()));
+            FDD_CALL(fdd_csr_plan_set_unit_values(plan, 1));
+            int pipelined = 0;
+            FDD_CALL(fdd_csr_plan_pipelined(plan, &pipelined));
+            FDD_CALL(fdd_csr_plan_num_blocks(plan, &reduced_blocks));
+            if (not pipelined)
+            {
+                FDD_CALL(fdd_csr_plan_destroy(plan));
+                plan = nullptr;
+                unusable = "the plan of the general rows does not run on the pipelined short-row kernel";
+                return false;
+            }
+            ptr_dev = dev().malloc<int>(nr + 1), col_dev = dev().malloc<int>(col.size()), row_map_dev = dev().malloc<int>(nr);
+            ptr_dev.copyFrom(ptr.data(), (nr + 1) * sizeof(int));
+            col_dev.copyFrom(col.data(), col.size() * sizeof(int));
+            row_map_dev.copyFrom(row_map.data(), nr * sizeof(int));
+        }
+        point_class_dof_dev = dev().malloc<int>(std::max<size_t>(point_class_dof.size(), 1));
+        if (not point_class_dof.empty()) point_class_dof_dev.copyFrom(point_class_dof.data(), point_class_dof.size() * sizeof(int));
+        on_device = true;
+        return true;
+    }
+
+    void gather_general(double *y, const double *q) const
+    {
+        if (row_map.empty()) return;
+        ProfileScope prof("csr_short_pipelined_kernel<gather, mapped>", 16.0 * (double)row_map.size() + 12.0 * (double)col.size() + 4.0);
+        FDD_CALL(fdd_csr_plan_gather_mapped(plan, y, row_map_dev.as<int>(), ptr_dev.as<int>(), col_dev.as<int>(), q, dev().stream));
+    }
+};
+
+}
+
+#endif
diff --git a/polynomial_reduction_with_full_domain_decomposition_preconditioner_amd/host/element_operator.hpp b/polynomial_reduction_with_full_domain_decomposition_preconditioner_amd/host/element_operator.hpp
--- a/polynomial_reduction_with_full_domain_decomposition_preconditioner_amd/host/element_operator.hpp
+++ b/polynomial_reduction_with_full_domain_decomposition_preconditioner_amd/host/element_operator.hpp
@@ -55,6 +55,7 @@
     bool line_stiffness;
     bool shared_factor_blocks;
     bool lean_line_stiffness;
+    bool assemble_in_stiffness;
 
     StiffnessFlags();
 };
@@ -70,16 +71,17 @@
     } entries[5];
 };
 
-inline const std::array<StiffnessFlagRow, 6> &stiffness_flag_table()
+inline const std::array<StiffnessFlagRow, 7> &stiffness_flag_table()
 {
 #define FDD_ENTRY(name) {(const void *)&name, #name}
-    static const std::array<StiffnessFlagRow, 6> table = {{
+    static const std::array<StiffnessFlagRow, 7> table = {{
         {"mfma_stiffness", &StiffnessFlags::mfma_stiffness, {}},
         {"skip_zero_factors", &StiffnessFlags::skip_zero_factors, {FDD_ENTRY(fdd_stiffness_offdiag_zero), FDD_ENTRY(fdd_stiffness_matrix_diag), FDD_ENTRY(fdd_stiffness_matrix_diag_f32)}},
         {"mfma_skip_zero_factors", &StiffnessFlags::mfma_skip_zero_factors, {FDD_ENTRY(fdd_stiffness_matrix_mfma_diag), FDD_ENTRY(fdd_stiffness_offdiag_zero), FDD_ENTRY(fdd_stiffness_matrix_diag), FDD_ENTRY(fdd_stiffness_matrix_diag_f32)}},
         {"line_stiffness", &StiffnessFlags::line_stiffness, {FDD_ENTRY(fdd_stiffness_matrix_lines), FDD_ENTRY(fdd_stiffness_matrix_lines_f32)}},
         {"shared_factor_blocks", &StiffnessFlags::shared_factor_blocks, {FDD_ENTRY(fdd_stiffness_matrix_lines_shared), FDD_ENTRY(fdd_stiffness_matrix_lines_shared_f32), FDD_ENTRY(fdd_stiffness_factor_block_hash), FDD_ENTRY(fdd_stiffness_factor_block_verify)}},
         {"lean_line_stiffness", &StiffnessFlags::lean_line_stiffness, {FDD_ENTRY(fdd_stiffness_matrix_lines_lean), FDD_ENTRY(fdd_stiffness_matrix_lines_lean_f32)}},
+        {"assemble_in_stiffness", &StiffnessFlags::assemble_in_stiffness, {FDD_ENTRY(fdd_stiffness_matrix_lines_direct), FDD_ENTRY(fdd_csr_plan_gather_mapped)}},
     }};
 #undef FDD_ENTRY
     return table;
@@ -377,6 +379,17 @@
         FDD_CALL((matrix_cores ? fdd_stiffness_matrix_mfma_gather : fdd_sub_stiffness_matrix_gather_scaled)(q, v, scale_dev, point_index, a.D_hat, a.G, nullptr, ll.num_elements, ll.poly_degree, stream));
 }
 
+inline bool direct_lines_apply(const LevelList &ll, const StiffnessFlags &flags) { return flags.assemble_in_stiffness and choose_stiffness(ll, flags, false, StiffnessForm::gather).lines(); }
+
+inline void apply_gather_direct(const LevelList &ll, double *q, double *y, const double *v, const int *point_class_dof, const double *scale_dev, int gathered_values, const StiffnessFlags &flags)
+{
+    q += ll.first_offset, point_class_dof += ll.first_offset;
+    const StiffnessChoice c = choose_stiffness(ll, flags, false, StiffnessForm::gather);
+    const StiffnessProfile p = stiffness_profile(StiffnessForm::gather, c, false);
+    ProfileScope prof(p.label, p.bytes_per_point * (double)ll.num_points() + (double)sizeof(double) * gathered_values);
+    FDD_CALL(fdd_stiffness_matrix_lines_direct(q, y, v, scale_dev, point_class_dof, ll.D_hat, ll.G, nullptr, c.shared ? ll.factor_elem.as<int>() : nullptr, c.lean ? 1 : 0, ll.num_elements, ll.poly_degree, 1, dev().stream));
+}
+
 constexpr double affine_tolerance = 64.0 * 2.220446049250313e-16;
 inline bool detect_affine(LevelList &ll)
 {
diff --git a/polynomial_reduction_with_full_domain_decomposition_preconditioner_amd/host/fdd_device.hpp b/polynomial_reduction_with_full_domain_decomposition_preconditioner_amd/host/fdd_device.hpp
--- a/polynomial_reduction_with_full_domain_decomposition_preconditioner_amd/host/fdd_device.hpp
+++ b/polynomial_reduction_with_full_domain_decomposition_preconditioner_amd/host/fdd_device.hpp
@@ -47,6 +47,8 @@
 #pragma weak fdd_stiffness_factor_block_verify
 #pragma weak fdd_stiffness_matrix_lines_lean
 #pragma weak fdd_stiffness_matrix_lines_lean_f32
+#pragma weak fdd_stiffness_matrix_lines_direct
+#pragma weak fdd_csr_plan_gather_mapped
 
 namespace fdd
 {
diff --git a/polynomial_reduction_with_full_domain_decomposition_preconditioner_amd/host/fdd_host_capi.cpp b/polynomial_reduction_with_full_domain_decomposition_preconditioner_amd/host/fdd_host_capi.cpp
--- a/polynomial_reduction_with_full_domain_decomposition_preconditioner_amd/host/fdd_host_capi.cpp
+++ b/polynomial_reduction_with_full_domain_decomposition_preconditioner_amd/host/fdd_host_capi.cpp
@@ -973,6 +973,56 @@
     });
 }
 
+int fddh_problem_assembly_info(fddh_problem *p, int *enabled, int *in_effect, long long *rows, long long *points, int *reduced_row_blocks, char *why_not, size_t why_not_len)
+{
+    try
+    {
+        if (int rc = rank_check(p)) return rc;
+        if (!p) return fail("null argument");
+        if (!p->subdomain) return fail("problem was created without a Subdomain");
+        Subdomain<SType> &sub = *p->subdomain;
+        if (enabled) *enabled = sub.stiffness.assemble_in_stiffness ? 1 : 0;
+        const char *obstacle = sub.assembly_obstacle();
+        if (!sub.assembly.built) sub.assembly_build();
+        if (in_effect) *in_effect = obstacle == nullptr ? 1 : 0;
+        if (rows) std::copy(sub.assembly.rows, sub.assembly.rows + 3, rows);
+        if (points) std::copy(sub.assembly.points, sub.assembly.points + 5, points);
+        if (reduced_row_blocks) *reduced_row_blocks = sub.assembly.reduced_blocks;
+        if (why_not && why_not_len > 0) snprintf(why_not, why_not_len, "%s", obstacle ? obstacle : "");
+        return 0;
+    }
+    catch (const std::exception &e)
+    {
+        return fail("%s", e.what());
+    }
+}
+
+int fddh_problem_assembly_arrays(fddh_problem *p, int *num_points, int *num_rows, int *num_nnz, int *point_class_dof, int *ptr, int *col, int *row_map)
+{
+    try
+    {
+        if (int rc = rank_check(p)) return rc;
+        if (!p) return fail("null argument");
+        if (!p->subdomain) return fail("problem was created without a Subdomain");
+        Subdomain<SType> &sub = *p->subdomain;
+        if (!sub.assembly.built) sub.assembly_build();
+        const fdd::AssemblyClasses &a = sub.assembly;
+        if (!a.unusable.empty()) return fail("no classes: %s", a.unusable.c_str());
+        if (num_points) *num_points = (int)a.point_class_dof.size();
+        if (num_rows) *num_rows = (int)a.row_map.size();
+        if (num_nnz) *num_nnz = (int)a.col.size();
+        if (point_class_dof) std::copy(a.point_class_dof.begin(), a.point_class_dof.end(), point_class_dof);
+        if (ptr) std::copy(a.ptr.begin(), a.ptr.end(), ptr);
+        if (col) std::copy(a.col.begin(), a.col.end(), col);
+        if (row_map) std::copy(a.row_map.begin(), a.row_map.end(), row_map);
+        return 0;
+    }
+    catch (const std::exception &e)
+    {
+        return fail("%s", e.what());
+    }
+}
+
 int fddh_problem_set_flag(fddh_problem *p, const char *name, int value)
 {
     try
diff --git a/polynomial_reduction_with_full_domain_decomposition_preconditioner_amd/host/subdomain.hpp b/polynomial_reduction_with_full_domain_decomposition_preconditioner_amd/host/subdomain.hpp
--- a/polynomial_reduction_with_full_domain_decomposition_preconditioner_amd/host/subdomain.hpp
+++ b/polynomial_reduction_with_full_domain_decomposition_preconditioner_amd/host/subdomain.hpp
@@ -11,6 +11,7 @@
 
 #include "amg.hpp"
 #include "amg_device_setup.hpp"
+#include "assembly_classes.hpp"
 #include "composite.hpp"
 #include "config.hpp"
 #include "csr_matrix.hpp"
@@ -790,6 +791,34 @@
         for (auto &ll : subdomain_operator.level_lists) fdd::apply_gather(ll, q, za, point_dof_dev.template as<int>(), scale_dev, subdomain_operator.num_extended_dofs, stiffness);
     }
 
+  public:
+    fdd::AssemblyClasses assembly;
+    void assembly_build()
+    {
+        CSR_Matrix<DType> &Qt = subdomain_operator.Qt;
+        std::vector<int> ptr((size_t)Qt.num_rows + 1, 0), col((size_t)Qt.num_nnz);
+        if (Qt.num_nnz > 0)
+        {
+            Qt.ptr.copyTo(ptr.data(), ptr.size() * sizeof(int));
+            Qt.col.copyTo(col.data(), col.size() * sizeof(int));
+        }
+        assembly.build(ptr.data(), col.data(), Qt.num_rows, subdomain_operator.num_points, point_dof, subdomain_operator.level_lists);
+    }
+    const char *assembly_obstacle()
+    {
+        if (not stiffness.assemble_in_stiffness) return "the flag is off";
+        if (precision != 64) return "the inner solve runs in float";
+        if (is_composite) return "a composite region";
+        if (not norm_weight_is_one) return "the gather is weighted";
+        if (subdomain_operator.level_lists.empty() or subdomain_operator.Qt.num_nnz == 0 or subdomain_operator.Qt.num_rows != subdomain_operator.num_extended_dofs or not subdomain_operator.Qt.unit_values) return "no boolean gather over every dof";
+        for (auto &ll : subdomain_operator.level_lists)
+            if (not fdd::direct_lines_apply(ll, stiffness)) return "a list does not run the degree-7 line form";
+        if (not assembly.built) assembly_build();
+        if (not assembly.ensure_device()) return assembly.unusable.c_str();
+        return nullptr;
+    }
+
+  private:
     template <typename Real>
     void operator_dofs(Real *y, Real *x, const double *scale_dev = nullptr)
     {
@@ -799,6 +828,13 @@
         const int nse = subdomain_operator.num_extended_dofs;
         if (not is_composite)
         {
+            if constexpr (not f32)
+                if (y != x and assembly_obstacle() == nullptr)
+                {
+                    for (auto &ll : subdomain_operator.level_lists) fdd::apply_gather_direct(ll, q, y, x, assembly.point_class_dof_dev.template as<int>(), scale_dev, nse, stiffness);
+                    assembly.gather_general(y, q);
+                    return;
+                }
             stiffness_from_dofs(q, x, scale_dev);
             if constexpr (f32)
                 subdomain_operator.Qt.gather(y, q, 0, nse);
@@ -1374,6 +1410,7 @@
                 subdomain_operator.Q.initialize(P, max_dof);
         }
         subdomain_operator.Q.transpose(subdomain_operator.Qt);
+        assembly.clear();
         point_dof.assign(P, -1);
         for (int p = 0; p < P; p++)
             if (tmp[p] > 0.0) point_dof[p] = (int)tmp[p] - 1;
@@ -1522,6 +1559,7 @@
         for (size_t t = 0; t < c.Q_row.size(); t++) subdomain_operator.Q.add_entry(c.Q_row[t], c.Q_col[t], c.Q_val[t]);
         subdomain_operator.Q.assemble();
         subdomain_operator.Q.transpose(subdomain_operator.Qt);
+        assembly.clear();
         subdomain_operator.num_dofs = c.sub_num_dofs;
         subdomain_operator.num_points = NP;
         subdomain_operator.num_extended_dofs = nse;
diff --git a/polynomial_reduction_with_full_domain_decomposition_preconditioner_amd/host_api.py b/polynomial_reduction_with_full_domain_decomposition_preconditioner_amd/host_api.py
--- a/polynomial_reduction_with_full_domain_decomposition_preconditioner_amd/host_api.py
+++ b/polynomial_reduction_with_full_domain_decomposition_preconditioner_amd/host_api.py
@@ -406,6 +406,21 @@
         _H().call("fddh_problem_lean_line_info", self.h, ctypes.byref(on), ctypes.byref(ok), ctypes.byref(dom), ctypes.byref(lean), ctypes.byref(lists))
         return {"enabled": bool(on.value), "fine_domain_table_ok": bool(ok.value), "fine_domain": bool(dom.value), "sub_lists_lean": lean.value, "sub_lists": lists.value}
 
+    def assembly_info(self):
+        on, eff, blocks = ctypes.c_int(0), ctypes.c_int(0), ctypes.c_int(0)
+        rows, points, why = (ctypes.c_longlong * 3)(), (ctypes.c_longlong * 5)(), ctypes.create_string_buffer(256)
+        _H().call("fddh_problem_assembly_info", self.h, ctypes.byref(on), ctypes.byref(eff), rows, points, ctypes.byref(blocks), why, len(why))
+        return {"enabled": bool(on.value), "in_effect": bool(eff.value), "why_not": why.value.decode(), "rows": dict(zip(("general", "single", "pair"), map(int, rows))),
+                "points": dict(zip(("general", "single", "pair_low", "pair_high", "none"), map(int, points))), "reduced_row_blocks": blocks.value}
+
+    def assembly_arrays(self):
+        npts, nr, nz = ctypes.c_int(), ctypes.c_int(), ctypes.c_int()
+        _H().call("fddh_problem_assembly_arrays", self.h, ctypes.byref(npts), ctypes.byref(nr), ctypes.byref(nz), None, None, None, None)
+        pcd, ptr, col, rmap = np.zeros(npts.value, np.int32), np.zeros(nr.value + 1, np.int32), np.zeros(nz.value, np.int32), np.zeros(nr.value, np.int32)
+        ip = lambda a: a.ctypes.data_as(ctypes.POINTER(ctypes.c_int))
+        _H().call("fddh_problem_assembly_arrays", self.h, None, None, None, ip(pcd), ip(ptr), ip(col), ip(rmap))
+        return pcd, ptr, col, rmap
+
     def dssum(self, u, mask=True, weight=False):
         out = np.zeros(self.n)
         _H().call("fddh_problem_dssum", self.h, _dp(out), _dp(np.ascontiguousarray(u)), int(mask), int(weight))
```
